# HighCWu/ControlLoRA

Measured on AMD Instinct MI355X. Metric: train images/sec SD-1.5+ControlLoRA 512^2 bs4/GPU, higher is better.
Workload: dtype f16; 1 GPU; configs/fill50k.json on SD-1.5 topology (seeded random weights), 512x512, bs=4/GPU, fp16; hot path = hint encoder + UNet fwd/bwd + adapter AdamW; latents/text embeddings synthetic (VAE/CLIP outside the hot path); global_batch=4, parallelism=dp1, hipgraph=True, allreduce_bytes=24188160, rccl_ranks=1, comm=torch, comm_requested=auto

## Files before the change

### controllora_amd/capi.py

```python
from __future__ import annotations

import ctypes as C
import os
from typing import Optional

import torch

_HERE = os.path.dirname(os.path.abspath(__file__))
LIB_PATH = os.environ.get("CLORA_LIB_PATH") or os.path.join(_HERE, "_build", "libclora.so")

ABI_VERSION = 4
OK, ERR_ARG, ERR_LAUNCH, ERR_WORKSPACE = 0, -1, -2, -3
_ERR = {ERR_ARG: "bad argument", ERR_LAUNCH: "kernel launch failed", ERR_WORKSPACE: "workspace too small"}


class CloraError(RuntimeError):
    pass


class ConvDesc(C.Structure):
    _fields_ = [(n, C.c_int) for n in (
        "enabled", "Hin", "Win", "Cin", "Hout", "Wout", "ksize", "mul", "kmul", "off", "lim_h", "lim_w", "shift",
        "need_even", "kchunk")]


class Epilogue(C.Structure):
    _fields_ = [("bias", C.c_void_p), ("rowadd", C.c_void_p), ("rows_per_batch", C.c_int), ("ld_rowadd", C.c_int),
                ("residual", C.c_void_p), ("ldr", C.c_int), ("lora_t", C.c_void_p), ("ldt", C.c_int),
                ("lora_u", C.c_void_p), ("ldu", C.c_int), ("lora_u_tr", C.c_int), ("lora_r", C.c_int), ("lora_seg", C.c_int), ("lora_scale", C.c_float),
                ("geglu", C.c_int), ("geglu_f", C.c_int), ("geglu_h", C.c_void_p), ("geglu_y", C.c_void_p),
                ("lora_dpack", C.c_void_p), ("lora_t_in", C.c_void_p), ("ldt_in", C.c_int), ("lora_t_in_rows", C.c_int),
                ("lora_t_in_mask", C.c_uint), ("defer", C.c_void_p),
                ("ln_gamma", C.c_void_p), ("ln_beta", C.c_void_p), ("ln_out", C.c_void_p), ("ln_eps", C.c_float),
                ("residual_lo", C.c_void_p), ("c_lo", C.c_void_p)]


class GemmTile(C.Structure):
    _fields_ = [(n, C.c_int) for n in ("tile_cfg", "family", "bm", "bn", "wm", "wn", "nst", "bk", "flags", "caps")]


TILE_RING, TILE_V1, TILE_EIGHT_PHASE, TILE_PATCH, TILE_PATCH_WIDE, TILE_STRIP = range(6)
TILE_CAP_GEGLU, TILE_CAP_DPACK, TILE_CAP_LN, TILE_CAP_CONV = 1, 2, 4, 8


class Deferred(C.Structure):
    _fields_ = [("partial", C.c_void_p), ("splits", C.c_int), ("M", C.c_int), ("N", C.c_int), ("C", C.c_void_p), ("ldc", C.c_int),
                ("epi", Epilogue)]


class LoraPackJob(C.Structure):
    _fields_ = [("D", C.c_void_p), ("out", C.c_void_p), ("ldd", C.c_int), ("R", C.c_int), ("K", C.c_int), ("kmajor", C.c_int),
                ("scale", C.c_float), ("pad_", C.c_int)]


class LoraDownJob(C.Structure):
    _fields_ = [("X", C.c_void_p), ("ldx", C.c_int), ("D", C.c_void_p), ("ldd", C.c_int), ("T", C.c_void_p), ("ldt", C.c_int),
                ("toff", C.c_int), ("M", C.c_int), ("K", C.c_int), ("R", C.c_int), ("accumulate", C.c_int), ("x_rows", C.c_int),
                ("d_kmajor", C.c_int), ("d_scale", C.c_float), ("X2", C.c_void_p), ("ldx2", C.c_int), ("x2_rows", C.c_int),
                ("r2", C.c_int), ("T_in", C.c_void_p), ("ldt_in", C.c_int), ("t_in_rows", C.c_int), ("t_in_r", C.c_int)]


class RankSite(C.Structure):
    _fields_ = [("Dq", C.c_void_p), ("lddq", C.c_int), ("Uc", C.c_void_p), ("lduc", C.c_int), ("M", C.c_void_p),
                ("Tc", C.c_void_p), ("ldtc", C.c_int), ("toff", C.c_int), ("Tq", C.c_void_p), ("ldtq", C.c_int),
                ("dTc", C.c_void_p), ("lddtc", C.c_int), ("gDq", C.c_void_p), ("gUc", C.c_void_p),
                ("rows", C.c_int), ("C", C.c_int), ("rc", C.c_int), ("scale", C.c_float)]


class LoraUpJob(C.Structure):
    _fields_ = [("base", C.c_void_p), ("ldb", C.c_int), ("T", C.c_void_p), ("ldt", C.c_int), ("toff", C.c_int), ("U", C.c_void_p),
                ("ldu", C.c_int), ("u_transposed", C.c_int), ("Y", C.c_void_p), ("ldy", C.c_int), ("M", C.c_int), ("N", C.c_int),
                ("R", C.c_int), ("scale", C.c_float)]


class LoraFoldMember(C.Structure):
    _fields_ = [("up", C.c_void_p), ("down", C.c_void_p), ("ldu", C.c_int), ("ldd", C.c_int), ("r", C.c_int), ("scale", C.c_float)]


LORA_FOLD_MAX_MEMBERS = 8


class LoraFoldJob(C.Structure):
    _fields_ = [("W", C.c_void_p), ("out", C.c_void_p), ("out_t", C.c_void_p), ("ldw", C.c_int), ("ldo", C.c_int), ("ldt", C.c_int),
                ("rows", C.c_int), ("K", C.c_int), ("nmem", C.c_int), ("m", LoraFoldMember * LORA_FOLD_MAX_MEMBERS)]


class ControlMixMember(C.Structure):
    _fields_ = [("T", C.c_void_p), ("ldt", C.c_int), ("toff", C.c_int), ("U", C.c_void_p), ("ldu", C.c_int), ("r", C.c_int),
                ("scale", C.c_float)]


CONTROL_MIX_MAX_MEMBERS = 8


class ControlMixJob(C.Structure):
    _fields_ = [("Y", C.c_void_p), ("ldy", C.c_int), ("M", C.c_int), ("N", C.c_int), ("rows_t", C.c_int), ("nmem", C.c_int),
                ("m", ControlMixMember * CONTROL_MIX_MAX_MEMBERS)]


class ControlChainMember(C.Structure):
    _fields_ = [("Dh", C.c_void_p), ("ldd", C.c_int), ("U", C.c_void_p), ("ldu", C.c_int), ("Tc", C.c_void_p), ("ldt", C.c_int),
                ("toff", C.c_int), ("r", C.c_int)]


CONTROL_CHAIN_MAX_MEMBERS = 8


class ControlChainJob(C.Structure):
    _fields_ = [("H", C.c_void_p), ("ldh", C.c_int), ("Y", C.c_void_p), ("ldy", C.c_int), ("G", C.c_void_p), ("ldg", C.c_int),
                ("M", C.c_int), ("C", C.c_int), ("rows_t", C.c_int), ("nmem", C.c_int), ("scale", C.c_float),
                ("m", ControlChainMember * CONTROL_CHAIN_MAX_MEMBERS)]


class LoraWgradJob(C.Structure):
    _fields_ = [("A", C.c_void_p), ("lda", C.c_int), ("T", C.c_void_p), ("ldt", C.c_int), ("toff", C.c_int), ("G", C.c_void_p),
                ("gs_n", C.c_int), ("gs_j", C.c_int), ("M", C.c_int), ("N", C.c_int), ("R", C.c_int), ("scale", C.c_float),
                ("a_rows", C.c_int), ("A2", C.c_void_p), ("lda2", C.c_int)]


class ConvPackJob(C.Structure):
    _fields_ = [("w", C.c_void_p), ("fwd", C.c_void_p), ("dgrad", C.c_void_p), ("Co", C.c_int), ("Ci", C.c_int), ("ksize", C.c_int),
                ("Cip", C.c_int), ("Cop", C.c_int), ("pad_", C.c_int)]


class ConvUnpackJob(C.Structure):
    _fields_ = [("stage", C.c_void_p), ("stage_b", C.c_void_p), ("grad_w", C.c_void_p), ("grad_b", C.c_void_p), ("Co", C.c_int),
                ("Ci", C.c_int), ("ksize", C.c_int), ("Cip", C.c_int)]


class SamplerCoef(C.Structure):
    _fields_ = [(n, C.c_float) for n in ("guidance", "x0_x", "x0_e", "k_x", "k_x0", "k_h", "k_e", "k_n")]


class ConvActJob(C.Structure):
    _fields_ = [("x", C.c_void_p), ("ldx", C.c_int), ("w", C.c_void_p), ("bias", C.c_void_p), ("y", C.c_void_p), ("ldy", C.c_int),
                ("Cin", C.c_int), ("Cout", C.c_int), ("relu", C.c_int)]


CONV_ACT_MAX_JOBS = 2
LORA_MAX_JOBS = 16
LORA_WGRAD_MAX_JOBS = 32
WGRAD_JOBS_PER_LAUNCH = min(LORA_WGRAD_MAX_JOBS, max(1, int(os.environ.get("CLORA_WGRAD_JOBS", "32"))))
CONV_MAX_JOBS = 32
CANNY_MAX_GROUP = 64
_P, _I, _Z, _F, _LL = C.c_void_p, C.c_int, C.c_size_t, C.c_float, C.c_longlong
_PROTOS = {
    "clora_gemm_f16": [_P, _I, _P, _P, _I, _I, _I, _I, C.POINTER(ConvDesc), C.POINTER(Epilogue), _I, _P, _Z, _P],
    "clora_gemm_f16_ex": [_P, _I, _P, _P, _I, _I, _I, _I, C.POINTER(ConvDesc), C.POINTER(Epilogue), _I, _I, _P, _Z, _P],
    "clora_conv_patch_eligible": [_I, C.POINTER(ConvDesc), _I],
    "clora_conv_strip_eligible": [_I, _I, C.POINTER(ConvDesc)],
    "clora_set_option": [C.c_char_p, _I],
    "clora_conv_wgrad_f16": [_P, _I, _P, _I, _P, _P, _I, _I, _I, C.POINTER(ConvDesc), _I, _P],
    "clora_conv_weight_pack_f32": [_P, _I, _I, _I, _I, _I, _P, _P, _P],
    "clora_conv_wgrad_unpack_f32": [_P, _P, _P, _P, _I, _I, _I, _I, _P],
    "clora_conv_weight_pack_multi_f32": [C.POINTER(ConvPackJob), _I, _P],
    "clora_conv_wgrad_unpack_multi_f32": [C.POINTER(ConvUnpackJob), _I, _P],
    "clora_attn_fwd_f16": [_P, _I, _P, _I, _P, _I, _P, _I, _P, _I, _I, _I, _I, _I, _F, _P],
    "clora_attn_max_head_dim": [_I],
    "clora_attn_fwd_causal_f16": [_P, _I, _P, _I, _P, _I, _P, _I, _I, _I, _I, _I, _F, _P],
    "clora_attn_bwd_f16": [_P, _I, _P, _I, _P, _I, _P, _I, _P, _I, _P, _P, _P, _I, _P, _I, _P, _I, _I, _I, _I, _I, _I, _F, _P, _Z, _P],
    "clora_groupnorm_fwd_f16": [_P, _P, _P, _P, _P, _I, _I, _I, _I, _F, _I, _P, _Z, _P],
    "clora_groupnorm_bwd_f16": [_P, _P, _P, _P, _P, _P, _P, _P, _P, _I, _I, _I, _I, _I, _I, _P, _Z, _P],
    "clora_groupnorm_fwd_f16_ex": [_P, _P, _I, C.POINTER(Deferred), _P, _P, _P, _P, _P, _I, _I, _I, _I, _F, _I, _P, _Z, _P],
    "clora_groupnorm_bwd_f16_ex": [_P, _P, C.POINTER(Deferred), _P, _P, _P, _I, _P, _P, _P, _P, _P, _I, _I, _I, _I, _I, _I, _P, _Z, _P],
    "clora_groupnorm_fwd_f16_team": [_P, _P, _I, C.POINTER(Deferred), _P, _P, _P, _P, _P, _I, _I, _I, _I, _F, _I, _P, _Z, _P, _Z, _P],
    "clora_groupnorm_fwd_f16_lo": [_P, _P, _I, C.POINTER(Deferred), _P, _P, _P, _P, _P, _I, _I, _I, _I, _F, _I, _P, _Z, _P, _Z, _P, _P, _P],
    "clora_layernorm_fwd_f16_lo": [_P, _P, _P, _P, _I, _I, _F, _P, _P],
    "clora_groupnorm_bwd_f16_team": [_P, _P, C.POINTER(Deferred), _P, _P, _P, _I, _P, _P, _P, _P, _P, _I, _I, _I, _I, _I, _I, _P, _Z, _P, _Z, _P],
    "clora_layernorm_bwd_f16_ex": [_P, _P, C.POINTER(Deferred), _P, _P, _P, _I, _I, _F, _P],
    "clora_finish_deferred": [C.POINTER(Deferred), _P],
    "clora_gemm_ln_fusable": [_I, _I, _I, _I, _I],
    "clora_gemm_tile_info": [_I, C.POINTER(GemmTile)],
    "clora_gemm_tile_at": [_I, C.POINTER(GemmTile)],
    "clora_gemm_fused_down_tile": [_I, _I, _I, C.POINTER(_I)],
    "clora_layernorm_fwd_f16": [_P, _P, _P, _P, _I, _I, _F, _P],
    "clora_softmax_rows_f16": [_P, _P, _I, _I, _I, _F, _P],
    "clora_layernorm_bwd_f16": [_P, _P, _P, _P, _P, _I, _I, _F, _P],
    "clora_geglu_fwd_f16": [_P, _P, _I, _I, _P],
    "clora_geglu_bwd_f16": [_P, _P, _P, _I, _I, _P],
    "clora_lora_down_f16": [_P, _I, _P, _I, _P, _I, _I, _I, _I, _I, _I, _I, _I, _F, _P],
    "clora_lora_down_multi_f16": [C.POINTER(LoraDownJob), _I, _P],
    "clora_lora_wgrad_multi_f16": [C.POINTER(LoraWgradJob), _I, _P, _Z, _P],
    "clora_lora_pack_f16": [_P, _I, _I, _P],
    "clora_rank_compose_f32": [C.POINTER(RankSite), _I, _P],
    "clora_rank_mix_f32": [C.POINTER(RankSite), _I, _I, _P, _Z, _P],
    "clora_rank_compose_bwd_f32": [C.POINTER(RankSite), _I, _P, _P],
    "clora_lora_up_f16": [_P, _I, _P, _I, _I, _P, _I, _I, _P, _I, _I, _I, _I, _F, _P],
    "clora_lora_up_multi_f16": [C.POINTER(LoraUpJob), _I, _P],
    "clora_lora_fold_f16": [_P, _I, _P],
    "clora_control_mix_q_f16": [C.POINTER(ControlMixJob), _P],
    "clora_control_chain_f16": [C.POINTER(ControlChainJob), _P],
    "clora_lora_wgrad_f16": [_P, _I, _P, _I, _I, _P, _I, _I, _I, _I, _I, _F, _I, _P, _Z, _P],
    "clora_comm_unique_id": [_P],
    "clora_comm_init": [_P, _I, _I],
    "clora_comm_library": [C.c_char_p, _Z],
    "clora_comm_world": [],
    "clora_comm_rank": [],
    "clora_allreduce_flat_f32": [_P, _Z, _P],
    "clora_comm_destroy": [],
    "clora_add_f16": [_P, _P, _P, _Z, _P],
    "clora_silu_f16": [_P, _P, _Z, _P],
    "clora_timestep_embedding_f16": [_P, _I, _I, _P, _P, _I, _I, _P],
    "clora_silu_bwd_f16": [_P, _P, _P, _Z, _P],
    "clora_quick_gelu_f16": [_P, _P, _Z, _P],
    "clora_copy2d_f16": [_P, _I, _P, _I, _Z, _I, _P],
    "clora_pool2x2_sum_f16": [_P, _P, _I, _I, _I, _I, _P],
    "clora_colsum_f16": [_P, _I, _P, _I, _I, _P],
    "clora_mse_f16": [_P, _P, _P, _P, _Z, _F, _P, _P],
    "clora_mse_weighted_f16": [_P, _P, _P, _P, _P, _I, _Z, _F, _P, _P],
    "clora_cast_f32_to_f16": [_P, _P, _Z, _P],
    "clora_cast_f16_to_f32": [_P, _P, _Z, _P],
    "clora_grad_sumsq_f32": [_P, _Z, _P, _P],
    "clora_optim_prep_f32": [_P, _F, _F, _F, _I, _F, _F, _I, _P],
    "clora_adamw_flat_f32": [_P, _P, _P, _P, _Z, _P, _F, _F, _F, _F, _F, _P],
    "clora_canny_classify_u8": [_P, _P, _P, _P, _I, _I, _I, _I, _P],
    "clora_canny_hysteresis_u8": [_P, _P, _I, _I, _I, _I, _I, _P],
    "clora_canny_emit": [_P, _P, _P, _I, _I, _I, _P],
    "clora_sampler_step_f16": [_P, _LL, _LL, _LL, _LL, _P, _P, _P, _P, _P, _LL, _I, _I, _I, _I, C.POINTER(SamplerCoef), _P],
    "clora_conv_act_f16": [C.POINTER(ConvActJob), _I, _I, _I, _I, _I, _P, _Z, _P],
    "clora_conv_act_workspace": [C.POINTER(ConvActJob), _I, _I, _I, _I, _I],
    "clora_conv_act_splits": [C.POINTER(ConvActJob), _I, _I, _I, _I, _I],
    "clora_conv_act_pack_f32": [_P, _P, _P, _I, _I, _I, _I, _P],
    "clora_maxpool2x2_f16": [_P, _P, _I, _I, _I, _I, _P],
    "clora_abi_version": [],
    "clora_clock_probe": [_P, _I, _I, _P],
    "clora_groupnorm_workspace_bytes": [_I, _I, _I, _I, _I, _I],
    "clora_groupnorm_team_state_bytes": [],
    "clora_lora_wgrad_workspace_bytes": [_I, _I, _I],
    "clora_rank_gram_ws_bytes": [_I, _I],
}


class Lib:

    def __init__(self, path: str = LIB_PATH, require_device: bool = True):
        if not os.path.exists(path):
            raise CloraError(
                f"{path} not found: the gfx950 kernel library is not built.  Run `python -m controllora_amd.build` "
                "(hipcc --offload-arch=gfx950).  There is no CPU / PyTorch fallback for this path.")
        self.path = path
        self.require_device = require_device
        self.cdll = C.CDLL(path)
        got = self.cdll.clora_abi_version() if hasattr(self.cdll, "clora_abi_version") else -1
        if got != ABI_VERSION and os.environ.get("CLORA_ABI_ANY", "") != "1":
            raise CloraError(f"{path} reports ABI {got}, this binding is written for ABI {ABI_VERSION} (include/clora.h); rebuild with "
                             "`python -m controllora_amd.build` (CLORA_ABI_ANY=1 overrides for A/B runs of older builds whose "
                             "struct layouts are known to match)")
        for name, argtypes in _PROTOS.items():
            if not hasattr(self.cdll, name) and os.environ.get("CLORA_ABI_ANY", "") == "1":
                continue
            fn = getattr(self.cdll, name)
            fn.argtypes = argtypes
            fn.restype = C.c_int
        self.cdll.clora_build_info.restype = C.c_char_p
        self.cdll.clora_groupnorm_workspace_bytes.restype = C.c_size_t
        self.cdll.clora_groupnorm_team_state_bytes.restype = C.c_size_t
        self.cdll.clora_lora_wgrad_workspace_bytes.restype = C.c_size_t
        self.cdll.clora_rank_gram_ws_bytes.restype = C.c_size_t
        if hasattr(self.cdll, "clora_conv_act_workspace"):
            self.cdll.clora_conv_act_workspace.restype = C.c_size_t
        self._options_from_env()
        self._derived = {}

    def derived(self, key, make):
        if key not in self._derived:
            self._derived[key] = make(self)
        return self._derived[key]

    def tiles(self) -> dict:
        def read(L):
            rows, r = {}, GemmTile()
            while L.cdll.clora_gemm_tile_at(len(rows), C.byref(r)) == OK:
                rows[r.tile_cfg], r = r, GemmTile()
            return rows
        return self.derived("tiles", read)

    _ENV_OPTIONS = {"CLORA_TILE_ORDER": ("tile_order", {"m": 0, "n": 1, "auto": 2, "a": 2, "grid": 3, "g": 3}), "CLORA_LN_ROWS": ("ln_rows", None),
                    "CLORA_ATTN_FWD_WAVES": ("attn_fwd_waves", None), "CLORA_ATTN_BWD_WAVES": ("attn_bwd_waves", None),
                    "CLORA_GN_BLOCKS": ("gn_blocks", None), "CLORA_EPI_TWO_PHASE": ("epi_two_phase", None),
                    "CLORA_LORA_DOWN_MODE": ("lora_down_mode", None), "CLORA_GN_UNROLL": ("gn_unroll", None),
                    "CLORA_EPI_HOIST": ("epi_hoist", None), "CLORA_GN_RESIDENT": ("gn_resident", None),
                    "CLORA_DEFER_MAX_ROWS": ("defer_max_rows", None), "CLORA_WGRAD_PATCH": ("wgrad_patch", None), "CLORA_STRIP_BLOCKS": ("strip_blocks", None),
                    "CLORA_GN_TEAM": ("gn_team", None)}

    def _options_from_env(self):
        for var, (name, names) in self._ENV_OPTIONS.items():
            v = os.environ.get(var)
            if v is None or v == "":
                continue
            try:
                val = names[v] if (names and v in names) else int(v)
                self.call("clora_set_option", name.encode(), val)
            except (ValueError, CloraError) as e:
                allowed = f"one of {sorted(names)} or an integer" if names else "an integer in the range include/clora.h documents"
                raise CloraError(f"environment variable {var}={v!r} is not a valid value for the library option "
                                 f"{name!r} (expected {allowed})") from e

    def call(self, name: str, *args) -> None:
        rc = getattr(self.cdll, name)(*args)
        if rc != OK:
            raise CloraError(f"{name} failed: {_ERR.get(rc, rc)}")


_LIB: Optional[Lib] = None


def lib() -> Lib:
    global _LIB
    if _LIB is None:
        _LIB = Lib()
    return _LIB


def ptr(t: Optional[torch.Tensor], dtype=None) -> Optional[int]:
    if t is None:
        return None
    L = lib()
    if L.require_device and not t.is_cuda:
        raise CloraError("libclora kernels need tensors on a HIP device (no CPU fallback)")
    if dtype is not None and t.dtype != dtype:
        raise CloraError(f"expected {dtype}, got {t.dtype}")
    return t.data_ptr()


def stream() -> Optional[int]:
    if lib().require_device:
        return torch.cuda.current_stream().cuda_stream
    return None
```

### controllora_amd/csrc/clora_common.h

```cpp
#pragma once
#include <hip/hip_runtime.h>
#include <stdint.h>

typedef _Float16 half_t;
typedef _Float16 half2v __attribute__((ext_vector_type(2)));
typedef _Float16 half4v __attribute__((ext_vector_type(4)));
typedef _Float16 half8 __attribute__((ext_vector_type(8)));
typedef float floatx4 __attribute__((ext_vector_type(4)));

#define CLORA_WAVE 64

#define CLORA_OK 0
#define CLORA_ERR_ARG (-1)
#define CLORA_ERR_LAUNCH (-2)
#define CLORA_ERR_WORKSPACE (-3)

#ifndef CLORA_ASYNC_PRIMS
#define CLORA_ASYNC_PRIMS
#define CLORA_GLDS16(gptr, lptr)                                                                      \
    __builtin_amdgcn_global_load_lds((const __attribute__((address_space(1))) void*)(gptr),            \
                                     (__attribute__((address_space(3))) void*)(lptr), 16, 0, 0)
#define CLORA_WAIT_VMCNT(n) asm volatile("s_waitcnt vmcnt(%0)" ::"n"(n) : "memory")
#define CLORA_RAW_BARRIER() __builtin_amdgcn_s_barrier()
typedef __fp16 clora_fp16x4 __attribute__((__vector_size__(4 * sizeof(__fp16))));
// ... 10 lines not shown
#define CLORA_KEEP_PURE(x) asm("" : "+v"(x))
#define CLORA_FMA_F32(acc, a, b) asm("v_fma_f32 %0, %1, %2, %0" : "+v"(acc) : "v"(a), "v"(b))
#define CLORA_CYCLES() ((unsigned long long)__builtin_readcyclecounter())
#define CLORA_WALL_TICKS() ((unsigned long long)wall_clock64())
#define CLORA_MFMA_INPLACE(acc, a, b) asm volatile("v_mfma_f32_16x16x32_f16 %0, %1, %2, %0" : "+v"(acc) : "v"(a), "v"(b))
#define CLORA_MFMA_DRAIN() asm volatile("s_nop 15\n\ts_nop 15" ::: "memory")
#define CLORA_WAIT_LGKMCNT(n) asm volatile("s_waitcnt lgkmcnt(%0)" ::"n"(n) : "memory")
#define CLORA_SETPRIO(n) __builtin_amdgcn_s_setprio(n)
#define CLORA_SCHED_BARRIER() __builtin_amdgcn_sched_barrier(0)
typedef __attribute__((address_space(1))) unsigned long long clora_gu64;
typedef __attribute__((address_space(1))) unsigned clora_gu32;
#define CLORA_LD_AGENT_U64(p) __hip_atomic_load((clora_gu64*)(p), __ATOMIC_RELAXED, __HIP_MEMORY_SCOPE_AGENT)
#define CLORA_ST_AGENT_U64(p, v) __hip_atomic_store((clora_gu64*)(p), (unsigned long long)(v), __ATOMIC_RELAXED, __HIP_MEMORY_SCOPE_AGENT)
#define CLORA_LD_AGENT_U32(p) __hip_atomic_load((clora_gu32*)(p), __ATOMIC_RELAXED, __HIP_MEMORY_SCOPE_AGENT)
#define CLORA_ST_AGENT_U32(p, v) __hip_atomic_store((clora_gu32*)(p), (unsigned)(v), __ATOMIC_RELAXED, __HIP_MEMORY_SCOPE_AGENT)
#define CLORA_SLEEP() __builtin_amdgcn_s_sleep(1)
#endif
#ifndef CLORA_SEQUENTIAL_BLOCKS
#define CLORA_SEQUENTIAL_BLOCKS 0
#endif

__device__ __forceinline__ floatx4 mfma16(half8 a, half8 b, floatx4 c) {
    return __builtin_amdgcn_mfma_f32_16x16x32_f16(a, b, c, 0, 0, 0);
}

__device__ __forceinline__ half8 ld8(const half_t* p) { return *reinterpret_cast<const half8*>(p); }
__device__ __forceinline__ void st8(half_t* p, half8 v) { *reinterpret_cast<half8*>(p) = v; }
__device__ __forceinline__ half4v ld4(const half_t* p) { return *reinterpret_cast<const half4v*>(p); }
__device__ __forceinline__ void st4(half_t* p, half4v v) { *reinterpret_cast<half4v*>(p) = v; }
__device__ __forceinline__ half8 zero8() {
    half8 z = {0, 0, 0, 0, 0, 0, 0, 0};
    return z;
}
__device__ __forceinline__ floatx4 zero4f() {
    floatx4 z = {0.f, 0.f, 0.f, 0.f};
    return z;
}

__device__ __forceinline__ float sigmoid_f(float x) { return CLORA_RCP(1.0f + CLORA_EXP2(-1.4426950408889634f * x)); }
__device__ __forceinline__ float silu_f(float x) { return x * sigmoid_f(x); }
__device__ __forceinline__ float dsilu_f(float x) {
    float s = sigmoid_f(x);
    return s * (1.0f + x * (1.0f - s));
}
__device__ __forceinline__ void gelu_parts(float x, float& cdf, float& pdf) {
    const float ax = fabsf(x) * 0.70710678118654752f;
    const float t = CLORA_RCP(1.0f + 0.3275911f * ax);
    const float ex = CLORA_EXP2(-1.4426950408889634f * ax * ax);
    const float poly = t * (0.254829592f + t * (-0.284496736f + t * (1.421413741f + t * (-1.453152027f + t * 1.061405429f))));
    const float erf_abs = 1.0f - poly * ex;
    cdf = 0.5f * (1.0f + (x < 0.f ? -erf_abs : erf_abs));
    pdf = 0.39894228040143268f * ex;
}
__device__ __forceinline__ float gelu_f(float x) {
    float cdf, pdf;
    gelu_parts(x, cdf, pdf);
    return x * cdf;
}
__device__ __forceinline__ float dgelu_f(float x) {
    float cdf, pdf;
    gelu_parts(x, cdf, pdf);
    return cdf + x * pdf;
}

__device__ __forceinline__ float wave_sum(float v) {
    v += __shfl_xor(v, 32);
    v += __shfl_xor(v, 16);
    v += __shfl_xor(v, 8);
    v += __shfl_xor(v, 4);
    v += __shfl_xor(v, 2);
    v += __shfl_xor(v, 1);
    return v;
}
__device__ __forceinline__ float wave_max(float v) {
    v = fmaxf(v, __shfl_xor(v, 32));
    v = fmaxf(v, __shfl_xor(v, 16));
    v = fmaxf(v, __shfl_xor(v, 8));
    v = fmaxf(v, __shfl_xor(v, 4));
    v = fmaxf(v, __shfl_xor(v, 2));
    v = fmaxf(v, __shfl_xor(v, 1));
    return v;
}

enum { CLORA_OPT_TILE_ORDER = 0, CLORA_OPT_LN_ROWS, CLORA_OPT_ATTN_FWD_WAVES, CLORA_OPT_ATTN_BWD_WAVES, CLORA_OPT_GN_BLOCKS, CLORA_OPT_EPI_TWO_PHASE, CLORA_OPT_LORA_DOWN_MODE, CLORA_OPT_GN_UNROLL, CLORA_OPT_EPI_HOIST, CLORA_OPT_GN_RESIDENT, CLORA_OPT_DEFER_MAX_ROWS, CLORA_OPT_WGRAD_PATCH, CLORA_OPT_STRIP_BLOCKS, CLORA_OPT_GN_TEAM, CLORA_OPT_COUNT };
__attribute__((visibility("hidden"))) int clora_option(int id);
static inline int clora_xcd_policy() { return clora_option(CLORA_OPT_TILE_ORDER); }
static inline int clora_ln_rows() { return clora_option(CLORA_OPT_LN_ROWS); }

static inline int clora_check_launch() { return hipGetLastError() == hipSuccess ? CLORA_OK : CLORA_ERR_LAUNCH; }
static inline int clora_cdiv(long a, long b) { return (int)((a + b - 1) / b); }
```

### controllora_amd/csrc/clora_ew.hip

```cpp
#include "clora_common.h"
#include "../../include/clora.h"

namespace {

int ew_grid(size_t work) {
    size_t b = (work + 255) / 256;
    return (int)(b > 4096 ? 4096 : (b < 1 ? 1 : b));
}

#define EW_LOOP(i, n) for (size_t i = (size_t)blockIdx.x * 256 + threadIdx.x; i < (n); i += (size_t)gridDim.x * 256)

__global__ __launch_bounds__(256) void add_kernel(const half_t* a, const half_t* b, half_t* y, size_t n8) {
    EW_LOOP(i, n8) {
        const half8 x = ld8(a + i * 8), z = ld8(b + i * 8);
        half8 o;
#pragma unroll
        for (int e = 0; e < 8; ++e) o[e] = (half_t)((float)x[e] + (float)z[e]);
        st8(y + i * 8, o);
    }
}

__global__ __launch_bounds__(256) void silu_kernel(const half_t* x, half_t* y, size_t n8) {
    EW_LOOP(i, n8) {
        const half8 v = ld8(x + i * 8);
// ... 336 lines not shown
    if (!pred || !target || !loss_sum || (n & 7)) return CLORA_ERR_ARG;
    int blocks = ew_grid(n / 8);
    if (blocks > 256) blocks = 256;
    hipLaunchKernelGGL(mse_kernel, dim3(blocks), dim3(256), 0, (hipStream_t)stream, H(pred), H(target), loss_sum, HM(dpred),
                       n / 8, grad_scale, loss_scale);
    return clora_check_launch();
}
extern "C" int clora_mse_weighted_f16(const clora_half* pred, const clora_half* target, const float* weights, float* sample_sums,
                                      clora_half* dpred, int B, size_t n_per_sample, float grad_scale, const float* loss_scale,
                                      void* stream) {
    if (!pred || !target || !weights || !sample_sums || B <= 0 || n_per_sample == 0 || (n_per_sample & 7)) return CLORA_ERR_ARG;
    const int bx = n_per_sample / 8 > 256 ? 2 : 1;
    const int by = B < 1024 ? B : 1024;
    hipLaunchKernelGGL(mse_weighted_kernel, dim3(bx, by), dim3(256), 0, (hipStream_t)stream, H(pred), H(target), weights, sample_sums,
                       HM(dpred), B, n_per_sample / 8, grad_scale, loss_scale);
    return clora_check_launch();
}
extern "C" int clora_cast_f32_to_f16(const float* x, clora_half* y, size_t n, void* stream) {
    if (!x || !y) return CLORA_ERR_ARG;
    hipLaunchKernelGGL(cast_f32_f16_kernel, dim3(ew_grid(n)), dim3(256), 0, (hipStream_t)stream, x, HM(y), n);
    return clora_check_launch();
}
extern "C" int clora_cast_f16_to_f32(const clora_half* x, float* y, size_t n, void* stream) {
    if (!x || !y) return CLORA_ERR_ARG;
    hipLaunchKernelGGL(cast_f16_f32_kernel, dim3(ew_grid(n)), dim3(256), 0, (hipStream_t)stream, H(x), y, n);
    return clora_check_launch();
}
extern "C" int clora_grad_sumsq_f32(const float* g, size_t n, float* state, void* stream) {
    if (!g || !state) return CLORA_ERR_ARG;
    int blocks = ew_grid(n);
    if (blocks > kSumsqBlocks) blocks = kSumsqBlocks;
    hipLaunchKernelGGL(grad_sumsq_kernel, dim3(blocks), dim3(256), 0, (hipStream_t)stream, g, n);
    hipLaunchKernelGGL(grad_sumsq_fold_kernel, dim3(1), dim3(256), 0, (hipStream_t)stream, blocks, state);
    return clora_check_launch();
}
extern "C" int clora_optim_prep_f32(float* state, float max_norm, float beta1, float beta2, int dynamic_scale,
                                    float growth_factor, float backoff_factor, int growth_interval, void* stream) {
    if (!state) return CLORA_ERR_ARG;
    hipLaunchKernelGGL(optim_prep_kernel, dim3(1), dim3(64), 0, (hipStream_t)stream, state, max_norm, beta1, beta2,
                       dynamic_scale, growth_factor, backoff_factor, growth_interval);
    return clora_check_launch();
}
extern "C" int clora_adamw_flat_f32(float* p, const float* g, float* m, float* v, size_t n, const float* state, float lr,
                                    float beta1, float beta2, float eps, float weight_decay, void* stream) {
    if (!p || !g || !m || !v || !state) return CLORA_ERR_ARG;
    hipLaunchKernelGGL(adamw_kernel, dim3(ew_grid(n)), dim3(256), 0, (hipStream_t)stream, p, g, m, v, n, state, lr, beta1,
                       beta2, eps, weight_decay);
    return clora_check_launch();
}
__global__ __launch_bounds__(256) void clock_probe_kernel(unsigned long long* out, int iters) {
    const int l = threadIdx.x & 63;
    half8 a, b;
#pragma unroll
    for (int e = 0; e < 8; ++e) {
        a[e] = (half_t)(((l * 37 + e * 11 + blockIdx.x) % 61) * (1.0f / 32.0f) - 0.95f);
        b[e] = (half_t)(((l * 53 + e * 29 + threadIdx.x) % 59) * (1.0f / 32.0f) - 0.9f);
    }
    floatx4 acc[8];
#pragma unroll
    for (int q = 0; q < 8; ++q) acc[q] = zero4f();
    __syncthreads();
    const unsigned long long c0 = CLORA_CYCLES(), w0 = CLORA_WALL_TICKS();
    for (int it = 0; it < iters; ++it) {
#pragma unroll
        for (int q = 0; q < 8; ++q) CLORA_MFMA_INPLACE(acc[q], a, b);
    }
    CLORA_MFMA_DRAIN();
    float s = 0.f;
#pragma unroll
    for (int q = 0; q < 8; ++q) s += acc[q][0] + acc[q][1] + acc[q][2] + acc[q][3];
    const unsigned long long c1 = CLORA_CYCLES(), w1 = CLORA_WALL_TICKS();
    if (threadIdx.x == 0) {
        out[3 * (size_t)blockIdx.x] = c1 - c0;
        out[3 * (size_t)blockIdx.x + 1] = w1 - w0;
        out[3 * (size_t)blockIdx.x + 2] = (unsigned long long)__float_as_uint(s);
    }
}
extern "C" int clora_clock_probe(unsigned long long* out, int blocks, int iters, void* stream) {
    if (!out || blocks <= 0 || iters <= 0) return CLORA_ERR_ARG;
    hipLaunchKernelGGL(clock_probe_kernel, dim3(blocks), dim3(256), 0, (hipStream_t)stream, out, iters);
    return clora_check_launch();
}
extern "C" int clora_abi_version(void) { return CLORA_ABI_VERSION; }
extern "C" const char* clora_build_info(void) { return "libclora gfx950 (v_mfma_f32_16x16x32_f16), ABI 2"; }

namespace {
struct ConvPackJobs { clora_conv_pack_job_t j[CLORA_CONV_MAX_JOBS]; };
struct ConvUnpackJobs { clora_conv_unpack_job_t j[CLORA_CONV_MAX_JOBS]; };

__global__ __launch_bounds__(256) void conv_weight_pack_multi_kernel(ConvPackJobs jobs) {
    const clora_conv_pack_job_t& p = jobs.j[blockIdx.y];
    const int taps = p.ksize * p.ksize, Co = p.Co, Ci = p.Ci, Cip = p.Cip, Cop = p.Cop;
    const float* w = p.w;
    half_t* fwd = (half_t*)p.fwd;
    half_t* dgrad = (half_t*)p.dgrad;
    const int nf = Co * taps * Cip, nd = dgrad ? Cip * taps * Cop : 0;
    for (int i = blockIdx.x * 256 + threadIdx.x; i < nf + nd; i += gridDim.x * 256) {
        if (i < nf) {
            const int ci = i % Cip, tap = (i / Cip) % taps, co = i / (Cip * taps);
            fwd[i] = ci < Ci ? (half_t)w[((size_t)co * Ci + ci) * taps + tap] : (half_t)0.f;
        } else {
            const int q = i - nf;
            const int co = q % Cop, tap = (q / Cop) % taps, ci = q / (Cop * taps);
            dgrad[q] = (ci < Ci && co < Co) ? (half_t)w[((size_t)co * Ci + ci) * taps + tap] : (half_t)0.f;
        }
    }
}

__global__ __launch_bounds__(256) void conv_wgrad_unpack_multi_kernel(ConvUnpackJobs jobs) {
    const clora_conv_unpack_job_t& p = jobs.j[blockIdx.y];
    const int taps = p.ksize * p.ksize, Co = p.Co, Ci = p.Ci, Cip = p.Cip;
    const int nw = Co * taps * Cip;
    for (int i = blockIdx.x * 256 + threadIdx.x; i < nw + (p.grad_b ? Co : 0); i += gridDim.x * 256) {
        if (i < nw) {
            const int ci = i % Cip, tap = (i / Cip) % taps, co = i / (Cip * taps);
            const float v = p.stage[i];
            p.stage[i] = 0.f;
            if (ci < Ci) p.grad_w[((size_t)co * Ci + ci) * taps + tap] += v;
        } else {
            const int co = i - nw;
            p.grad_b[co] += p.stage_b[co];
            p.stage_b[co] = 0.f;
        }
    }
}
}

extern "C" int clora_conv_weight_pack_multi_f32(const clora_conv_pack_job_t* jobs, int njobs, void* stream) {
    if (!jobs || njobs <= 0 || njobs > CLORA_CONV_MAX_JOBS) return CLORA_ERR_ARG;
    ConvPackJobs cj;
    long most = 0;
    for (int i = 0; i < njobs; ++i) {
        const clora_conv_pack_job_t& j = jobs[i];
        if (!j.w || !j.fwd || j.Co <= 0 || j.Ci <= 0 || (j.ksize != 1 && j.ksize != 3) || j.Cip < j.Ci || (j.Cip & 7) ||
            (j.dgrad && (j.Cop < j.Co || (j.Cop & 7))))
            return CLORA_ERR_ARG;
        const int taps = j.ksize * j.ksize;
        const long total = (long)j.Co * taps * j.Cip + (j.dgrad ? (long)j.Cip * taps * j.Cop : 0);
        if (total > most) most = total;
        cj.j[i] = j;
    }
    int blocks = clora_cdiv(most, 256 * 4);
    if (blocks > 1024) blocks = 1024;
    hipLaunchKernelGGL(conv_weight_pack_multi_kernel, dim3(blocks, njobs), dim3(256), 0, (hipStream_t)stream, cj);
    return clora_check_launch();
}

extern "C" int clora_conv_wgrad_unpack_multi_f32(const clora_conv_unpack_job_t* jobs, int njobs, void* stream) {
    if (!jobs || njobs <= 0 || njobs > CLORA_CONV_MAX_JOBS) return CLORA_ERR_ARG;
    ConvUnpackJobs cj;
    long most = 0;
    for (int i = 0; i < njobs; ++i) {
        const clora_conv_unpack_job_t& j = jobs[i];
        if (!j.stage || !j.grad_w || j.Co <= 0 || j.Ci <= 0 || j.Cip < j.Ci || (j.ksize != 1 && j.ksize != 3) ||
            ((j.grad_b == nullptr) != (j.stage_b == nullptr)))
            return CLORA_ERR_ARG;
        const long total = (long)j.Co * j.ksize * j.ksize * j.Cip + (j.grad_b ? j.Co : 0);
        if (total > most) most = total;
        cj.j[i] = j;
    }
    int blocks = clora_cdiv(most, 256 * 4);
    if (blocks > 1024) blocks = 1024;
    hipLaunchKernelGGL(conv_wgrad_unpack_multi_kernel, dim3(blocks, njobs), dim3(256), 0, (hipStream_t)stream, cj);
    return clora_check_launch();
}
```

### controllora_amd/csrc/clora_gemm.hip

```cpp
#include <string.h>
#include "clora_common.h"
#include "../../include/clora.h"
#include "clora_epilogue.h"

namespace {

struct GemmArgs {
    const half_t* A;
    const half_t* B;
    half_t* C;
    float* partial;
    int lda, ldc, M, N, K;
    int k_per_split;
    int tiles_n;
    int two_phase;
    int hoist_on;
    int tiles_m, n_major;
    int xg_s, xg_m, xg_n;
    clora_conv_t conv;
    clora_epilogue_t epi;
};

template <int BM, int BN, int WM, int WN>
__global__ __launch_bounds__(256) void gemm_kernel(GemmArgs p) {
    constexpr int BK = 32, LD = BK + 8;
    constexpr int FM = BM / WM / 16, FN = BN / WN / 16;
    constexpr int A_CH = BM / 64, B_CH = BN / 64;
    constexpr int STAGE = (BM + BN) * LD;
    constexpr int C_LD = BN + 8;
    constexpr int SMEM = (2 * STAGE > BM * C_LD) ? 2 * STAGE : BM * C_LD;
    __shared__ __attribute__((aligned(16))) half_t smem[SMEM];

    const int t = threadIdx.x;
    const int tile_m = blockIdx.x / p.tiles_n, tile_n = blockIdx.x % p.tiles_n;
    const int split = blockIdx.y;
    const int m0 = tile_m * BM, n0 = tile_n * BN;
    const int kbeg = split * p.k_per_split;
    const int kend = (kbeg + p.k_per_split < p.K) ? kbeg + p.k_per_split : p.K;
    const int nk = (kend - kbeg + BK - 1) / BK;

    const int kc = t & 3, r0 = t >> 2;
    const bool conv = p.conv.enabled != 0;
    bool a_ok[A_CH];
    size_t a_base[A_CH];
    int a_ty[A_CH], a_tx[A_CH];
#pragma unroll
    for (int i = 0; i < A_CH; ++i) {
        const int m = m0 + r0 + 64 * i;
        a_ok[i] = m < p.M;
        a_base[i] = 0; a_ty[i] = 0; a_tx[i] = 0;
        if (a_ok[i]) {
            if (!conv) {
                a_base[i] = (size_t)m * p.lda;
            } else {
                const int hw = p.conv.Hout * p.conv.Wout;
                const int b = m / hw, rem = m - b * hw;
                const int yo = rem / p.conv.Wout, xo = rem - yo * p.conv.Wout;
                a_base[i] = (size_t)b * p.conv.Hin * p.conv.Win;
                a_ty[i] = yo * p.conv.mul + p.conv.off;
                a_tx[i] = xo * p.conv.mul + p.conv.off;
            }
        }
    }
    bool b_ok[B_CH];
    size_t b_base[B_CH];
#pragma unroll
    for (int i = 0; i < B_CH; ++i) {
        const int n = n0 + r0 + 64 * i;
        b_ok[i] = n < p.N;
        b_base[i] = (size_t)n * p.K;
    }
    int k = kbeg + kc * 8;
    const int kcs = p.conv.kchunk > 0 ? p.conv.kchunk : p.conv.Cin, ntap = p.conv.ksize * p.conv.ksize;
    int tap = 0, ci = k, cb = 0;
    if (conv) { cb = (k / (ntap * kcs)) * kcs; const int r = k % (ntap * kcs); tap = r / kcs; ci = r - tap * kcs; }

    half8 ra[A_CH], rb[B_CH];
    auto load_tile = [&]() {
        const bool kok = k < kend;
        int ky = 0, kx = 0;
        if (conv) { ky = tap / p.conv.ksize; kx = tap - ky * p.conv.ksize; }
#pragma unroll
        for (int i = 0; i < A_CH; ++i) {
            half8 v = zero8();
            if (a_ok[i] && kok) {
                if (!conv) {
                    v = ld8(p.A + a_base[i] + k);
                } else {
                    const int ty = a_ty[i] + ky * p.conv.kmul, tx = a_tx[i] + kx * p.conv.kmul;
                    bool ok = ty >= 0 && ty < p.conv.lim_h && tx >= 0 && tx < p.conv.lim_w;
                    if (p.conv.need_even) ok = ok && (((ty | tx) & 1) == 0);
                    if (ok)
                        v = ld8(p.A + (a_base[i] + (size_t)(ty >> p.conv.shift) * p.conv.Win + (tx >> p.conv.shift)) * p.conv.Cin + cb + ci);
                }
            }
            ra[i] = v;
        }
#pragma unroll
        for (int i = 0; i < B_CH; ++i) {
            half8 v = zero8();
            if (b_ok[i] && kok) v = ld8(p.B + b_base[i] + k);
            rb[i] = v;
        }
// ... 800 lines not shown
#pragma unroll
        for (int ks = 0; ks < 2; ++ks)
#pragma unroll
            for (int j = 0; j < 2; ++j) b0[ks][j] = ld8(buf + 1 * HT + b_row + j * 16 * BK + fsw[ks]);
#pragma unroll
        for (int ks = 0; ks < 2; ++ks)
#pragma unroll
            for (int i = 0; i < 4; ++i) a0[ks][i] = ld8(buf + 0 * HT + a_row + i * 16 * BK + fsw[ks]);
        stage(kt + 1, 3);
        CLORA_WAIT_LGKMCNT(0);
        CLORA_RAW_BARRIER();
        CLORA_SCHED_BARRIER();
        CLORA_SETPRIO(1);
#pragma unroll
        for (int ks = 0; ks < 2; ++ks)
#pragma unroll
            for (int i = 0; i < 4; ++i)
#pragma unroll
                for (int j = 0; j < 2; ++j) acc[i][j] = mfma16(a0[ks][i], b0[ks][j], acc[i][j]);
        CLORA_SETPRIO(0);
        CLORA_SCHED_BARRIER();
        CLORA_RAW_BARRIER();
#pragma unroll
        for (int ks = 0; ks < 2; ++ks)
#pragma unroll
            for (int j = 0; j < 2; ++j) b1[ks][j] = ld8(buf + 2 * HT + b_row + j * 16 * BK + fsw[ks]);
        stage(kt + 2, 0);
        CLORA_WAIT_LGKMCNT(0);
        CLORA_RAW_BARRIER();
        CLORA_SCHED_BARRIER();
        CLORA_SETPRIO(1);
#pragma unroll
        for (int ks = 0; ks < 2; ++ks)
#pragma unroll
            for (int i = 0; i < 4; ++i)
#pragma unroll
                for (int j = 0; j < 2; ++j) acc[i][2 + j] = mfma16(a0[ks][i], b1[ks][j], acc[i][2 + j]);
        CLORA_SETPRIO(0);
        CLORA_SCHED_BARRIER();
        CLORA_RAW_BARRIER();
#pragma unroll
        for (int ks = 0; ks < 2; ++ks)
#pragma unroll
            for (int i = 0; i < 4; ++i) a1[ks][i] = ld8(buf + 3 * HT + a_row + i * 16 * BK + fsw[ks]);
        stage(kt + 2, 1);
        CLORA_WAIT_LGKMCNT(0);
        CLORA_RAW_BARRIER();
        CLORA_SCHED_BARRIER();
        CLORA_SETPRIO(1);
#pragma unroll
        for (int ks = 0; ks < 2; ++ks)
#pragma unroll
            for (int i = 0; i < 4; ++i)
#pragma unroll
                for (int j = 0; j < 2; ++j) acc[4 + i][2 + j] = mfma16(a1[ks][i], b1[ks][j], acc[4 + i][2 + j]);
        CLORA_SETPRIO(0);
        CLORA_SCHED_BARRIER();
        CLORA_RAW_BARRIER();
        stage(kt + 2, 2);
        CLORA_WAIT_VMCNT(kInFlight8p);
        CLORA_RAW_BARRIER();
        CLORA_SCHED_BARRIER();
        CLORA_SETPRIO(1);
#pragma unroll
        for (int ks = 0; ks < 2; ++ks)
#pragma unroll
            for (int i = 0; i < 4; ++i)
#pragma unroll
                for (int j = 0; j < 2; ++j) acc[4 + i][j] = mfma16(a1[ks][i], b0[ks][j], acc[4 + i][j]);
        CLORA_SETPRIO(0);
        CLORA_SCHED_BARRIER();
        CLORA_RAW_BARRIER();
    }
    if (wr == 0) CLORA_RAW_BARRIER();
    CLORA_WAIT_VMCNT(0);
    dma_epilogue<BM, BN, WM, WN, NT, SMEM, true>(p, acc, m0, n0, split, smem, t);
}

template <int BM, int BN> struct PatchCfg {
    static constexpr int MAXPP = (BM == 256) ? 400 : 288;
};
constexpr int kPatchWide = 392;

template <int BM, int BN, int WM, int WN, int NST, int MAXPP_ = 0>
__global__ __launch_bounds__(WM * WN * 64, 1) void conv3x3_patch_kernel(GemmArgs p) {
    constexpr int NT = WM * WN * 64, NW = WM * WN, BK = 64;
    constexpr int FM = BM / WM / 16, FN = BN / WN / 16;
    constexpr int MAXPP = MAXPP_ > 0 ? MAXPP_ : PatchCfg<BM, BN>::MAXPP;
    constexpr int PA_IN = (MAXPP / 8 + NW - 1) / NW;
    constexpr int B_NI = BN / 8;
    constexpr int B_IN = (B_NI + NW - 1) / NW;
    constexpr bool NODUMP = BM == 256 && BN == 160;
    constexpr int PATCH = MAXPP * 64 + (NODUMP ? 0 : 512);
    constexpr int BST = BN * BK + (((B_NI % NW) && !NODUMP) ? 512 : 0);
    constexpr int SMEM = 2 * PATCH + NST * BST;
    static_assert(SMEM * 2 <= 160 * 1024, "LDS per workgroup");
    static_assert(!NODUMP || (PA_IN >= 2 && (NW * PA_IN - NW) * 8 <= MAXPP && B_IN >= 2 && NW * B_IN - NW <= B_NI), "a surplus instruction needs a valid predecessor in its wave");
    static_assert(64 * (BN + 4) * 2 <= SMEM, "epilogue staging");
    __shared__ __attribute__((aligned(16))) half_t smem[SMEM];
    half_t* const Pb = smem;
    half_t* const Bring = smem + 2 * PATCH;

    const int t = threadIdx.x;
    const int tiles = gridDim.x, nwg = gridDim.x * gridDim.y;
    const int lin = blockIdx.y * gridDim.x + blockIdx.x;
    const int xq = nwg >> 3, xr = nwg & 7, xcd = lin & 7;
    const int logical = (xcd < xr ? xcd * (xq + 1) : xr * (xq + 1) + (xcd - xr) * xq) + (lin >> 3);
    int split = logical / tiles, tile = logical - split * tiles;
    int tile_m = p.n_major ? tile % p.tiles_m : tile / p.tiles_n, tile_n = p.n_major ? tile / p.tiles_m : tile % p.tiles_n;
    if (p.xg_m) {
        const int rn = p.tiles_n / p.xg_n, rm = p.tiles_m / p.xg_m, rs = (int)gridDim.y / p.xg_s, idx = lin >> 3;
        const int sl = idx / (rm * rn), r = idx - sl * (rm * rn);
        split = (xcd / (p.xg_m * p.xg_n)) * rs + sl;
        tile_m = ((xcd / p.xg_n) % p.xg_m) * rm + r / rn;
        tile_n = (xcd % p.xg_n) * rn + r % rn;
    }
    const int m0 = tile_m * BM, n0 = tile_n * BN;
    const int w = t >> 6, l = t & 63, g = l >> 4, li = l & 15;
    const int wm = w / WN, wn = w % WN;
    const half_t* zero_page = reinterpret_cast<const half_t*>(g_clora_zero16);

    const int H = p.conv.Hout, W = p.conv.Wout, C = p.conv.Cin, HW = H * W, sh = p.conv.shift;
    const int nimg = HW >= BM ? 1 : BM / HW, rpi = HW >= BM ? (W >= BM ? 1 : BM / W) : H, TW = W > BM ? BM : W;
    const int PW = TW + 2, PRI = rpi + 2;
    const int npp = nimg * PRI * PW;
    const int b0 = m0 / HW, y0 = (m0 - b0 * HW) / W, x0 = W > BM ? (m0 - b0 * HW - y0 * W) : 0;
    const int nb = p.M / HW;
    const int slabs = C / 64;
    const int cs_beg = split * p.k_per_split, cs_end_ = cs_beg + p.k_per_split;
    const int cs_end = cs_end_ < slabs ? cs_end_ : slabs;

    int poff[PA_IN];
#pragma unroll
    for (int j = 0; j < PA_IN; ++j) {
        const int ip = (NODUMP && (w + NW * j) * 8 >= MAXPP) ? w + NW * (j - 1) : w + NW * j;
        const int sl = ip * 64 + l, pp = sl >> 3, pos = sl & 7;
        poff[j] = -1;
        if (pp < npp) {
            const int img = pp / (PRI * PW), rem = pp - img * (PRI * PW);
            const int pr = rem / PW, pc = rem - pr * PW;
            const int y = y0 - 1 + pr, x = x0 + pc - 1, b = b0 + img;
            if (b < nb && y >= 0 && y < H && x >= 0 && x < W)
                poff[j] = ((b * p.conv.Hin + (y >> sh)) * p.conv.Win + (x >> sh)) * C + ((pos ^ (pp & 7)) * 8);
        }
    }
    auto issue_patch = [&](int cs, int buf) {
        half_t* dst = Pb + buf * PATCH;
        const bool live = cs < cs_end;
#pragma unroll
        for (int j = 0; j < PA_IN; ++j) {
            const int i = w + NW * j;
            const half_t* src = (live && poff[j] >= 0) ? p.A + poff[j] + cs * 64 : zero_page;
            CLORA_GLDS16(src, (i * 8 < MAXPP) ? dst + i * 512 : dst + (NODUMP ? (i - NW) * 512 : MAXPP * 64));
        }
    };
    const int lrow = l >> 3, bpos = l & 7, kc = bpos ^ (lrow & 7);
    bool b_ok[B_IN];
    size_t b_base[B_IN];
#pragma unroll
    for (int i = 0; i < B_IN; ++i) {
        const int ib = w + NW * i, ibe = (NODUMP && ib >= B_NI) ? ib - NW : ib, n = n0 + ibe * 8 + lrow;
        b_ok[i] = ibe < B_NI && n < p.N;
        b_base[i] = (size_t)n * p.K + kc * 8;
    }
    const int kbeg = cs_beg * 576, kend = cs_end * 576;
    int kq = kbeg;
    auto issue_b = [&](int buf) {
        half_t* Bs = Bring + buf * BST;
        const bool kok = kq < kend;
#pragma unroll
        for (int i = 0; i < B_IN; ++i) {
            const int ib = w + NW * i;
            const half_t* src = (b_ok[i] && kok) ? p.B + b_base[i] + kq : zero_page;
            CLORA_GLDS16(src, Bs + (ib < B_NI ? ib * 8 * BK : (NODUMP ? (ib - NW) * 8 * BK : BN * BK)));
        }
        kq += BK;
    };

    int pp0[FM];
#pragma unroll
    for (int i = 0; i < FM; ++i) {
        const int ml = wm * FM * 16 + i * 16 + li;
        const int img = ml / (rpi * TW), rem = ml - img * (rpi * TW);
        const int yl = rem / TW, x = rem - yl * TW;
        pp0[i] = (img * PRI + yl) * PW + x;
    }
    int bsw[2];
#pragma unroll
    for (int ks = 0; ks < 2; ++ks) bsw[ks] = ((ks * 4 + g) ^ (li & 7)) * 8;
    const int toff0 = 1 + p.conv.off, tmul = p.conv.kmul;

    floatx4 acc[FM][FN];
#pragma unroll
    for (int i = 0; i < FM; ++i)
#pragma unroll
        for (int j = 0; j < FN; ++j) acc[i][j] = zero4f();

    issue_patch(cs_beg, 0);
#pragma unroll
    for (int st = 0; st < NST - 1; ++st) issue_b(st);
    int rd = 0, wr = NST - 1;
    for (int cs = cs_beg; cs < cs_end; ++cs) {
        const half_t* P = Pb + ((cs - cs_beg) & 1) * PATCH;
#pragma unroll
        for (int tap = 0; tap < 9; ++tap) {
            if (tap >= 1 && tap <= NST - 1) CLORA_WAIT_VMCNT((NST - 2) * B_IN + PA_IN);
            else CLORA_WAIT_VMCNT((NST - 2) * B_IN);
            CLORA_RAW_BARRIER();
            issue_b(wr);
            wr = (wr + 1 == NST) ? 0 : wr + 1;
            if (tap == 0) issue_patch(cs + 1, ((cs - cs_beg) & 1) ^ 1);
            const half_t* Bs = Bring + rd * BST;
            rd = (rd + 1 == NST) ? 0 : rd + 1;
            const int ky = tap / 3, kx = tap - ky * 3;
            const int tapoff = (toff0 + ky * tmul) * PW + (toff0 + kx * tmul);
            half8 af[2][FM], bf[2][FN];
#pragma unroll
            for (int i = 0; i < FM; ++i) {
                const int pp = pp0[i] + tapoff;
                const half_t* q = P + pp * 64;
                const int k7 = pp & 7;
                af[0][i] = ld8(q + ((g ^ k7) * 8));
                af[1][i] = ld8(q + (((4 + g) ^ k7) * 8));
            }
#pragma unroll
            for (int ks = 0; ks < 2; ++ks)
#pragma unroll
                for (int j = 0; j < FN; ++j) bf[ks][j] = ld8(Bs + (wn * FN * 16 + j * 16 + li) * BK + bsw[ks]);
#pragma unroll
            for (int ks = 0; ks < 2; ++ks)
#pragma unroll
                for (int i = 0; i < FM; ++i)
#pragma unroll
                    for (int j = 0; j < FN; ++j) acc[i][j] = mfma16(af[ks][i], bf[ks][j], acc[i][j]);
        }
    }
    CLORA_WAIT_VMCNT(0);
    dma_epilogue<BM, BN, WM, WN, NT, SMEM>(p, acc, m0, n0, split, smem, t);
}

__global__ __launch_bounds__(256) void splitk_finish_kernel(GemmArgs p, int splits) {
    const size_t chunks = (size_t)p.M * (p.N / 8);
    for (size_t c = (size_t)blockIdx.x * 256 + threadIdx.x; c < chunks; c += (size_t)gridDim.x * 256) {
        const int m = (int)(c / (p.N / 8));
        const int n = (int)(c - (size_t)m * (p.N / 8)) * 8;
        if (p.epi.c_lo) {
            half8 lo;
            st8(p.C + (size_t)m * p.ldc + n, finish_chunk8(p.partial, splits, p.M, p.N, p.epi, m, n, &lo));
            st8((half_t*)p.epi.c_lo + (size_t)m * p.ldc + n, lo);
        } else {
            st8(p.C + (size_t)m * p.ldc + n, finish_chunk8(p.partial, splits, p.M, p.N, p.epi, m, n));
        }
    }
}

struct WgradArgs {
    const half_t* dY;
    const half_t* X;
    float* dW;
    float* db;
    int ldy, ldx, M, N, K;
    int oihw_ci;
    int m_per_block;
    int tiles_n, tiles_k;
    clora_conv_t conv;
};

__device__ __attribute__((aligned(16))) const unsigned short g_clora_one16[8] = {0x3C00u, 0, 0, 0, 0, 0, 0, 0};

__global__ __launch_bounds__(256, 3) void conv_wgrad_kernel(WgradArgs p) {
    constexpr int BMR = 64, NST = 3;
    constexpr int SUB = BMR * 16;
    constexpr int STAGE = 8 * SUB;
    __shared__ __attribute__((aligned(16))) half_t smem[NST * STAGE];
    const int t = threadIdx.x;
    const int tile = blockIdx.x;
    const int tn = tile % p.tiles_n, tk = tile / p.tiles_n;
    const int n0 = tn * 64, k0 = tk * 64;
    const int mbeg = blockIdx.y * p.m_per_block;
    const int mend = (mbeg + p.m_per_block < p.M) ? mbeg + p.m_per_block : p.M;
    const int nst = (mend - mbeg + BMR - 1) / BMR;
    const bool conv = p.conv.enabled != 0;
    const half_t* zero_page = reinterpret_cast<const half_t*>(g_clora_zero16);
    const half_t* one_page = reinterpret_cast<const half_t*>(g_clora_one16);

    const int w = t >> 6, l = t & 63, g = l >> 4, li = l & 15;
    const int lm = (w & 1) * 32 + (l >> 1);
    const int c8 = (l & 1) * 8;
    int ncol[2], kcol[2], ky[2], kx[2], ci[2];
    bool n_ok[2], k_ok[2], k_one[2];
#pragma unroll
    for (int q = 0; q < 2; ++q) {
        const int sub = q * 2 + (w >> 1);
        ncol[q] = n0 + sub * 16 + c8;
        kcol[q] = k0 + sub * 16 + c8;
        n_ok[q] = ncol[q] < p.N;
        k_ok[q] = kcol[q] < p.K;
        k_one[q] = p.db != nullptr && kcol[q] == p.K;
        ky[q] = 0; kx[q] = 0; ci[q] = kcol[q];
        if (conv && k_ok[q]) {
            const int tap = kcol[q] / p.conv.Cin;
            ci[q] = kcol[q] - tap * p.conv.Cin;
            ky[q] = tap / p.conv.ksize;
            kx[q] = tap - ky[q] * p.conv.ksize;
        }
    }
    int mrow = mbeg + lm;
    auto issue_stage = [&](int buf) {
        half_t* base = smem + buf * STAGE + (w & 1) * 512;
        const bool mok = mrow < mend;
        size_t xrow = 0;
        int ty0 = 0, tx0 = 0;
        if (mok) {
            if (!conv) {
                xrow = (size_t)mrow * p.ldx;
            } else {
                const int hw = p.conv.Hout * p.conv.Wout;
// ... 464 lines not shown
        const size_t orow = ((size_t)img * p.H + y) * p.W + x0 + (w * MF) * 16 + li;
#pragma unroll
        for (int m = 0; m < MF; ++m)
#pragma unroll
            for (int f = 0; f < NF; ++f) {
                const int n = f * 16 + 4 * g;
                if (n < p.N) {
                    half4v o;
#pragma unroll
                    for (int r = 0; r < 4; ++r) o[r] = (half_t)acc[f][m][r];
                    st4(p.C + (orow + m * 16) * p.ldc + n, o);
                }
            }
        CLORA_RAW_BARRIER();
    }
    CLORA_WAIT_VMCNT(0);
}

template <int CIN, int NF, int TW>
int launch_strip(StripArgs& a, hipStream_t s) {
    a.nseg = a.W / TW;
    const long strips = (long)a.nimg * a.nseg;
    const long target = clora_option(CLORA_OPT_STRIP_BLOCKS);
    long rpb = ((long)a.H * strips + target - 1) / target;
    if (rpb < 8) rpb = 8;
    if (rpb > a.H) rpb = a.H;
    a.rows_per_block = (int)rpb;
    a.row_chunks = clora_cdiv(a.H, rpb);
    hipLaunchKernelGGL((conv3x3_strip_kernel<CIN, NF, TW>), dim3((unsigned)(strips * a.row_chunks)), dim3(256), 0, s, a);
    return clora_check_launch();
}

template <int NF, int TW>
int launch_strip8(StripArgs& a, hipStream_t s) {
    a.nseg = a.W / TW;
    const long strips = (long)a.nimg * a.nseg;
    const long target = clora_option(CLORA_OPT_STRIP_BLOCKS);
    long rpb = ((long)a.H * strips + target - 1) / target;
    if (rpb < 8) rpb = 8;
    if (rpb > a.H) rpb = a.H;
    a.rows_per_block = (int)rpb;
    a.row_chunks = clora_cdiv(a.H, rpb);
    hipLaunchKernelGGL((conv3x3_strip8_kernel<NF, TW>), dim3((unsigned)(strips * a.row_chunks)), dim3(256), 0, s, a);
    return clora_check_launch();
}

int strip_plan(int M, int N, const clora_conv_t& c) {
    if (!c.enabled || c.ksize != 3 || c.mul != 1 || c.shift != 0 || c.need_even != 0 || c.kchunk != 0) return 0;
    if (!((c.kmul == 1 && c.off == -1) || (c.kmul == -1 && c.off == 1))) return 0;
    if (c.Hout != c.Hin || c.Wout != c.Win || c.lim_h != c.Hin || c.lim_w != c.Win || c.Hout <= 0 || (c.Wout % 128)) return 0;
    if ((M % (c.Hout * c.Wout)) || (long)M * 64 >= (1L << 31) || (N & 3)) return 0;
    if (c.Cin == 8 && N <= 32) return 802;
    if (c.Cin == 8 && N <= 64) return 804;
    if (c.Cin == 32 && N <= 32) return 3202;
    if (c.Cin == 32 && N <= 64) return 3204;
    if (c.Cin == 64 && N <= 32) return 6402;
    return 0;
}

__global__ __launch_bounds__(256) void conv_weight_pack_kernel(const float* w, int Co, int Ci, int taps, int Cip, int Cop,
                                                               half_t* fwd, half_t* dgrad) {
    const int nf = Co * taps * Cip, nd = dgrad ? Cip * taps * Cop : 0;
    for (int i = blockIdx.x * 256 + threadIdx.x; i < nf + nd; i += gridDim.x * 256) {
        if (i < nf) {
            const int ci = i % Cip, tap = (i / Cip) % taps, co = i / (Cip * taps);
            fwd[i] = ci < Ci ? (half_t)w[((size_t)co * Ci + ci) * taps + tap] : (half_t)0.f;
        } else {
            const int q = i - nf;
            const int co = q % Cop, tap = (q / Cop) % taps, ci = q / (Cop * taps);
            dgrad[q] = (ci < Ci && co < Co) ? (half_t)w[((size_t)co * Ci + ci) * taps + tap] : (half_t)0.f;
        }
    }
}

int conv_mode(const GemmArgs& a, int bk) {
    const clora_conv_t& c = a.conv;
    if (!c.enabled) return 0;
    const int kcs = c.kchunk > 0 ? c.kchunk : c.Cin;
    const bool fast = c.ksize == 3 && c.shift == 0 && c.need_even == 0 && (c.kmul == 1 || c.kmul == -1) &&
                      (kcs % bk) == 0 && (a.k_per_split % bk) == 0 && c.lim_h == c.Hin && c.lim_w == c.Win;
    return fast ? 2 : 1;
}

int g_opts[CLORA_OPT_COUNT] = {3, 1, 0, 0, 512, 1, 1, 0, 1, 1, 4, 1, 512, 2};
int tile_order_mode() { return g_opts[CLORA_OPT_TILE_ORDER]; }

double fabric_model_bytes(int tiles_m, int tiles_n, int splits, double a_panel, double b_panel, bool n_major) {
    const int tiles = tiles_m * tiles_n, nwg = tiles * splits;
    const int inner = n_major ? tiles_m : tiles_n;
    const int xq = nwg >> 3, xr = nwg & 7;
    double bytes = 0.0;
    int beg = 0;
    for (int x = 0; x < 8; ++x) {
        const int end = beg + xq + (x < xr ? 1 : 0);
        for (int sp = beg / tiles; sp * tiles < end && sp < splits; ++sp) {
            const int t0 = (beg > sp * tiles ? beg : sp * tiles) - sp * tiles, t1 = (end < (sp + 1) * tiles ? end : (sp + 1) * tiles) - sp * tiles;
            if (t1 <= t0) continue;
            const int outer = (t1 - 1) / inner - t0 / inner + 1;
            const int inn = (t1 - t0 < inner) ? t1 - t0 : inner;
            bytes += n_major ? outer * b_panel + inn * a_panel : outer * a_panel + inn * b_panel;
        }
        beg = end;
    }
    return bytes;
}

void pick_tile_order(GemmArgs& a, int BM, int BN, int splits, bool patch) {
    a.tiles_m = clora_cdiv(a.M, BM);
    a.n_major = 0;
    a.xg_s = a.xg_m = a.xg_n = 0;
    const int mode = tile_order_mode();
    if (mode == 0 || a.tiles_m == 1 || a.tiles_n == 1) return;
    if (mode == 1) { a.n_major = 1; return; }
    const double kper = patch ? (double)a.k_per_split * 576 : (double)a.k_per_split;
    const double a_panel = a.conv.enabled && a.conv.ksize == 3 ? BM * (kper / 9.0) * 2.0 * 1.5 : BM * kper * 2.0;
    const double b_panel = BN * kper * 2.0;
    const double m_cost = fabric_model_bytes(a.tiles_m, a.tiles_n, splits, a_panel, b_panel, false);
    const double n_cost = fabric_model_bytes(a.tiles_m, a.tiles_n, splits, a_panel, b_panel, true);
    a.n_major = n_cost < 0.85 * m_cost;
    if (mode == 3) {
        double best = 0.95 * (a.n_major ? n_cost : m_cost);
        for (int gs = 1; gs <= 8; gs *= 2)
            for (int gm = 1; gs * gm <= 8; gm *= 2) {
                const int gn = 8 / (gs * gm);
                if (splits % gs || a.tiles_m % gm || a.tiles_n % gn) continue;
                const double c = 8.0 * (splits / gs) * ((a.tiles_m / gm) * a_panel + (a.tiles_n / gn) * b_panel);
                if (c < best) { best = c; a.xg_s = gs; a.xg_m = gm; a.xg_n = gn; }
            }
        if (a.xg_m) a.n_major = 0;
    }
}

constexpr int kG = CLORA_TILE_CAP_GEGLU, kD = CLORA_TILE_CAP_DPACK, kL = CLORA_TILE_CAP_LN, kC = CLORA_TILE_CAP_CONV;
#define CLORA_GEMM_TILES(RING, V1, EIGHT, PATCH, WPATCH, STRIP)                                                                      \
    PATCH(71, 256, 128, 4, 2, 3, 64, 0, 0)           \
    PATCH(72, 128, 128, 2, 4, 3, 64, 0, 0)           \
    PATCH(73, 128, 128, 4, 2, 3, 64, 0, 0)           \
    PATCH(74, 256, 64, 8, 1, 4, 64, 0, 0)                                                                                            \
    PATCH(75, 128, 64, 4, 2, 4, 64, 0, 0)                                                                                            \
    WPATCH(77, 128, 128, 2, 4, 3, 64, 0, 0)          \
    WPATCH(78, 128, 64, 4, 2, 4, 64, 0, 0)                                                                                           \
    PATCH(79, 256, 160, 4, 2, 3, 64, 0, 0)           \
    PATCH(76, 128, 160, 4, 2, 3, 64, 0, 0)           \
    RING(1, 128, 128, 2, 2, 3, 32, 0, kG | kC)       \
    RING(2, 128, 64, 4, 1, 3, 32, 0, kC)                                                                                             \
    RING(3, 64, 64, 2, 2, 3, 32, 0, kC)                                                                                              \
    RING(4, 128, 128, 2, 2, 5, 32, 0, kG | kC)       \
    RING(5, 128, 64, 4, 1, 6, 32, 0, kC)                                                                                             \
    RING(6, 64, 64, 2, 2, 8, 32, 0, kC)                                                                                              \
    RING(7, 256, 128, 2, 2, 3, 32, 0, kG | kC)       \
    RING(8, 256, 128, 2, 2, 3, 32, 1, kG | kC)                                                                                       \
    RING(21, 128, 128, 2, 2, 2, 64, 0, kG | kD | kC)  \
    RING(22, 128, 64, 4, 1, 3, 64, 0, kD | kC)                                                                                       \
    RING(23, 64, 64, 2, 2, 3, 64, 0, kD | kC)                                                                                        \
    RING(26, 128, 64, 4, 1, 2, 64, 0, kD | kC)                                                                                       \
    RING(31, 128, 128, 2, 2, 3, 32, 1, kG | kC)      \
    RING(32, 128, 64, 4, 1, 3, 32, 1, kC)                                                                                            \
    RING(33, 64, 64, 2, 2, 3, 32, 1, kC)                                                                                             \
    RING(9, 128, 128, 2, 2, 3, 32, 2, kG | kC)       \
    RING(51, 128, 320, 4, 2, 2, 64, 0, kD | kL | kC)  \
    RING(52, 64, 320, 2, 4, 3, 64, 0, kD | kL | kC)  \
    RING(53, 128, 256, 4, 2, 3, 64, 0, kG | kC)                                                                                      \
    RING(57, 256, 320, 4, 2, 2, 64, 1, kC)           \
    RING(58, 256, 256, 4, 2, 2, 64, 1, kG | kC)                                                                                      \
    EIGHT(59, 256, 256, 2, 4, 0, 64, 0, kG)          \
    RING(54, 128, 320, 4, 2, 2, 64, 1, kD | kL | kC)  \
    RING(55, 64, 320, 2, 4, 3, 64, 1, kD | kL | kC)                                                                                  \
    RING(56, 128, 256, 4, 2, 3, 64, 1, kG | kC)                                                                                      \
    RING(41, 128, 128, 2, 2, 2, 64, 1, kG | kD | kC)  \
    RING(42, 128, 64, 4, 1, 3, 64, 1, kD | kC)                                                                                       \
    RING(43, 64, 64, 2, 2, 3, 64, 1, kD | kC)                                                                                        \
    V1(11, 128, 128, 2, 2, 3, 32, 0, kC)             \
    V1(12, 128, 64, 4, 1, 3, 32, 0, kC)              \
    V1(13, 64, 64, 2, 2, 3, 32, 0, kC)                                                                                               \
    STRIP(61, 0, 0, 0, 0, 0, 0, 0, 0)
#ifdef CLORA_DMA_PROBE
#define CLORA_GEMM_PROBE_TILES(RING)                                                                                    \
    RING(91, 128, 128, 2, 2, 2, 64, 4, 0) RING(92, 128, 128, 2, 2, 2, 64, 8, 0) RING(93, 128, 128, 2, 2, 2, 64, 12, 0)  \
    RING(94, 128, 64, 4, 1, 2, 64, 4, 0) RING(95, 128, 64, 4, 1, 2, 64, 8, 0) RING(96, 128, 64, 4, 1, 2, 64, 12, 0)
#else
#define CLORA_GEMM_PROBE_TILES(RING)
#endif

constexpr bool tile_carries_dpack(int BM, int BN, int waves, int NST, int BK) {
    return BK == 64 && ((waves == 8 && BN == 320 && BM <= 128) || (waves == 4 && BM * BN <= 128 * 128 && NST <= 3));
}
constexpr bool tile_takes_geglu(int BN) { return BN % 128 == 0; }
constexpr bool tile_fuses_ln(int BM, int BN, int waves) { return BN == 320 && waves == 8 && (BM == 64 || BM == 128); }

#define CLORA_ROW(FAM, cfg, BM, BN, WM, WN, NST, BK, FLAGS, caps) {cfg, FAM, BM, BN, WM, WN, NST, BK, FLAGS, caps},
#define ROW_RING(...) CLORA_ROW(CLORA_TILE_RING, __VA_ARGS__)
#define ROW_V1(...) CLORA_ROW(CLORA_TILE_V1, __VA_ARGS__)
#define ROW_EIGHT(...) CLORA_ROW(CLORA_TILE_EIGHT_PHASE, __VA_ARGS__)
#define ROW_PATCH(...) CLORA_ROW(CLORA_TILE_PATCH, __VA_ARGS__)
#define ROW_WPATCH(...) CLORA_ROW(CLORA_TILE_PATCH_WIDE, __VA_ARGS__)
#define ROW_STRIP(...) CLORA_ROW(CLORA_TILE_STRIP, __VA_ARGS__)
constexpr clora_gemm_tile_t kTileRows[] = {CLORA_GEMM_TILES(ROW_RING, ROW_V1, ROW_EIGHT, ROW_PATCH, ROW_WPATCH, ROW_STRIP)
                                           CLORA_GEMM_PROBE_TILES(ROW_RING)};
constexpr int kNumTileRows = sizeof(kTileRows) / sizeof(kTileRows[0]);
constexpr clora_gemm_tile_t kNoTile = {-1, -1, 0, 0, 0, 0, 0, 32, 0, 0};

#define CHECK_RING(cfg, BM, BN, WM, WN, NST, BK, FLAGS, caps)                                                                         \
    static_assert((((caps) & kD) != 0) == tile_carries_dpack(BM, BN, (WM) * (WN), NST, BK), "tile " #cfg ": D bit");                 \
    static_assert((((caps) & kG) != 0) == tile_takes_geglu(BN), "tile " #cfg ": G bit");                                             \
    static_assert((((caps) & kL) != 0) == tile_fuses_ln(BM, BN, (WM) * (WN)), "tile " #cfg ": L bit");
#define CHECK_OTHER(cfg, BM, BN, WM, WN, NST, BK, FLAGS, caps) static_assert(((caps) & (kD | kL)) == 0, "tile " #cfg ": only the DMA ring carries D / L");
CLORA_GEMM_TILES(CHECK_RING, CHECK_OTHER, CHECK_OTHER, CHECK_OTHER, CHECK_OTHER, CHECK_OTHER)

const clora_gemm_tile_t& tile_row(int cfg) {
    for (const clora_gemm_tile_t& r : kTileRows)
        if (r.tile_cfg == cfg) return r;
    return kNoTile;
}

template <int BM, int BN, int WM, int WN, int NST = 3, int BK = 32, int FLAGS = 0>
int launch_gemm(GemmArgs& a, int splits, hipStream_t s, bool dma) {
    a.tiles_n = clora_cdiv(a.N, BN);
    const int tiles_m = clora_cdiv(a.M, BM);
    pick_tile_order(a, BM, BN, splits, false);
    if (!dma) { a.n_major = 0; a.xg_s = a.xg_m = a.xg_n = 0; }
    const dim3 grid(tiles_m * a.tiles_n, splits);
    if (dma && a.epi.lora_dpack) {
        if constexpr (tile_carries_dpack(BM, BN, WM * WN, NST, BK)) {
            hipLaunchKernelGGL((gemm_dma_kernel<BM, BN, WM, WN, NST, 0, BK, FLAGS, 8>), grid, dim3(WM * WN * 64), 0, s, a);
            return clora_check_launch();
        } else {
            return CLORA_ERR_ARG;
        }
    }
    if (dma) {
        const int cm = conv_mode(a, BK);
        if (cm == 0) hipLaunchKernelGGL((gemm_dma_kernel<BM, BN, WM, WN, NST, 0, BK, FLAGS>), grid, dim3(WM * WN * 64), 0, s, a);
        else if (cm == 1) hipLaunchKernelGGL((gemm_dma_kernel<BM, BN, WM, WN, NST, 1, BK, FLAGS>), grid, dim3(WM * WN * 64), 0, s, a);
        else hipLaunchKernelGGL((gemm_dma_kernel<BM, BN, WM, WN, NST, 2, BK, FLAGS>), grid, dim3(WM * WN * 64), 0, s, a);
    }
    else if constexpr (BM * BN <= 128 * 128 && WM * WN == 4)
        hipLaunchKernelGGL((gemm_kernel<BM, BN, WM, WN>), dim3(tiles_m * a.tiles_n, splits), dim3(256), 0, s, a);
    else return CLORA_ERR_ARG;
    return clora_check_launch();
}

int launch_gemm_8p(GemmArgs& a, int splits, hipStream_t s) {
    a.tiles_n = clora_cdiv(a.N, 256);
    pick_tile_order(a, 256, 256, splits, false);
    const dim3 grid(clora_cdiv(a.M, 256) * a.tiles_n, splits);
    hipLaunchKernelGGL((gemm_8p_kernel<0>), grid, dim3(512), 0, s, a);
    return clora_check_launch();
}

bool patch_eligible(const GemmArgs& a, int bm, int maxpp = 0) {
    const clora_conv_t& c = a.conv;
    if (!c.enabled || c.ksize != 3 || c.mul != 1 || c.need_even != 0 || c.kchunk != 64 || (c.Cin % 64)) return false;
    if (c.shift == 0) {
        if (!((c.kmul == 1 && c.off == -1) || (c.kmul == -1 && c.off == 1))) return false;
        if (c.Hout != c.Hin || c.Wout != c.Win || c.lim_h != c.Hin || c.lim_w != c.Win) return false;
    } else {
        if (c.shift != 1 || c.kmul != 1 || c.off != -1 || c.Hout != 2 * c.Hin || c.Wout != 2 * c.Win || c.lim_h != c.Hout || c.lim_w != c.Wout)
            return false;
    }
    const int W = c.Wout, HW = c.Hout * c.Wout;
    if (W <= 0 || (a.M % HW) || (long)a.M * c.Cin >= (1L << 31)) return false;
    if ((bm % W) && !(maxpp > 0 && (W % bm) == 0)) return false;
    if (!((HW % bm) == 0 || (bm % HW) == 0)) return false;
    const int nimg = HW >= bm ? 1 : bm / HW, rpi = HW >= bm ? (W >= bm ? 1 : bm / W) : c.Hout, tw = W > bm ? bm : W;
    return nimg * (rpi + 2) * (tw + 2) <= (maxpp > 0 ? maxpp : (bm == 256 ? 400 : 288));
}

bool is_patch_tile(const clora_gemm_tile_t& r) { return r.family == CLORA_TILE_PATCH || r.family == CLORA_TILE_PATCH_WIDE; }
bool patch_eligible(const GemmArgs& a, const clora_gemm_tile_t& r) {
    return patch_eligible(a, r.bm, r.family == CLORA_TILE_PATCH_WIDE ? kPatchWide : 0);
}

template <int BM, int BN, int WM, int WN, int NST, int MAXPP_ = 0>
int launch_patch(GemmArgs& a, int splits, hipStream_t s) {
    a.tiles_n = clora_cdiv(a.N, BN);
    pick_tile_order(a, BM, BN, splits, true);
    const dim3 grid(clora_cdiv(a.M, BM) * a.tiles_n, splits);
    hipLaunchKernelGGL((conv3x3_patch_kernel<BM, BN, WM, WN, NST, MAXPP_>), grid, dim3(WM * WN * 64), 0, s, a);
    return clora_check_launch();
}

int finish_or_defer(GemmArgs& a, int splits, clora_deferred_t* defer, hipStream_t s) {
    if (defer) {
        defer->partial = a.partial; defer->splits = splits; defer->M = a.M; defer->N = a.N; defer->C = (clora_half*)a.C; defer->ldc = a.ldc;
        defer->epi = a.epi;
        defer->epi.defer = nullptr;
        return CLORA_OK;
    }
    const size_t chunks = (size_t)a.M * (a.N / 8);
    int blocks = (int)((chunks + 255) / 256);
    if (blocks > 2048) blocks = 2048;
    hipLaunchKernelGGL(splitk_finish_kernel, dim3(blocks), dim3(256), 0, s, a, splits);
    return clora_check_launch();
}


}

namespace {
struct TileCfg { int cfg, conc; double t_k; };
const TileCfg kTiles[3] = {{1, 3, 0.85e-6}, {2, 4, 0.82e-6}, {3, 6, 0.52e-6}};

void plan_gemm(int M, int N, int K, int max_split, int& tile, int& splits) {
    const int ksteps = clora_cdiv(K, 32);
    double best = 1e30;
    tile = 0; splits = 1;
    for (int c = 0; c < 3; ++c) {
        const TileCfg& tc = kTiles[c];
        const clora_gemm_tile_t& r = tile_row(tc.cfg);
        const long tiles = (long)clora_cdiv(M, r.bm) * clora_cdiv(N, r.bn);
        for (int s = 1; s <= max_split && s <= 16; ++s) {
            if (s > 1 && ksteps / s < 4) break;
            const int kps = clora_cdiv(ksteps, s);
            const int real_s = clora_cdiv(ksteps, kps);
            const long blocks = tiles * real_s;
            const long rounds = (blocks + 256L * tc.conc - 1) / (256L * tc.conc);
            double t = (double)rounds * (kps * tc.t_k + 3.0e-6);
            if (real_s > 1) t += (double)M * N * (8.0 * real_s + 2.0) / 6.0e12 + 4.0e-6;
            if (t < best) { best = t; tile = c; splits = real_s; }
        }
    }
}
}

extern "C" int clora_gemm_f16_ex(const clora_half* A, int lda, const clora_half* B, clora_half* C, int ldc, int M, int N,
                                 int K, const clora_conv_t* conv, const clora_epilogue_t* epi, int split_k, int tile_cfg,
                                 void* workspace, size_t workspace_bytes, void* stream) {
    if (!A || !B || (!C && !(epi && epi->geglu == 1)) || M <= 0 || N <= 0 || K <= 0 || (K & 7) || (N & 7) || (ldc & 7)) return CLORA_ERR_ARG;
    GemmArgs a;
    a.A = (const half_t*)A; a.B = (const half_t*)B; a.C = (half_t*)C; a.partial = nullptr;
    a.lda = lda; a.ldc = ldc; a.M = M; a.N = N; a.K = K;
    a.tiles_m = 0; a.n_major = 0; a.xg_s = a.xg_m = a.xg_n = 0;
    a.two_phase = g_opts[CLORA_OPT_EPI_TWO_PHASE];
    a.hoist_on = g_opts[CLORA_OPT_EPI_HOIST];
    if (conv && conv->enabled) {
        a.conv = *conv;
        if ((conv->Cin & 7) || K != conv->ksize * conv->ksize * conv->Cin) return CLORA_ERR_ARG;
        if (conv->kchunk < 0 || (conv->kchunk > 0 && ((conv->kchunk & 7) || conv->Cin % conv->kchunk))) return CLORA_ERR_ARG;
    } else {
        a.conv = clora_conv_t();
        a.conv.enabled = 0;
        if (lda & 7) return CLORA_ERR_ARG;
    }
    if (epi) a.epi = *epi; else a.epi = clora_epilogue_t();
    if (a.epi.ln_out && (!a.epi.ln_gamma || !a.epi.ln_beta || !clora_gemm_ln_fusable(M, N, K, tile_cfg, split_k) || a.epi.geglu ||
                         a.conv.enabled || ((uintptr_t)a.epi.ln_gamma & 15) || ((uintptr_t)a.epi.ln_beta & 15)))
        return CLORA_ERR_ARG;
    clora_deferred_t* const defer = a.epi.defer;
    a.epi.defer = nullptr;
    if (defer) {
        if (a.epi.geglu) return CLORA_ERR_ARG;
        defer->splits = 0;
        defer->partial = nullptr;
    }
    if (a.epi.lora_t && (a.epi.lora_r <= 0 || a.epi.lora_seg <= 0 || (a.epi.lora_seg & 15))) return CLORA_ERR_ARG;
    if (a.epi.rowadd && a.epi.rows_per_batch <= 0) return CLORA_ERR_ARG;
    if (a.epi.residual && (a.epi.ldr & 7)) return CLORA_ERR_ARG;
    if ((a.epi.residual_lo && !a.epi.residual) || ((a.epi.residual_lo || a.epi.c_lo) && (a.epi.geglu || !C || (ldc & 7))) || (a.epi.c_lo && defer))
        return CLORA_ERR_ARG;
    if (a.epi.geglu) {
        const int F = a.epi.geglu_f;
        if (a.epi.geglu < 0 || a.epi.geglu > 2 || F <= 0 || (F & 63) || a.epi.rowadd || a.epi.residual || a.epi.lora_t) return CLORA_ERR_ARG;
        if (a.epi.geglu == 1 && (N != 2 * F || !a.epi.geglu_y || (C && ldc < 2 * F))) return CLORA_ERR_ARG;
        if (a.epi.geglu == 2 && (N != F || !a.epi.geglu_h || !C || ldc < 2 * F)) return CLORA_ERR_ARG;
        if (split_k > 1) return CLORA_ERR_ARG;
        split_k = 1;
    }
    hipStream_t s = (hipStream_t)stream;
    if (tile_row(tile_cfg).family == CLORA_TILE_STRIP) {
        const int plan = (a.conv.enabled && split_k <= 1 && !defer && !a.epi.rowadd && !a.epi.residual && !a.epi.lora_t && !a.epi.geglu &&
                          !a.epi.ln_out && !a.epi.c_lo && C && (ldc & 3) == 0 && K == 9 * a.conv.Cin)
                             ? strip_plan(M, N, a.conv) : 0;
        if (plan) {
            StripArgs q;
            q.X = a.A; q.Wt = a.B; q.C = a.C; q.bias = a.epi.bias; q.N = N; q.ldc = ldc; q.H = a.conv.Hout; q.W = a.conv.Wout;
            q.nimg = M / (a.conv.Hout * a.conv.Wout); q.off = a.conv.off; q.kmul = a.conv.kmul;
            if (plan == 802) return launch_strip8<2, 128>(q, s);
            if (plan == 804) return launch_strip8<4, 128>(q, s);
            if (plan == 3202) return launch_strip<32, 2, 128>(q, s);
            if (plan == 3204) return launch_strip<32, 4, 128>(q, s);
            return launch_strip<64, 2, 128>(q, s);
        }
        tile_cfg = 0;
    }
    int tile = 0, splits = 1;
    const int ws_cap = workspace ? (int)(workspace_bytes / ((size_t)M * N * sizeof(float))) : 1;
    plan_gemm(M, N, K, split_k >= 1 ? 1 : (ws_cap < 1 ? 1 : ws_cap), tile, splits);
    if (split_k >= 1) {
        const int ksteps = clora_cdiv(K, 32);
        splits = split_k > ksteps ? ksteps : split_k;
    }
    if (a.epi.lora_dpack) {
        const clora_epilogue_t& e = a.epi;
        if (a.conv.enabled || !e.lora_t || e.lora_r != 4 || e.geglu || (e.lora_seg % 64) || (N % e.lora_seg) || (K & 63) || split_k > 1 ||
            (e.ldt & 3) || (e.lora_u_tr ? (e.ldu & 3) != 0 : e.ldu != 4) || N / e.lora_seg > 32 ||
            (e.lora_t_in && ((e.ldt_in & 3) || e.lora_t_in_rows < 0)))
            return CLORA_ERR_ARG;
        clora_gemm_fused_down_tile(M, e.lora_seg, tile_cfg, &tile_cfg);
        split_k = 1; splits = 1;
    }
    const clora_gemm_tile_t* row = &tile_row(tile_cfg > 0 ? tile_cfg : kTiles[tile].cfg);
    const bool dma = row->family != CLORA_TILE_V1;
    const clora_gemm_tile_t& patch = tile_row((N % 160 == 0) ? 76 : 72);
    if (tile_cfg == 0 && !a.epi.geglu && patch_eligible(a, patch)) {
        row = &patch;
        if (split_k == 0) {
            const long blocks = (long)clora_cdiv(M, patch.bm) * clora_cdiv(N, patch.bn);
            const int slabs = a.conv.Cin / 64;
            int want = (int)((256 + blocks - 1) / blocks);
            if (want > slabs) want = slabs;
            while (want > 1 && (!workspace || workspace_bytes < (size_t)want * M * N * sizeof(float))) --want;
            splits = want < 1 ? 1 : want;
        }
    }
    if (a.epi.geglu) {
        if (!dma) return CLORA_ERR_ARG;
        if (a.epi.geglu == 1 && !(row->caps & kG)) { if (tile_cfg > 0) return CLORA_ERR_ARG; row = &tile_row(1); }
    }
    if (is_patch_tile(*row)) {
        if (!patch_eligible(a, *row)) row = &tile_row(21);
        else {
            const int slabs = a.conv.Cin / 64;
            if (splits > slabs) splits = slabs;
            a.k_per_split = clora_cdiv(slabs, splits);
            splits = clora_cdiv(slabs, a.k_per_split);
            if (splits > 1) {
                if (!workspace || workspace_bytes < (size_t)splits * M * N * sizeof(float)) return CLORA_ERR_WORKSPACE;
                a.partial = (float*)workspace;
            }
            int rc;
            switch (row->tile_cfg) {
#define CASE_PATCH(cfg, BM, BN, WM, WN, NST, BK, FLAGS, caps) case cfg: rc = launch_patch<BM, BN, WM, WN, NST>(a, splits, s); break;
#define CASE_WPATCH(cfg, BM, BN, WM, WN, NST, BK, FLAGS, caps) case cfg: rc = launch_patch<BM, BN, WM, WN, NST, kPatchWide>(a, splits, s); break;
#define CASE_NONE(...)
                CLORA_GEMM_TILES(CASE_NONE, CASE_NONE, CASE_NONE, CASE_PATCH, CASE_WPATCH, CASE_NONE)
                default: return CLORA_ERR_ARG;
            }
            if (rc != CLORA_OK) return rc;
            if (splits > 1) rc = finish_or_defer(a, splits, defer, s);
            return rc;
        }
    }
    if (a.conv.enabled && row->family == CLORA_TILE_EIGHT_PHASE) row = &tile_row(58);
    const int bk = row->bk;
    a.k_per_split = clora_cdiv(clora_cdiv(K, bk), splits) * bk;
    splits = clora_cdiv(K, a.k_per_split);
    if (splits > 1) {
        if (!workspace || workspace_bytes < (size_t)splits * M * N * sizeof(float)) return CLORA_ERR_WORKSPACE;
        a.partial = (float*)workspace;
    }
    int rc;
    switch (row->tile_cfg) {
#define CASE_RING(cfg, BM, BN, WM, WN, NST, BK, FLAGS, caps) case cfg: rc = launch_gemm<BM, BN, WM, WN, NST, BK, FLAGS>(a, splits, s, true); break;
#define CASE_V1(cfg, BM, BN, WM, WN, NST, BK, FLAGS, caps) case cfg: rc = launch_gemm<BM, BN, WM, WN, NST, BK, FLAGS>(a, splits, s, false); break;
#define CASE_EIGHT(cfg, ...) case cfg: rc = launch_gemm_8p(a, splits, s); break;
        CLORA_GEMM_TILES(CASE_RING, CASE_V1, CASE_EIGHT, CASE_NONE, CASE_NONE, CASE_NONE)
        CLORA_GEMM_PROBE_TILES(CASE_RING)
        default: return CLORA_ERR_ARG;
    }
    if (rc != CLORA_OK) return rc;
    if (splits > 1) rc = finish_or_defer(a, splits, defer, s);
    return rc;
}

extern "C" int clora_gemm_ln_fusable(int M, int N, int K, int tile_cfg, int split_k) {
    (void)K;
    const clora_gemm_tile_t& r = tile_row(tile_cfg);
    return M > 0 && (r.caps & kL) && N == r.bn && split_k == 1 ? 1 : 0;
}

extern "C" int clora_gemm_tile_info(int tile_cfg, clora_gemm_tile_t* out) {
    const clora_gemm_tile_t& r = tile_row(tile_cfg);
    if (!out || &r == &kNoTile) return CLORA_ERR_ARG;
    *out = r;
    return CLORA_OK;
}

extern "C" int clora_gemm_tile_at(int index, clora_gemm_tile_t* out) {
    if (!out || index < 0 || index >= kNumTileRows) return CLORA_ERR_ARG;
    *out = kTileRows[index];
    return CLORA_OK;
}

extern "C" int clora_gemm_fused_down_tile(int M, int lora_seg, int tile_cfg, int* out) {
    if (!out || M <= 0 || lora_seg <= 0) return CLORA_ERR_ARG;
    const clora_gemm_tile_t& r = tile_row(tile_cfg);
    if ((r.caps & kD) && lora_seg % r.bn == 0) *out = tile_cfg;
    else if (lora_seg % tile_row(55).bn == 0) *out = M >= 32768 ? 54 : 55;
    else *out = 43;
    return CLORA_OK;
}

extern "C" int clora_finish_deferred(const clora_deferred_t* d, void* stream) {
    if (!d || !d->partial || !d->C || d->splits <= 1 || d->M <= 0 || d->N <= 0 || (d->N & 7) || (d->ldc & 7)) return CLORA_ERR_ARG;
    GemmArgs a = GemmArgs();
    a.partial = const_cast<float*>(d->partial); a.C = (half_t*)d->C; a.ldc = d->ldc; a.M = d->M; a.N = d->N; a.epi = d->epi;
    a.epi.defer = nullptr;
    return finish_or_defer(a, d->splits, nullptr, (hipStream_t)stream);
}

int clora_option(int id) { return (id >= 0 && id < CLORA_OPT_COUNT) ? g_opts[id] : 0; }

extern "C" int clora_set_option(const char* name, int value) {
    if (!name) return CLORA_ERR_ARG;
    struct Opt { const char* name; int id, lo, hi; };
    static const Opt kOpts[] = {{"tile_order", CLORA_OPT_TILE_ORDER, 0, 3}, {"ln_rows", CLORA_OPT_LN_ROWS, 0, 1},
                                {"attn_fwd_waves", CLORA_OPT_ATTN_FWD_WAVES, 0, 16}, {"attn_bwd_waves", CLORA_OPT_ATTN_BWD_WAVES, 0, 8},
                                {"gn_blocks", CLORA_OPT_GN_BLOCKS, 64, 1 << 16}, {"epi_two_phase", CLORA_OPT_EPI_TWO_PHASE, 0, 1},
                                {"lora_down_mode", CLORA_OPT_LORA_DOWN_MODE, 0, 2}, {"gn_unroll", CLORA_OPT_GN_UNROLL, 0, 1},
                                {"epi_hoist", CLORA_OPT_EPI_HOIST, 0, 1}, {"gn_resident", CLORA_OPT_GN_RESIDENT, 0, 1},
                                {"defer_max_rows", CLORA_OPT_DEFER_MAX_ROWS, 0, 16}, {"wgrad_patch", CLORA_OPT_WGRAD_PATCH, 0, 8192}, {"strip_blocks", CLORA_OPT_STRIP_BLOCKS, 64, 16384},
                                {"gn_team", CLORA_OPT_GN_TEAM, 0, 4}};
    for (const Opt& o : kOpts)
        if (!strcmp(name, o.name)) {
            if (value < o.lo || value > o.hi) return CLORA_ERR_ARG;
            if ((o.id == CLORA_OPT_ATTN_FWD_WAVES && value != 0 && value != 4 && value != 6 && value != 8 && value != 16) ||
                (o.id == CLORA_OPT_ATTN_BWD_WAVES && value != 0 && value != 4 && value != 8)) return CLORA_ERR_ARG;
            g_opts[o.id] = value;
            return CLORA_OK;
        }
    return CLORA_ERR_ARG;
}

extern "C" int clora_conv_strip_eligible(int M, int N, const clora_conv_t* conv) {
    return (conv && strip_plan(M, N, *conv)) ? 1 : 0;
}

extern "C" int clora_conv_patch_eligible(int M, const clora_conv_t* conv, int tile_cfg) {
    const clora_gemm_tile_t& r = tile_row(tile_cfg);
    if (!conv || !is_patch_tile(r)) return 0;
    GemmArgs a;
    a.M = M; a.conv = *conv;
    return patch_eligible(a, r) ? 1 : 0;
}

extern "C" int clora_gemm_f16(const clora_half* A, int lda, const clora_half* B, clora_half* C, int ldc, int M, int N,
                              int K, const clora_conv_t* conv, const clora_epilogue_t* epi, int split_k,
                              void* workspace, size_t workspace_bytes, void* stream) {
    return clora_gemm_f16_ex(A, lda, B, C, ldc, M, N, K, conv, epi, split_k, 0, workspace, workspace_bytes, stream);
}

__global__ __launch_bounds__(256) void conv_wgrad_unpack_kernel(float* stage, float* stage_b, float* gw, float* gb, int Co, int Ci,
                                                                int taps, int Cip) {
    const int nw = Co * taps * Cip;
    for (int i = blockIdx.x * 256 + threadIdx.x; i < nw + (gb ? Co : 0); i += gridDim.x * 256) {
        if (i < nw) {
            const int ci = i % Cip, tap = (i / Cip) % taps, co = i / (Cip * taps);
            const float v = stage[i];
            stage[i] = 0.f;
            if (ci < Ci) gw[((size_t)co * Ci + ci) * taps + tap] += v;
        } else {
            const int co = i - nw;
            gb[co] += stage_b[co];
            stage_b[co] = 0.f;
        }
    }
}

extern "C" int clora_conv_wgrad_unpack_f32(float* stage, float* stage_b, float* grad_w, float* grad_b, int Co, int Ci, int ksize,
                                           int Cip, void* stream) {
    if (!stage || !grad_w || Co <= 0 || Ci <= 0 || Cip < Ci || (ksize != 1 && ksize != 3) || ((grad_b == nullptr) != (stage_b == nullptr)))
        return CLORA_ERR_ARG;
    const int taps = ksize * ksize;
    const long total = (long)Co * taps * Cip + (grad_b ? Co : 0);
    int blocks = (int)((total + 255) / 256);
    if (blocks > 2048) blocks = 2048;
    hipLaunchKernelGGL(conv_wgrad_unpack_kernel, dim3(blocks), dim3(256), 0, (hipStream_t)stream, stage, stage_b, grad_w, grad_b,
                       Co, Ci, taps, Cip);
    return clora_check_launch();
}

extern "C" int clora_conv_weight_pack_f32(const float* w, int Co, int Ci, int ksize, int Cip, int Cop, clora_half* fwd,
                                          clora_half* dgrad, void* stream) {
    if (!w || !fwd || Co <= 0 || Ci <= 0 || (ksize != 1 && ksize != 3) || Cip < Ci || (Cip & 7) || (dgrad && (Cop < Co || (Cop & 7))))
        return CLORA_ERR_ARG;
    const int taps = ksize * ksize;
    const long total = (long)Co * taps * Cip + (dgrad ? (long)Cip * taps * Cop : 0);
    int blocks = (int)((total + 255) / 256);
    if (blocks > 2048) blocks = 2048;
    hipLaunchKernelGGL(conv_weight_pack_kernel, dim3(blocks), dim3(256), 0, (hipStream_t)stream, w, Co, Ci, taps, Cip, Cop,
                       (half_t*)fwd, (half_t*)dgrad);
    return clora_check_launch();
}

extern "C" int clora_conv_wgrad_f16(const clora_half* dY, int ldy, const clora_half* X, int ldx, float* dW, float* db,
                                    int M, int N, int K, const clora_conv_t* conv, int oihw_ci, void* stream) {
    if (!dY || !X || !dW || M <= 0 || N <= 0 || K <= 0 || (K & 7) || (N & 7) || (ldy & 7) || oihw_ci < 0) return CLORA_ERR_ARG;
    WgradArgs a;
    a.dY = (const half_t*)dY; a.X = (const half_t*)X; a.dW = dW; a.db = db;
    a.ldy = ldy; a.ldx = ldx; a.M = M; a.N = N; a.K = K; a.oihw_ci = oihw_ci;
    if (conv && conv->enabled) {
        a.conv = *conv;
        if ((conv->Cin & 7) || K != conv->ksize * conv->ksize * conv->Cin || conv->kchunk != 0) return CLORA_ERR_ARG;
    } else {
        a.conv = clora_conv_t();
// ... 40 lines not shown
```

### controllora_amd/kernels.py

```python
from __future__ import annotations

import ctypes as C
import os
from typing import Optional, Tuple

import torch

from . import capi
from .capi import ConvDesc, Epilogue, ptr

f16, f32 = torch.float16, torch.float32


class KernelProfiler:

    def __init__(self, detail=False):
        self.detail = detail
        self.records = []

    def summary(self):
        torch.cuda.synchronize()
        agg = {}
        for name, e0, e1, fl, by in self.records:
            a = agg.setdefault(name, dict(calls=0, ms=0.0, flops=0.0, bytes=0.0))
            a["calls"] += 1
            a["ms"] += e0.elapsed_time(e1)
            a["flops"] += fl
            a["bytes"] += by
        return agg


PROFILER: Optional[KernelProfiler] = None


_PENDING = {}
_pending_task = [None]
FUSE_LN = os.environ.get("CLORA_FUSE_LN", "1") != "0"
DEFER_FINISH = os.environ.get("CLORA_DEFER_FINISH", "1") != "0"


class LayerNormSlot:

    def __init__(self, gamma, beta, eps):
        self.params, self.out = (gamma, beta, eps), None


def flush_pending():
    while _PENDING:
        _, (d, keep) = _PENDING.popitem()
        capi.lib().call("clora_finish_deferred", C.byref(d), capi.stream())


def take_pending(t: torch.Tensor):
    hit = _PENDING.pop(t.data_ptr(), None) if _PENDING else None
    if _PENDING:
        flush_pending()
    return hit if hit is not None else (None, None)


def _call(name, *args, flops=0.0, nbytes=0.0, tag=None):
    if _PENDING:
        flush_pending()
    if PROFILER is None:
        capi.lib().call(name, *args, capi.stream())
        return
    e0, e1 = torch.cuda.Event(enable_timing=True), torch.cuda.Event(enable_timing=True)
    e0.record()
    capi.lib().call(name, *args, capi.stream())
    e1.record()
    PROFILER.records.append((name if not (tag and PROFILER.detail) else f"{name}[{tag}]", e0, e1, float(flops), float(nbytes)))


def _c2(t: torch.Tensor) -> torch.Tensor:
    assert t.is_contiguous(), "kernel operands must be contiguous"
    return t.reshape(-1, t.shape[-1])


def conv_fwd_desc(Hin, Win, Cin, ksize=3, stride=1, pad=1, upsample=False, asym_pad=False, kchunk=0) -> Tuple[ConvDesc, int, int]:
    if upsample:
        Hout, Wout = 2 * Hin, 2 * Win
        return ConvDesc(1, Hin, Win, Cin, Hout, Wout, ksize, 1, 1, -pad, 2 * Hin, 2 * Win, 1, 0, kchunk), Hout, Wout
    if asym_pad:
        Hout, Wout = (Hin + 1 - ksize) // stride + 1, (Win + 1 - ksize) // stride + 1
        return ConvDesc(1, Hin, Win, Cin, Hout, Wout, ksize, stride, 1, 0, Hin, Win, 0, 0, kchunk), Hout, Wout
    Hout, Wout = (Hin + 2 * pad - ksize) // stride + 1, (Win + 2 * pad - ksize) // stride + 1
    return ConvDesc(1, Hin, Win, Cin, Hout, Wout, ksize, stride, 1, -pad, Hin, Win, 0, 0, kchunk), Hout, Wout


def conv_dgrad_desc(Hout, Wout, Cout, Hin, Win, ksize=3, stride=1, pad=1, asym_pad=False, kchunk=0) -> ConvDesc:
    p = 0 if asym_pad else pad
    if stride == 1:
        return ConvDesc(1, Hout, Wout, Cout, Hin, Win, ksize, 1, -1, p, Hout, Wout, 0, 0, kchunk)
    assert stride == 2
    return ConvDesc(1, Hout, Wout, Cout, Hin, Win, ksize, 1, -1, p, 2 * Hout, 2 * Wout, 1, 1, kchunk)


_ws_cache = {}


def workspace(nbytes: int, device) -> torch.Tensor:
    key = str(device)
    w = _ws_cache.get(key)
    if w is None or w.numel() < nbytes:
        floor = GEMM_WS_BYTES if torch.device(device).type == "cuda" else (1 << 20)
        if w is not None:
            _ws_retired.append(w)
        w = torch.empty(max(nbytes, floor), dtype=torch.uint8, device=device)
        _ws_cache[key] = w
    return w


_ws_retired = []
CONV_STRIP = os.environ.get("CLORA_CONV_STRIP", "1") != "0"
GEMM_WS_BYTES = 256 << 20


def gemm_tiles() -> dict:
    return capi.lib().tiles()


def _tile_has(tile_cfg: int, cap: int) -> bool:
    r = gemm_tiles().get(tile_cfg)
    return r is not None and bool(r.caps & cap)


def fused_down_tile(M: int, lora_seg: int, tile_cfg: int) -> int:
    out = C.c_int()
    capi.lib().call("clora_gemm_fused_down_tile", M, lora_seg, tile_cfg, C.byref(out))
    return out.value



_TUNING = None


def tuning_key(M, N, K, conv) -> str:
    if conv is None:
        return f"{M}x{N}x{K}"
    return f"{M}x{N}x{K}:c{conv.ksize}m{conv.mul}k{conv.kmul}s{conv.shift}e{conv.need_even}h{conv.Hin}"


def tuned_entry(M, N, K, conv):
    global _TUNING
    if _TUNING is None:
        import json
        path = os.environ.get("CLORA_GEMM_TUNING_FILE") or os.path.join(os.path.dirname(os.path.abspath(__file__)), "gemm_tuning_gfx950.json")
        use = os.path.exists(path) and os.environ.get("CLORA_GEMM_TUNING", "1") != "0"
        _TUNING = json.load(open(path))["table"] if use else {}
    return _TUNING.get(tuning_key(M, N, K, conv))


def _tuned_fused(M, N, K):
    tuned_entry(M, N, K, None)
    return _TUNING.get(f"{M}x{N}x{K}:x")


def gemm(A: torch.Tensor, Bw: torch.Tensor, M: int, N: int, K: int, *, lda: Optional[int] = None,
         conv: Optional[ConvDesc] = None, bias=None, rowadd=None, rows_per_batch=0, residual=None,
         lora_t=None, lora_u=None, lora_seg=0, lora_scale=1.0, lora_u_tr=False, lora_r=None,
         out: Optional[torch.Tensor] = None,
         split_k: int = 0, tile_cfg: int = 0, _tuned: bool = True,
         geglu: int = 0, geglu_h: Optional[torch.Tensor] = None, geglu_y: Optional[torch.Tensor] = None,
         geglu_keep_h: bool = True, lora_dpack: Optional[torch.Tensor] = None, lora_t_in: Optional[torch.Tensor] = None,
         lora_t_in_mask: int = 0, lora_t_in_rows: int = 0, defer: bool = False, ln=None, trunk: bool = False) -> torch.Tensor:
    assert A.dtype == f16 and Bw.dtype == f16 and Bw.shape == (N, K) and Bw.is_contiguous()
    e = Epilogue()
    if geglu == 1:
        F_ = N // 2
        C_ = torch.empty((M, N), dtype=f16, device=A.device) if geglu_keep_h else None
        y = geglu_y if geglu_y is not None else torch.empty((M, F_), dtype=f16, device=A.device)
        e.geglu, e.geglu_f, e.geglu_y = 1, F_, ptr(y, f16)
    elif geglu == 2:
        assert geglu_h is not None and geglu_h.shape == (M, 2 * N) and geglu_h.is_contiguous()
        C_ = out if out is not None else torch.empty((M, 2 * N), dtype=f16, device=A.device)
        e.geglu, e.geglu_f, e.geglu_h = 2, N, ptr(geglu_h, f16)
    else:
        C_ = out if out is not None else torch.empty((M, N), dtype=f16, device=A.device)
    assert C_ is None or (C_.dtype == f16 and C_.stride(-1) == 1)
    ldc = (C_.stride(0) if C_.dim() == 2 else N) if C_ is not None else N
    if bias is not None:
        assert bias.dtype == f32 and bias.numel() == N
        e.bias = ptr(bias)
    if rowadd is not None:
        assert rowadd.dtype == f16 and rowadd.dim() == 2 and rowadd.shape[1] == N and rowadd.stride(1) == 1 and rowadd.stride(0) % 8 == 0
        e.rowadd, e.rows_per_batch, e.ld_rowadd = ptr(rowadd), rows_per_batch, rowadd.stride(0)
    if residual is not None:
        assert residual.dtype == f16 and residual.stride(-1) == 1
        e.residual, e.ldr = ptr(residual), (residual.stride(0) if residual.dim() == 2 else N)
    c_lo = trunk_hit = None
    want_lo_out = not _TRUNK_NO_OUT[0]
    if _TRUNK_LO_ON[0] and not geglu and C_ is not None and C_.dim() == 2 and (residual is not None or (trunk and want_lo_out)):
        if residual is not None:
            hit = _TRUNK_LO.get(residual.data_ptr()) if _TRUNK_NORMS[0] else _TRUNK_LO.pop(residual.data_ptr(), None)
            if hit is not None and hit[0].numel() == residual.numel() and (residual.stride(0) if residual.dim() == 2 else N) == e.ldr:
                e.residual_lo = ptr(hit[1], f16)
                _trunk_keep[:] = [hit]
                trunk_hit = hit
        if want_lo_out:
            c_lo = torch.empty_strided(C_.shape, C_.stride(), dtype=f16, device=A.device)
            e.c_lo = ptr(c_lo)
            defer = False
    if lora_t is not None:
        assert lora_t.dtype == f32 and lora_u.dtype == f32 and lora_t.stride(1) == 1 and lora_u.stride(1) == 1
        e.lora_t, e.ldt, e.lora_u, e.ldu, e.lora_u_tr = ptr(lora_t), lora_t.stride(0), ptr(lora_u), lora_u.stride(0), int(lora_u_tr)
        e.lora_r = lora_r if lora_r is not None else (lora_u.shape[0] if lora_u_tr else lora_u.shape[1])
        e.lora_seg, e.lora_scale = (lora_seg or N), float(lora_scale)
    if lora_dpack is not None:
        assert lora_t is not None and lora_dpack.dtype == f16 and lora_dpack.is_contiguous() and lora_dpack.shape == (N // e.lora_seg * 8, K)
        e.lora_dpack = ptr(lora_dpack)
        if lora_t_in is not None:
            assert lora_t_in.dtype == f32 and lora_t_in.stride(1) == 1
            e.lora_t_in, e.ldt_in, e.lora_t_in_rows, e.lora_t_in_mask = ptr(lora_t_in), lora_t_in.stride(0), int(lora_t_in_rows), int(lora_t_in_mask)
        split_k = 1
    if (CONV_STRIP and conv is not None and split_k == 0 and tile_cfg == 0 and not geglu and rowadd is None and residual is None
            and lora_t is None and not defer and ln is None and capi.lib().cdll.clora_conv_strip_eligible(M, N, C.byref(conv))):
        tile_cfg, split_k = 61, 1
    if _tuned and split_k == 0 and tile_cfg == 0:
        hit = tuned_entry(M, N, K, conv)
        if hit is not None:
            tile_cfg, split_k = hit
    if geglu:
        split_k = 1
        if geglu == 1 and not _tile_has(tile_cfg, capi.TILE_CAP_GEGLU):
            tile_cfg = 0
    ws = workspace(GEMM_WS_BYTES if split_k == 0 else max(split_k, 1) * M * N * 4, A.device) if split_k != 1 else None
    if (ln is not None and ln.out is None and FUSE_LN and not geglu and conv is None and C_ is not None and C_.is_contiguous()
            and not (_TRUNK_NORMS[0] and c_lo is not None)):
        tc = tile_cfg
        if lora_dpack is not None and not _tile_has(tc, capi.TILE_CAP_LN):
            tc = fused_down_tile(M, e.lora_seg, 0)
        if capi.lib().cdll.clora_gemm_ln_fusable(M, N, K, tc, split_k):
            g_, b_, eps_ = ln.params
            assert g_.dtype == f32 and b_.dtype == f32 and g_.numel() == N and b_.numel() == N
            tile_cfg = tc
            ln.out = torch.empty((M, N), dtype=f16, device=A.device)
            e.ln_gamma, e.ln_beta, e.ln_out, e.ln_eps = ptr(g_), ptr(b_), ptr(ln.out), float(eps_)
    d = None
    if defer and DEFER_FINISH and split_k != 1 and not geglu and PROFILER is None and C_ is not None and C_.is_contiguous():
        d = capi.Deferred()
        e.defer = C.addressof(d)
    _call("clora_gemm_f16_ex", ptr(A), lda if lda is not None else K, ptr(Bw), ptr(C_) if C_ is not None else None, ldc, M, N, K,
          C.byref(conv) if conv is not None else None, C.byref(e), split_k, tile_cfg,
          ptr(ws) if ws is not None else None, ws.numel() if ws is not None else 0,
          flops=2.0 * M * N * K, nbytes=2.0 * (A.numel() + N * K + M * N),
          tag=f"{M}x{N}x{K}{'conv' if conv is not None else ''}")
    if d is not None and d.splits > 1:
        _PENDING[C_.data_ptr()] = (d, (C_, bias, rowadd, residual, lora_t, lora_u, ws, trunk_hit))
        task = _graph_task_id()
        if task >= 0 and _pending_task[0] != task:
            _pending_task[0] = task
            torch.autograd.Variable._execution_engine.queue_callback(flush_pending)
    if c_lo is not None:
        _TRUNK_LO[C_.data_ptr()] = (C_, c_lo)
    if geglu == 1:
        return y, C_
    return C_


_TRUNK_LO = {}
_trunk_keep = []
_TRUNK_LO_ON = [False]
_TRUNK_NORMS = [False]
TRUNK_LO_MODE = os.environ.get("CLORA_TRUNK_LO", "infer")


class TrunkLo:

    def __init__(self, enabled: bool, norms: bool = False):
        self.enabled = bool(enabled)
        self.norms = self.enabled and bool(norms)

    def __enter__(self):
        self.prev, self.prev_norms = _TRUNK_LO_ON[0], _TRUNK_NORMS[0]
        if self.enabled and not self.prev:
            _TRUNK_LO.clear(); _trunk_keep.clear()
        _TRUNK_LO_ON[0] = self.enabled or self.prev
        _TRUNK_NORMS[0] = self.norms or self.prev_norms
        return self

    def __exit__(self, *exc):
        _TRUNK_LO_ON[0], _TRUNK_NORMS[0] = self.prev, self.prev_norms
        if not self.prev:
            _TRUNK_LO.clear(); _trunk_keep.clear()
        return False


def trunk_lo_of(x: torch.Tensor, *also) -> Optional[torch.Tensor]:
    if not (_TRUNK_NORMS[0] and _TRUNK_LO) or torch.is_grad_enabled() or x.requires_grad or any(t.requires_grad for t in also):
        return None
    hit = _TRUNK_LO.get(x.data_ptr())
    if hit is None or hit[0].numel() != x.numel() or not hit[0].is_contiguous() or not x.is_contiguous():
        return None
    return hit[1].view(x.shape)


_TRUNK_NO_OUT = [False]


class TrunkNoOut:

    def __init__(self, cond: bool = True, norm_reads: bool = False):
        self.cond = bool(cond) and not (norm_reads and _TRUNK_NORMS[0])

    def __enter__(self):
        self.prev = _TRUNK_NO_OUT[0]
        _TRUNK_NO_OUT[0] = self.cond or self.prev
        return self

    def __exit__(self, *exc):
        _TRUNK_NO_OUT[0] = self.prev
        return False


def trunk_lo_wanted() -> bool:
    return TRUNK_LO_MODE == "always" or (TRUNK_LO_MODE in ("infer", "norms") and not torch.is_grad_enabled())


def trunk_norms_wanted() -> bool:
    return TRUNK_LO_MODE == "norms" and not torch.is_grad_enabled()


def conv_patch_eligible(M: int, conv: ConvDesc, tile_cfg: int) -> bool:
    return bool(capi.lib().cdll.clora_conv_patch_eligible(M, C.byref(conv), tile_cfg))


TILE_ORDERS = {"m": 0, "n": 1, "auto": 2, "grid": 3}
DEFAULT_TILE_ORDER = "grid"


def set_option(name: str, value: int) -> None:
    capi.lib().call("clora_set_option", name.encode(), int(value))


def set_tile_order(mode: str) -> None:
    set_option("tile_order", TILE_ORDERS[mode])


def conv_wgrad(dY: torch.Tensor, X: torch.Tensor, M: int, N: int, K: int, conv: Optional[ConvDesc],
               ldx: Optional[int] = None, with_bias: bool = False):
    buf = torch.zeros(N * K + (N if with_bias else 0), dtype=f32, device=dY.device)
    dW, db = buf[:N * K].view(N, K), (buf[N * K:] if with_bias else None)
    _call("clora_conv_wgrad_f16", ptr(dY, f16), N, ptr(X, f16), ldx if ldx is not None else K, ptr(dW), ptr(db), M, N, K,
          C.byref(conv) if conv is not None else None, 0, flops=2.0 * M * N * K)
    return (dW, db) if with_bias else dW


def conv_wgrad_into(dY: torch.Tensor, X: torch.Tensor, M: int, N: int, K: int, conv: Optional[ConvDesc],
                    weight_grad: torch.Tensor, bias_grad: Optional[torch.Tensor]):
    assert weight_grad.dtype == f32 and weight_grad.is_contiguous() and weight_grad.shape[0] == N
    _call("clora_conv_wgrad_f16", ptr(dY, f16), N, ptr(X, f16), K, ptr(weight_grad), ptr(bias_grad, f32) if bias_grad is not None else None,
          M, N, K, C.byref(conv) if conv is not None else None, weight_grad.shape[1], flops=2.0 * M * N * K)


def conv_wgrad_staged(dY, X, M, N, K, conv, stage: torch.Tensor, weight_grad: torch.Tensor, bias_grad: Optional[torch.Tensor], Cip: int):
    assert stage.dtype == f32 and stage.numel() == N * K + N and weight_grad.dtype == f32 and weight_grad.is_contiguous()
    sw, sb = stage[:N * K], stage[N * K:]
    _call("clora_conv_wgrad_f16", ptr(dY, f16), N, ptr(X, f16), K, ptr(sw), ptr(sb), M, N, K,
          C.byref(conv) if conv is not None else None, 0, flops=2.0 * M * N * K)
    if bias_grad is not None and conv_unpack_defer(conv_unpack_job(stage, weight_grad, bias_grad, Cip), stage, weight_grad, bias_grad):
        return
    Co, Ci, k, _ = weight_grad.shape
    _call("clora_conv_wgrad_unpack_f32", ptr(sw), ptr(sb) if bias_grad is not None else None, ptr(weight_grad),
          ptr(bias_grad, f32) if bias_grad is not None else None, Co, Ci, k, Cip)
    if bias_grad is None:
        sb.zero_()


def conv_weight_pack(weight: torch.Tensor, Cip: int, need_dgrad: bool, out=None):
    Co, Ci, k, _ = weight.shape
    Cop = (Co + 7) // 8 * 8
    if out is not None:
        fwd, dgrad = out
    else:
        fwd = torch.empty((Co, k * k * Cip), dtype=f16, device=weight.device)
        dgrad = torch.empty((Cip, k * k * Cop), dtype=f16, device=weight.device) if need_dgrad else None
    _call("clora_conv_weight_pack_f32", ptr(weight, f32), Co, Ci, k, Cip, Cop, ptr(fwd), ptr(dgrad) if dgrad is not None else None)
    return fwd, dgrad


def conv_pack_job(weight: torch.Tensor, Cip: int, fwd: torch.Tensor, dgrad: Optional[torch.Tensor]):
    Co, Ci, k, _ = weight.shape
    assert weight.dtype == f32 and weight.is_contiguous() and fwd.dtype == f16 and fwd.numel() == Co * k * k * Cip
    return capi.ConvPackJob(ptr(weight, f32), ptr(fwd), ptr(dgrad) if dgrad is not None else None, Co, Ci, k, Cip, (Co + 7) // 8 * 8, 0)


def conv_weight_pack_multi(jobs):
    for i in range(0, len(jobs), capi.CONV_MAX_JOBS):
        chunk = jobs[i:i + capi.CONV_MAX_JOBS]
        arr = (capi.ConvPackJob * len(chunk))(*chunk)
        _call("clora_conv_weight_pack_multi_f32", arr, len(chunk))


def conv_unpack_job(stage: torch.Tensor, weight_grad: torch.Tensor, bias_grad: Optional[torch.Tensor], Cip: int):
    Co, Ci, k, _ = weight_grad.shape
    nw = Co * k * k * Cip
    assert stage.dtype == f32 and stage.numel() == nw + Co and weight_grad.dtype == f32 and weight_grad.is_contiguous()
    sw, sb = stage[:nw], stage[nw:]
    return capi.ConvUnpackJob(ptr(sw), ptr(sb) if bias_grad is not None else None, ptr(weight_grad),
                              ptr(bias_grad, f32) if bias_grad is not None else None, Co, Ci, k, Cip)


def conv_wgrad_unpack_multi(jobs):
    for i in range(0, len(jobs), capi.CONV_MAX_JOBS):
        chunk = jobs[i:i + capi.CONV_MAX_JOBS]
        arr = (capi.ConvUnpackJob * len(chunk))(*chunk)
        _call("clora_conv_wgrad_unpack_multi_f32", arr, len(chunk))


def softmax_rows(x: torch.Tensor, scale: float = 1.0, out: Optional[torch.Tensor] = None) -> torch.Tensor:
    assert x.dim() == 2 and x.stride(1) == 1
    y = out if out is not None else torch.empty_like(x)
    assert y.stride(0) == x.stride(0)
    _call("clora_softmax_rows_f16", ptr(x, f16), ptr(y, f16), x.shape[0], x.shape[1], x.stride(0), float(scale),
          nbytes=4.0 * x.numel())
    return y


def attn_max_head_dim(backward: bool = False) -> int:
    return int(capi.lib().cdll.clora_attn_max_head_dim(1 if backward else 0))


def attn_fwd(q, k, v, B, H, Nq, Nk, D, scale, out=None):
    o = out if out is not None else torch.empty((B * Nq, H * D), dtype=f16, device=q.device)
    lse = torch.empty((B, H, Nq), dtype=f32, device=q.device)
    _call("clora_attn_fwd_f16", ptr(q, f16), q.stride(0), ptr(k, f16), k.stride(0), ptr(v, f16), v.stride(0),
          ptr(o), o.stride(0), ptr(lse), B, H, Nq, Nk, D, float(scale), flops=4.0 * B * H * Nq * Nk * D)
    return o, lse


def attn_fwd_causal(q, k, v, B, H, N, D, scale, out=None):
    o = out if out is not None else torch.empty((B * N, H * D), dtype=f16, device=q.device)
    _call("clora_attn_fwd_causal_f16", ptr(q, f16), q.stride(0), ptr(k, f16), k.stride(0), ptr(v, f16), v.stride(0),
          ptr(o), o.stride(0), B, H, N, D, float(scale), flops=2.0 * B * H * N * N * D)
    return o


def attn_bwd(q, k, v, o, dO, lse, B, H, Nq, Nk, D, scale, dq, dk, dv):
    delta = torch.empty((B, H, Nq), dtype=f32, device=q.device)
    ws = workspace(16 * 2 * B * Nk * H * D * 4, q.device) if Nk <= 1024 else None
    _call("clora_attn_bwd_f16", ptr(q, f16), q.stride(0), ptr(k, f16), k.stride(0), ptr(v, f16), v.stride(0),
          ptr(o, f16), o.stride(0), ptr(dO, f16), dO.stride(0), ptr(lse, f32), ptr(delta),
          ptr(dq, f16), dq.stride(0), ptr(dk, f16), dk.stride(0), ptr(dv, f16), dv.stride(0),
          B, H, Nq, Nk, D, float(scale), ptr(ws) if ws is not None else None, ws.numel() if ws is not None else 0,
          flops=10.0 * B * H * Nq * Nk * D)
    return dq, dk, dv


_gn_team = {}


def _dev_key(device) -> str:
    d = torch.device(device)
    if d.type == "cuda" and d.index is None:
        d = torch.device("cuda", torch.cuda.current_device())
    return str(d)


def gn_team_state(device) -> torch.Tensor:
    key = _dev_key(device)
    st = _gn_team.get(key)
    if st is None:
        st = torch.zeros(capi.lib().cdll.clora_groupnorm_team_state_bytes(), dtype=torch.uint8, device=device)
        _gn_team[key] = st
    return st


def gn_team_errors(device) -> int:
    st = _gn_team.get(_dev_key(device))
    return 0 if st is None else int(st[:4].view(torch.int32).item())


def _gn_ws(B, HW, Cc, G, device, bwd, params):
    n = capi.lib().cdll.clora_groupnorm_workspace_bytes(B, HW, Cc, G, int(bwd), int(params))
    if n == 0:
        raise capi.CloraError(f"unsupported GroupNorm shape B={B} HW={HW} C={Cc} G={G}")
    return workspace(n, device)


def groupnorm_fwd(x, gamma, beta, G, eps, silu, x2=None, x_lo=None, x2_lo=None):
    B, HW, Ca = x.shape
    Cc = Ca + (x2.shape[-1] if x2 is not None else 0)
    src, _keep = take_pending(x)
    y = torch.empty((B, HW, Cc), dtype=f16, device=x.device)
    stats = torch.empty((B, G, 2), dtype=f32, device=x.device)
    xcat = torch.empty((B, HW, Cc), dtype=f16, device=x.device) if x2 is not None else None
    if src is not None and x2 is not None:
        capi.lib().call("clora_finish_deferred", C.byref(src), capi.stream())
        src = None
    ws = _gn_ws(B, HW, Cc, G, x.device, False, False)
    team = gn_team_state(x.device)
    entry, lo_args = "clora_groupnorm_fwd_f16_team", ()
    if x_lo is not None or x2_lo is not None:
        assert x_lo is None or (x_lo.shape == x.shape and x_lo.is_contiguous())
        assert x2_lo is None or (x2 is not None and x2_lo.shape == x2.shape and x2_lo.is_contiguous())
        assert x.is_contiguous() and (x2 is None or x2.is_contiguous())
        entry = "clora_groupnorm_fwd_f16_lo"
        lo_args = (ptr(x_lo, f16) if x_lo is not None else None, ptr(x2_lo, f16) if x2_lo is not None else None)
    _call(entry, ptr(x, f16), ptr(x2, f16) if x2 is not None else None, Ca if x2 is not None else 0,
          C.byref(src) if src is not None else None, ptr(xcat) if xcat is not None else None, ptr(y), ptr(gamma, f32), ptr(beta, f32),
          ptr(stats), B, HW, Cc, G, float(eps), int(silu), ptr(team), team.numel(), ptr(ws), ws.numel(), *lo_args)
    return (y, stats, xcat) if x2 is not None else (y, stats)


def groupnorm_bwd(x, dy, gamma, beta, stats, G, silu, want_param_grads=False, grads_into=None, dres=None, split_at=0):
    B, HW, Cc = x.shape
    dy_src, _keep = take_pending(dy)
    if split_at:
        dx = torch.empty((B, HW, split_at), dtype=f16, device=x.device)
        dx2 = torch.empty((B, HW, Cc - split_at), dtype=f16, device=x.device)
    else:
        dx, dx2 = torch.empty_like(x), None
    dg = db = None
    if grads_into is not None:
        dg, db = grads_into
        want_param_grads = True
    elif want_param_grads:
        dg = torch.empty(Cc, dtype=f32, device=x.device)
        db = torch.empty(Cc, dtype=f32, device=x.device)
    ws = _gn_ws(B, HW, Cc, G, x.device, True, want_param_grads)
    assert dres is None or (dres.shape == x.shape and dres.is_contiguous())
    team = gn_team_state(x.device)
    _call("clora_groupnorm_bwd_f16_team", ptr(x, f16), ptr(dy, f16), C.byref(dy_src) if dy_src is not None else None,
          ptr(dres, f16) if dres is not None else None, ptr(dx), ptr(dx2) if dx2 is not None else None, int(split_at),
          ptr(gamma, f32), ptr(beta, f32), ptr(stats, f32),
          ptr(dg, f32) if dg is not None else None, ptr(db, f32) if db is not None else None, B, HW, Cc, G, int(silu),
          int(grads_into is not None), ptr(team), team.numel(), ptr(ws), ws.numel())
    if split_at:
        dx = (dx, dx2)
    return (dx, None, None) if grads_into is not None else (dx, dg, db)


def layernorm_fwd(x, gamma, beta, eps, x_lo=None):
    x2 = _c2(x)
    y = torch.empty_like(x)
    if x_lo is not None:
        assert x_lo.shape == x.shape and x_lo.is_contiguous()
        _call("clora_layernorm_fwd_f16_lo", ptr(x2, f16), ptr(y), ptr(gamma, f32), ptr(beta, f32), x2.shape[0], x2.shape[1], float(eps),
              ptr(x_lo, f16))
        return y
    _call("clora_layernorm_fwd_f16", ptr(x2, f16), ptr(y), ptr(gamma, f32), ptr(beta, f32), x2.shape[0], x2.shape[1], float(eps))
    return y


def layernorm_bwd(x, dy, gamma, eps, dres=None):
    x2 = _c2(x)
    dx = torch.empty_like(x)
    dy_src, _keep = take_pending(dy)
    _call("clora_layernorm_bwd_f16_ex", ptr(x2, f16), ptr(_c2(dy), f16), C.byref(dy_src) if dy_src is not None else None,
          ptr(_c2(dres), f16) if dres is not None else None, ptr(dx), ptr(gamma, f32), x2.shape[0], x2.shape[1], float(eps))
    return dx


def geglu_fwd(h):
    h2 = _c2(h)
    M, F2 = h2.shape
    y = torch.empty(h.shape[:-1] + (F2 // 2,), dtype=f16, device=h.device)
    _call("clora_geglu_fwd_f16", ptr(h2, f16), ptr(y), M, F2 // 2)
    return y


def geglu_bwd(h, dy):
    h2 = _c2(h)
    M, F2 = h2.shape
    dh = torch.empty_like(h)
    _call("clora_geglu_bwd_f16", ptr(h2, f16), ptr(_c2(dy), f16), ptr(dh), M, F2 // 2)
    return dh


# ... 508 lines not shown
```

### controllora_amd/ops.py

```python
from __future__ import annotations

from typing import List, Optional, Sequence, Tuple

import torch

from . import kernels as K

f16, f32 = torch.float16, torch.float32


class LinearPack:

    def __init__(self, weight: torch.Tensor, bias: Optional[torch.Tensor], pad_n_to: int = 8):
        w = weight.detach().reshape(weight.shape[0], -1).to(f16)
        N, Kd = w.shape
        if Kd % 8:
            w = torch.cat([w, w.new_zeros(N, 8 - Kd % 8)], 1)
            Kd = w.shape[1]
        Np = (N + pad_n_to - 1) // pad_n_to * pad_n_to
        if Np != N:
            w = torch.cat([w, w.new_zeros(Np - N, Kd)], 0)
        self.N, self.K, self.N_logical = Np, Kd, N
        self.w = w.contiguous()
        self.wt = w.t().contiguous()
        self.bias = None
        if bias is not None:
            b = bias.detach().to(f32)
            self.bias = torch.cat([b, b.new_zeros(Np - N)]) if Np != N else b.contiguous()


class FoldedPack:

    def __init__(self, base: LinearPack):
        self.base = base
        self.N, self.K, self.N_logical, self.bias = base.N, base.K, base.N_logical, base.bias
        self.w = torch.empty_like(base.w)
        self.wt = torch.empty_like(base.wt)

    def jobs(self, segments):
        assert sorted((r0, r0 + n) for r0, n, _ in segments)[0][0] == 0 and sum(n for _, n, _ in segments) == self.N
        return [K.lora_fold_job(self.base.w[r0:r0 + n], self.w[r0:r0 + n], self.wt[:, r0:r0 + n], members) for r0, n, members in segments]


class GegluPack:

    def __init__(self, weight: torch.Tensor, bias: Optional[torch.Tensor]):
        w = weight.detach().to(f16)
        N, Kd = w.shape
        F_ = N // 2
        assert N % 128 == 0 and Kd % 8 == 0
        idx = torch.arange(N, device=w.device).reshape(N // 128, 2, 64)
        src = torch.where(torch.arange(2, device=w.device).reshape(1, 2, 1) == 0,
                          (idx[:, :1] // 128) * 64 + idx[:, :1] % 64,
                          F_ + (idx[:, 1:] // 128) * 64 + idx[:, 1:] % 64).reshape(-1)
        self.N, self.K, self.F = N, Kd, F_
        self.w = w[src].contiguous()
        self.wt = w.t().contiguous()
        self.bias = bias.detach().to(f32)[src].contiguous() if bias is not None else None


import os as _os
KCHUNK = int(_os.environ.get("CLORA_KCHUNK", "64"))


def conv_k_order(w_taps_ci: torch.Tensor, kchunk: int) -> torch.Tensor:
    rows, taps, Cc = w_taps_ci.shape
    if kchunk == 0:
        return w_taps_ci.reshape(rows, taps * Cc).contiguous()
    return w_taps_ci.reshape(rows, taps, Cc // kchunk, kchunk).permute(0, 2, 1, 3).reshape(rows, taps * Cc).contiguous()


class ConvPack:

    def __init__(self, weight: torch.Tensor, bias: Optional[torch.Tensor], stride=1, pad=1, upsample=False,
                 asym_pad=False, need_dgrad=True):
        w = weight.detach().to(f16)
        Co, Ci, kh, kw = w.shape
        assert kh == 3 and kw == 3
        Cip, Cop = (Ci + 7) // 8 * 8, (Co + 7) // 8 * 8
        wp = w.new_zeros(Cop, 3, 3, Cip)
        wp[:Co, :, :, :Ci] = w.permute(0, 2, 3, 1)
        self.Ci, self.Co, self.Cip, self.Cop = Ci, Co, Cip, Cop
        self.kchunk = KCHUNK if (KCHUNK and Cip % KCHUNK == 0) else 0
        self.kchunk_d = KCHUNK if (KCHUNK and Cop % KCHUNK == 0) else 0
        self.w = conv_k_order(wp.reshape(Cop, 9, Cip), self.kchunk)
        self.wd = None
        if need_dgrad:
            wd = w.new_zeros(Cip, 3, 3, Cop)
            wd[:Ci, :, :, :Co] = w.permute(1, 2, 3, 0)
            self.wd = conv_k_order(wd.reshape(Cip, 9, Cop), self.kchunk_d)
        self.bias = None
        if bias is not None:
            b = bias.detach().to(f32)
            self.bias = torch.cat([b, b.new_zeros(Cop - Co)]) if Cop != Co else b.contiguous()
        self.stride, self.pad, self.upsample, self.asym_pad = stride, pad, upsample, asym_pad


class _FrozenLinearFn(torch.autograd.Function):
    @staticmethod
    def forward(ctx, x, pack: LinearPack, residual, rowadd, rows_per_batch, defer_out=False, defer_dx=False, ln=None, trunk=False):
        M = x.shape[0]
        y = K.gemm(x, pack.w, M, pack.N, pack.K, bias=pack.bias, residual=residual, rowadd=rowadd,
                   rows_per_batch=rows_per_batch, defer=defer_out and ln is None, ln=ln, trunk=trunk)
        ctx.pack, ctx.has_res, ctx.defer_dx = pack, residual is not None, defer_dx
        return y

    @staticmethod
    def backward(ctx, dy):
        dy = dy.contiguous()
        p = ctx.pack
        dx = K.gemm(dy, p.wt, dy.shape[0], p.K, p.N, defer=ctx.defer_dx) if ctx.needs_input_grad[0] else None
        return dx, None, (dy if ctx.has_res and ctx.needs_input_grad[2] else None), None, None, None, None, None, None


def frozen_linear(x, pack: LinearPack, residual=None, rowadd=None, rows_per_batch=0, defer_out=False, defer_dx=False, ln=None, trunk=False):
    return _FrozenLinearFn.apply(x, pack, residual, rowadd, rows_per_batch, defer_out, defer_dx, ln, trunk)


class _FrozenConvFn(torch.autograd.Function):
    @staticmethod
    def forward(ctx, x, pack: ConvPack, B, H, W, residual, rowadd, defer_out=False, defer_dx=False):
        cd, Ho, Wo = K.conv_fwd_desc(H, W, pack.Cip, 3, pack.stride, pack.pad, pack.upsample, pack.asym_pad, pack.kchunk)
        M = B * Ho * Wo
        y = K.gemm(x, pack.w, M, pack.Cop, 9 * pack.Cip, conv=cd, bias=pack.bias, residual=residual, rowadd=rowadd,
                   rows_per_batch=Ho * Wo, defer=defer_out)
        ctx.pack, ctx.dims, ctx.has_res, ctx.defer_dx = pack, (B, H, W, Ho, Wo), residual is not None, defer_dx
        return y

    @staticmethod
    def backward(ctx, dy):
        dy = dy.contiguous()
        p = ctx.pack
        B, H, W, Ho, Wo = ctx.dims
        dx = None
        if ctx.needs_input_grad[0]:
            Hi, Wi = (2 * H, 2 * W) if p.upsample else (H, W)
            cdd = K.conv_dgrad_desc(Ho, Wo, p.Cop, Hi, Wi, 3, p.stride, p.pad, p.asym_pad, p.kchunk_d)
            dx = K.gemm(dy, p.wd, B * Hi * Wi, p.Cip, 9 * p.Cop, conv=cdd, defer=ctx.defer_dx and not p.upsample)
            if p.upsample:
                dx = K.pool2x2_sum(dx, B, H, W, p.Cip).reshape(B * H * W, p.Cip)
        return dx, None, None, None, None, (dy if ctx.has_res and ctx.needs_input_grad[5] else None), None, None, None


def frozen_conv3x3(x, pack: ConvPack, B, H, W, residual=None, rowadd=None, defer_out=False, defer_dx=False):
    return _FrozenConvFn.apply(x, pack, B, H, W, residual, rowadd, defer_out, defer_dx)


class _GroupNormFn(torch.autograd.Function):

    @staticmethod
    def forward(ctx, x, gamma, beta, G, eps, silu, fork):
        y, stats = K.groupnorm_fwd(x, gamma, beta, G, eps, silu, x_lo=K.trunk_lo_of(x))
        ctx.save_for_backward(x, gamma, beta, stats)
        ctx.cfg = (G, silu)
        ctx.affine = (gamma, beta)
        return (y, x) if fork else y

    @staticmethod
    def backward(ctx, dy, dres=None):
        x, gamma, beta, stats = ctx.saved_tensors
        G, silu = ctx.cfg
        into = None
        if ctx.needs_input_grad[1]:
            g_, b_ = ctx.affine
            into = (_grad_buffer(g_), _grad_buffer(b_))
        dx, _, _ = K.groupnorm_bwd(x, dy.contiguous(), gamma, beta, stats, G, silu, grads_into=into,
                                   dres=dres.contiguous().view_as(x) if dres is not None else None)
        return dx, None, None, None, None, None, None


def group_norm(x, gamma, beta, G, eps, silu):
    return _GroupNormFn.apply(x, gamma, beta, G, eps, silu, False)


class _GroupNormCatFn(torch.autograd.Function):

    @staticmethod
    def forward(ctx, a, b, gamma, beta, G, eps, silu):
        y, stats, xcat = K.groupnorm_fwd(a, gamma, beta, G, eps, silu, x2=b, x_lo=K.trunk_lo_of(a, b), x2_lo=K.trunk_lo_of(b, a))
        ctx.save_for_backward(xcat, gamma, beta, stats)
        ctx.cfg = (G, silu, a.shape[-1])
        return y, xcat

    @staticmethod
    def backward(ctx, dy, dres=None):
        xcat, gamma, beta, stats = ctx.saved_tensors
        G, silu, Ca = ctx.cfg
        (da, db), _, _ = K.groupnorm_bwd(xcat, dy.contiguous(), gamma, beta, stats, G, silu,
                                         dres=dres.contiguous().view_as(xcat) if dres is not None else None, split_at=Ca)
        return da, db, None, None, None, None, None


def group_norm_cat(a, b, gamma, beta, G, eps, silu):
    return _GroupNormCatFn.apply(a, b, gamma, beta, G, eps, silu)


def group_norm_fork(x, gamma, beta, G, eps, silu):
    return _GroupNormFn.apply(x, gamma, beta, G, eps, silu, True)


class _LayerNormFn(torch.autograd.Function):

    @staticmethod
    def forward(ctx, x, gamma, beta, eps, fork, pre=None):
        ctx.save_for_backward(x, gamma)
        ctx.eps = eps
        y = pre.view_as(x) if pre is not None else K.layernorm_fwd(x, gamma, beta, eps, x_lo=K.trunk_lo_of(x))
        return (y, x) if fork else y

    @staticmethod
    def backward(ctx, dy, dres=None):
        x, gamma = ctx.saved_tensors
        dx = K.layernorm_bwd(x, dy.contiguous(), gamma, ctx.eps, dres=dres.contiguous().view_as(x) if dres is not None else None)
        return dx, None, None, None, None, None


def layer_norm(x, gamma, beta, eps=1e-5, pre=None):
    return _LayerNormFn.apply(x, gamma, beta, eps, False, pre)


def layer_norm_fork(x, gamma, beta, eps=1e-5, pre=None):
    return _LayerNormFn.apply(x, gamma, beta, eps, True, pre)


class _GegluFn(torch.autograd.Function):
    @staticmethod
    def forward(ctx, h):
        ctx.save_for_backward(h)
        return K.geglu_fwd(h)

    @staticmethod
    def backward(ctx, dy):
        (h,) = ctx.saved_tensors
        return K.geglu_bwd(h, dy.contiguous())


def geglu(h):
    return _GegluFn.apply(h)


class _FeedForwardFn(torch.autograd.Function):

    @staticmethod
    def forward(ctx, x, pack1: "GegluPack", pack2: LinearPack, residual, defer_dx=False):
        ctx.defer_dx = defer_dx
        M = x.shape[0]
        need = ctx.needs_input_grad[0]
        y, h = K.gemm(x, pack1.w, M, pack1.N, pack1.K, bias=pack1.bias, geglu=1, geglu_keep_h=need)
        out = K.gemm(y, pack2.w, M, pack2.N, pack2.K, bias=pack2.bias, residual=residual)
        ctx.packs, ctx.has_res = (pack1, pack2), residual is not None
        if need:
            ctx.save_for_backward(h)
        return out

    @staticmethod
    def backward(ctx, dout):
        dout = dout.contiguous()
        (h,) = ctx.saved_tensors
        p1, p2 = ctx.packs
        M = dout.shape[0]
        dx = None
        if ctx.needs_input_grad[0]:
            dh = K.gemm(dout, p2.wt, M, p2.K, p2.N, geglu=2, geglu_h=h)
            dx = K.gemm(dh, p1.wt, M, p1.K, p1.N, defer=ctx.defer_dx)
        return dx, None, None, (dout if ctx.has_res and ctx.needs_input_grad[3] else None), None


def feed_forward(x, pack1: "GegluPack", pack2: LinearPack, residual=None, defer_dx=False):
    return _FeedForwardFn.apply(x, pack1, pack2, residual, defer_dx)


class _AddFn(torch.autograd.Function):
    @staticmethod
    def forward(ctx, a, b):
        return K.add(a, b)

    @staticmethod
# ... 1121 lines not shown
```

### controllora_amd/unet.py

```python
from __future__ import annotations

import math
from types import SimpleNamespace
from typing import Dict, Optional

import torch
import torch.nn as nn

from . import kernels as K
from . import ops

f16, f32 = torch.float16, torch.float32

import os as _os
CAT_IN_PLACE = _os.environ.get("CLORA_CAT_IN_PLACE", "1") != "0"

SD15_CONFIG = dict(
    in_channels=4, out_channels=4, block_out_channels=(320, 640, 1280, 1280), layers_per_block=2,
    down_block_types=("CrossAttnDownBlock2D", "CrossAttnDownBlock2D", "CrossAttnDownBlock2D", "DownBlock2D"),
    up_block_types=("UpBlock2D", "CrossAttnUpBlock2D", "CrossAttnUpBlock2D", "CrossAttnUpBlock2D"),
    attention_head_dim=8, cross_attention_dim=768, norm_num_groups=32, norm_eps=1e-5)


def _frozen(t: torch.Tensor) -> nn.Parameter:
# ... 1 lines not shown


class _Packed(nn.Module):

    def __init__(self):
        super().__init__()
        self._pack = None
        self._pack_key = None

    def _key(self):
        return tuple((p.data_ptr(), p._version, str(p.device)) for p in self.parameters(recurse=False))

    def pack(self):
        k = self._key()
        if self._pack is None or self._pack_key != k:
            self._pack, self._pack_key = self._build(), k
        return self._pack


class Conv3x3(_Packed):
    def __init__(self, cin, cout, stride=1, pad=1, upsample=False, need_dgrad=True, asym_pad=False):
        super().__init__()
        self.weight = _frozen(torch.empty(cout, cin, 3, 3, dtype=f16))
        self.bias = _frozen(torch.empty(cout, dtype=f16))
        self.cfg = dict(stride=stride, pad=pad, upsample=upsample, need_dgrad=need_dgrad, asym_pad=asym_pad)

    def _build(self):
        return ops.ConvPack(self.weight, self.bias, **self.cfg)

    def forward(self, x, B, H, W, residual=None, rowadd=None, defer_out=False, defer_dx=False):
        return ops.frozen_conv3x3(x, self.pack(), B, H, W, residual, rowadd, defer_out, defer_dx)


class Conv1x1(_Packed):

    def __init__(self, cin, cout):
        super().__init__()
        self.weight = _frozen(torch.empty(cout, cin, 1, 1, dtype=f16))
        self.bias = _frozen(torch.empty(cout, dtype=f16))

    def _build(self):
        return ops.LinearPack(self.weight, self.bias)

    def forward(self, x, residual=None, defer_out=False, defer_dx=False, ln=None, trunk=False):
        return ops.frozen_linear(x, self.pack(), residual, defer_out=defer_out, defer_dx=defer_dx, ln=ln, trunk=trunk)


class Linear(_Packed):
    def __init__(self, cin, cout, bias=True):
        super().__init__()
        self.weight = _frozen(torch.empty(cout, cin, dtype=f16))
        self.bias = _frozen(torch.empty(cout, dtype=f16)) if bias else None

    def _build(self):
        return ops.LinearPack(self.weight, self.bias)

    def forward(self, x, residual=None):
        return ops.frozen_linear(x, self.pack(), residual)


class _Norm(_Packed):
    def __init__(self, c):
        super().__init__()
        self.weight = _frozen(torch.empty(c, dtype=f16))
        self.bias = _frozen(torch.empty(c, dtype=f16))

    def _build(self):
        return self.weight.detach().to(f32).contiguous(), self.bias.detach().to(f32).contiguous()


class GroupNorm(_Norm):
    def __init__(self, groups, c, eps):
        super().__init__(c)
        self.groups, self.eps = groups, eps

    def forward(self, x, silu):
        g, b = self.pack()
        return ops.group_norm(x, g, b, self.groups, self.eps, silu)

    def fork(self, x, silu):
        g, b = self.pack()
        return ops.group_norm_fork(x, g, b, self.groups, self.eps, silu)

    def fork_cat(self, x, skip, silu):
        g, b = self.pack()
        return ops.group_norm_cat(x, skip, g, b, self.groups, self.eps, silu)


class LayerNorm(_Norm):
    def forward(self, x, pre=None):
        g, b = self.pack()
        return ops.layer_norm(x, g, b, 1e-5, pre)

    def fork(self, x, pre=None):
        g, b = self.pack()
        return ops.layer_norm_fork(x, g, b, 1e-5, pre)

    def slot(self):
        g, b = self.pack()
        return K.LayerNormSlot(g, b, 1e-5)


class CrossAttnProcessor:

    def __call__(self, attn, hidden_states, encoder_hidden_states=None, attention_mask=None, residual=None):
        return attn.plain_attention(hidden_states, encoder_hidden_states, residual)


class CrossAttention(nn.Module):

    def __init__(self, query_dim, cross_attention_dim=None, heads=8, dim_head=64):
        super().__init__()
        inner = heads * dim_head
        self.is_cross = cross_attention_dim is not None
        ctx = cross_attention_dim if cross_attention_dim is not None else query_dim
        self.heads, self.dim_head, self.scale, self.inner_dim, self.query_dim = heads, dim_head, dim_head ** -0.5, inner, query_dim
        self.to_q = Linear(query_dim, inner, bias=False)
        self.to_k = Linear(ctx, inner, bias=False)
        self.to_v = Linear(ctx, inner, bias=False)
        self.to_out = nn.ModuleList([Linear(inner, query_dim), nn.Dropout(0.0)])
        self.processor = CrossAttnProcessor()
        self._fused = None
        self._fused_key = None

    def set_processor(self, processor):
        if isinstance(getattr(self, "processor", None), nn.Module) and not isinstance(processor, nn.Module):
            self._modules.pop("processor")
        self.processor = processor

    def prepare_attention_mask(self, attention_mask, target_length, batch_size=None):
        if attention_mask is not None:
            raise NotImplementedError("attention masks are never used on this path (SURVEY.md A2)")
        return None

    def fused_packs(self):
        key = tuple((m.weight.data_ptr(), m.weight._version) for m in (self.to_q, self.to_k, self.to_v))
        if self._fused is None or self._fused_key != key:
            if self.is_cross:
                self._fused = (ops.LinearPack(self.to_q.weight, None),
                               ops.LinearPack(torch.cat([self.to_k.weight, self.to_v.weight], 0), None))
            else:
                self._fused = (ops.LinearPack(torch.cat([self.to_q.weight, self.to_k.weight, self.to_v.weight], 0), None),)
            self._fused_key = key
        return self._fused

    def forward(self, hidden_states, encoder_hidden_states=None, attention_mask=None, residual=None, **kw):
        if residual is not None and getattr(self.processor, "fuses_residual", True) is False:
            out = self.processor(self, hidden_states, encoder_hidden_states=encoder_hidden_states,
                                 attention_mask=attention_mask, **kw)
            return ops.add(out.reshape(residual.shape), residual)
        return self.processor(self, hidden_states, encoder_hidden_states=encoder_hidden_states,
                              attention_mask=attention_mask, residual=residual, **kw)

    def attend(self, q_or_qkv, kv, B, N, Nk):
        if kv is None:
            return ops.attention_self(q_or_qkv, B, self.heads, N, self.dim_head, self.scale)
        return ops.attention_cross(q_or_qkv, kv, B, self.heads, N, Nk, self.dim_head, self.scale)

    def plain_attention(self, hidden_states, encoder_hidden_states=None, residual=None):
        B, N, C_ = hidden_states.shape
        h2 = hidden_states.reshape(B * N, C_)
        packs = self.fused_packs()
        if self.is_cross:
            e2 = encoder_hidden_states.reshape(-1, encoder_hidden_states.shape[-1])
            q = ops.frozen_linear(h2, packs[0])
            kv = ops.frozen_linear(e2, packs[1])
            a = self.attend(q, kv, B, N, encoder_hidden_states.shape[1])
        else:
            a = self.attend(ops.frozen_linear(h2, packs[0]), None, B, N, N)
        res2 = residual.reshape(B * N, C_) if residual is not None else None
        return self.to_out[0](a, res2).reshape(B, N, C_)


class _GegluLinear(Linear):

    def _build(self):
        return ops.GegluPack(self.weight, self.bias)


class GEGLU(nn.Module):
    def __init__(self, dim_in, dim_out):
        super().__init__()
        self.proj = _GegluLinear(dim_in, dim_out * 2)


class FeedForward(nn.Module):
    def __init__(self, dim, mult=4):
        super().__init__()
        self.net = nn.ModuleList([GEGLU(dim, dim * mult), nn.Dropout(0.0), Linear(dim * mult, dim)])

    def forward(self, x, residual, defer_dx=False):
        return ops.feed_forward(x, self.net[0].proj.pack(), self.net[2].pack(), residual, defer_dx)


class BasicTransformerBlock(nn.Module):
    def __init__(self, dim, heads, dim_head, cross_attention_dim):
        super().__init__()
        self.attn1 = CrossAttention(dim, None, heads, dim_head)
        self.ff = FeedForward(dim)
        self.attn2 = CrossAttention(dim, cross_attention_dim, heads, dim_head)
        self.norm1, self.norm2, self.norm3 = LayerNorm(dim), LayerNorm(dim), LayerNorm(dim)

    def forward(self, x, ehs, kw, pre_ln1=None, last=True):
        B, N, C_ = x.shape
        grad = torch.is_grad_enabled() and x.requires_grad
        n, xr = self.norm1.fork(x, pre_ln1) if grad else (self.norm1(x, pre_ln1), x)
        with ops.input_from_norm(), ops.next_layernorm(self.norm2.slot()) as s2:
            x = self.attn1(n, residual=xr, **kw)
        n, xr = self.norm2.fork(x, s2.out) if grad else (self.norm2(x, s2.out), x)
        with ops.input_from_norm(), ops.next_layernorm(self.norm3.slot()) as s3:
            x = self.attn2(n, encoder_hidden_states=ehs, residual=xr, **kw)
        n, xr = self.norm3.fork(x, s3.out) if grad else (self.norm3(x, s3.out), x)
        with K.TrunkNoOut(last):
            return self.ff(n.reshape(B * N, C_), xr.reshape(B * N, C_), defer_dx=grad).reshape(B, N, C_)


class Transformer2DModel(nn.Module):
    def __init__(self, heads, dim_head, in_channels, cross_attention_dim, groups):
        super().__init__()
        inner = heads * dim_head
        self.norm = GroupNorm(groups, in_channels, 1e-6)
        self.proj_in = Conv1x1(in_channels, inner)
        self.transformer_blocks = nn.ModuleList([BasicTransformerBlock(inner, heads, dim_head, cross_attention_dim)])
        self.proj_out = Conv1x1(inner, in_channels)

    def forward(self, x, ehs, kw, out_to_norm=False, trunk_out=True):
        B, N, C_ = x.shape
        grad = torch.is_grad_enabled() and x.requires_grad
        n, xr = self.norm.fork(x, False) if grad else (self.norm(x, False), x)
        s1 = self.transformer_blocks[0].norm1.slot()
        h = self.proj_in(n.reshape(B * N, C_), defer_dx=grad, ln=s1, trunk=True).reshape(B, N, -1)
        for i, blk in enumerate(self.transformer_blocks):
            h = blk(h, ehs, kw, pre_ln1=s1.out if i == 0 else None, last=i == len(self.transformer_blocks) - 1)
        with K.TrunkNoOut(not trunk_out, norm_reads=out_to_norm):
            return self.proj_out(h.reshape(B * N, -1), xr.reshape(B * N, C_), defer_out=out_to_norm).reshape(B, N, C_)


class ResnetBlock2D(nn.Module):
    def __init__(self, cin, cout, temb_c, groups, eps):
        super().__init__()
        self.norm1 = GroupNorm(groups, cin, eps)
        self.conv1 = Conv3x3(cin, cout)
        self.time_emb_proj = Linear(temb_c, cout)
        self.norm2 = GroupNorm(groups, cout, eps)
        self.conv2 = Conv3x3(cout, cout)
        self.conv_shortcut = Conv1x1(cin, cout) if cin != cout else None

    def forward(self, x, temb_act, H, W, temb_proj=None, skip=None, out_to_norm=False, trunk_out=True):
        B, N, _ = x.shape
        if temb_proj is not None:
            t = temb_proj
        else:
            with torch.no_grad():
                t = self.time_emb_proj(temb_act)
        grad = torch.is_grad_enabled() and (x.requires_grad or (skip is not None and skip.requires_grad))
        if skip is not None:
            n, xr = self.norm1.fork_cat(x, skip, True)
        else:
            n, xr = self.norm1.fork(x, True) if grad else (self.norm1(x, True), x)
        Cin = xr.shape[-1]
        h = self.conv1(n.reshape(B * N, Cin), B, H, W, rowadd=t, defer_out=True, defer_dx=grad)
        Cout = h.shape[1]
        h = self.norm2(h.reshape(B, N, Cout), True).reshape(B * N, Cout)
        x2 = xr.reshape(B * N, Cin)
        sc = self.conv_shortcut(x2, trunk=True) if self.conv_shortcut is not None else x2
        with K.TrunkNoOut(not trunk_out, norm_reads=out_to_norm):
            return self.conv2(h, B, H, W, residual=sc, defer_out=out_to_norm, defer_dx=grad).reshape(B, N, Cout)


class Downsample2D(nn.Module):
    def __init__(self, c):
        super().__init__()
        self.conv = Conv3x3(c, c, stride=2, pad=1)

    def forward(self, x, H, W, out_to_norm=False):
        B, N, C_ = x.shape
        return self.conv(x.reshape(B * N, C_), B, H, W, defer_out=out_to_norm).reshape(B, (H // 2) * (W // 2), C_)


class Upsample2D(nn.Module):
    def __init__(self, c):
        super().__init__()
        self.conv = Conv3x3(c, c, upsample=True)

    def forward(self, x, H, W, out_to_norm=False):
        B, N, C_ = x.shape
        return self.conv(x.reshape(B * N, C_), B, H, W, defer_out=out_to_norm).reshape(B, 4 * N, C_)


class CrossAttnDownBlock2D(nn.Module):
    has_attn = True

    def __init__(self, cin, cout, temb_c, layers, heads, ctx, groups, eps, add_down):
        super().__init__()
        self.resnets = nn.ModuleList([ResnetBlock2D(cin if i == 0 else cout, cout, temb_c, groups, eps) for i in range(layers)])
        self.attentions = nn.ModuleList([Transformer2DModel(heads, cout // heads, cout, ctx, groups) for _ in range(layers)])
        self.downsamplers = nn.ModuleList([Downsample2D(cout)]) if add_down else None


class DownBlock2D(nn.Module):
    has_attn = False

    def __init__(self, cin, cout, temb_c, layers, groups, eps, add_down):
        super().__init__()
        self.resnets = nn.ModuleList([ResnetBlock2D(cin if i == 0 else cout, cout, temb_c, groups, eps) for i in range(layers)])
        self.downsamplers = nn.ModuleList([Downsample2D(cout)]) if add_down else None


class UNetMidBlock2DCrossAttn(nn.Module):
    def __init__(self, c, temb_c, heads, ctx, groups, eps):
        super().__init__()
        self.attentions = nn.ModuleList([Transformer2DModel(heads, c // heads, c, ctx, groups)])
        self.resnets = nn.ModuleList([ResnetBlock2D(c, c, temb_c, groups, eps), ResnetBlock2D(c, c, temb_c, groups, eps)])


class _UpBase(nn.Module):
    def __init__(self, cin, prev, cout, temb_c, layers, groups, eps, add_up):
        super().__init__()
        rs = []
        for i in range(layers):
            skip = cin if i == layers - 1 else cout
            rin = prev if i == 0 else cout
            rs.append(ResnetBlock2D(rin + skip, cout, temb_c, groups, eps))
        self.resnets = nn.ModuleList(rs)
        self.upsamplers = nn.ModuleList([Upsample2D(cout)]) if add_up else None


class UpBlock2D(_UpBase):
    has_attn = False


class CrossAttnUpBlock2D(_UpBase):
    has_attn = True

    def __init__(self, cin, prev, cout, temb_c, layers, heads, ctx, groups, eps, add_up):
        super().__init__(cin, prev, cout, temb_c, layers, groups, eps, add_up)
        self.attentions = nn.ModuleList([Transformer2DModel(heads, cout // heads, cout, ctx, groups) for _ in range(layers)])


class TimestepEmbedding(nn.Module):
    def __init__(self, cin, ct):
        super().__init__()
        self.linear_1, self.linear_2 = Linear(cin, ct), Linear(ct, ct)


class UNetOutput:
# ... 198 lines not shown
```

### include/clora.h

```cpp
#ifndef CLORA_H
#define CLORA_H
#include <stddef.h>
#include <stdint.h>

#ifdef __cplusplus
extern "C" {
#endif

#define CLORA_OK 0
#define CLORA_ERR_ARG (-1)
#define CLORA_ERR_LAUNCH (-2)
#define CLORA_ERR_WORKSPACE (-3)

typedef uint16_t clora_half;

typedef struct {
    int enabled;
    int Hin, Win, Cin;
    int Hout, Wout;
    int ksize;
    int mul, kmul, off, lim_h, lim_w, shift, need_even;
    int kchunk;
} clora_conv_t;

struct clora_deferred;

typedef struct {
    const float* bias;
    const clora_half* rowadd;
    int rows_per_batch;
    int ld_rowadd;
    const clora_half* residual;
    int ldr;
    const float* lora_t;
    int ldt;
    const float* lora_u;
    int ldu;
    int lora_u_tr;
    int lora_r;
    int lora_seg;
    float lora_scale;
    int geglu;
    int geglu_f;
    const clora_half* geglu_h;
    clora_half* geglu_y;
    const clora_half* lora_dpack;
    const float* lora_t_in;
    int ldt_in, lora_t_in_rows;
    unsigned lora_t_in_mask;
    struct clora_deferred* defer;
    const float* ln_gamma;
    const float* ln_beta;
    clora_half* ln_out;
    float ln_eps;
    const clora_half* residual_lo;
    clora_half* c_lo;
} clora_epilogue_t;

typedef struct clora_deferred {
    const float* partial;
    int splits, M, N;
    clora_half* C;
    int ldc;
    clora_epilogue_t epi;
} clora_deferred_t;
int clora_gemm_ln_fusable(int M, int N, int K, int tile_cfg, int split_k);

enum { CLORA_TILE_RING = 0,
       CLORA_TILE_V1 = 1,
       CLORA_TILE_EIGHT_PHASE = 2,
       CLORA_TILE_PATCH = 3,
       CLORA_TILE_PATCH_WIDE = 4,
       CLORA_TILE_STRIP = 5 };
#define CLORA_TILE_CAP_GEGLU 1
#define CLORA_TILE_CAP_DPACK 2
#define CLORA_TILE_CAP_LN 4
#define CLORA_TILE_CAP_CONV 8
typedef struct {
    int tile_cfg, family;
    int bm, bn, wm, wn;
    int nst, bk, flags;
    int caps;
} clora_gemm_tile_t;
int clora_gemm_tile_info(int tile_cfg, clora_gemm_tile_t* out);
int clora_gemm_tile_at(int index, clora_gemm_tile_t* out);
int clora_gemm_fused_down_tile(int M, int lora_seg, int tile_cfg, int* out);
int clora_finish_deferred(const clora_deferred_t* d, void* stream);

typedef struct {
    const float* D;
    clora_half* out;
    int ldd, R, K, kmajor;
    float scale;
    int pad_;
} clora_lora_pack_job_t;
int clora_lora_pack_f16(const clora_lora_pack_job_t* table, int njobs, int max_k, void* stream);

int clora_gemm_f16(const clora_half* A, int lda, const clora_half* B, clora_half* C, int ldc,
                   int M, int N, int K, const clora_conv_t* conv, const clora_epilogue_t* epi,
                   int split_k, void* workspace, size_t workspace_bytes, void* stream);
int clora_gemm_f16_ex(const clora_half* A, int lda, const clora_half* B, clora_half* C, int ldc,
                      int M, int N, int K, const clora_conv_t* conv, const clora_epilogue_t* epi,
                      int split_k, int tile_cfg, void* workspace, size_t workspace_bytes, void* stream);

int clora_conv_patch_eligible(int M, const clora_conv_t* conv, int tile_cfg);

int clora_conv_strip_eligible(int M, int N, const clora_conv_t* conv);

int clora_set_option(const char* name, int value);

int clora_conv_wgrad_f16(const clora_half* dY, int ldy, const clora_half* X, int ldx, float* dW, float* db,
                         int M, int N, int K, const clora_conv_t* conv, int oihw_ci, void* stream);

int clora_conv_wgrad_unpack_f32(float* stage, float* stage_b, float* grad_w, float* grad_b, int Co, int Ci, int ksize,
                                int Cip, void* stream);

int clora_conv_weight_pack_f32(const float* w, int Co, int Ci, int ksize, int Cip, int Cop, clora_half* fwd,
                               clora_half* dgrad, void* stream);

#define CLORA_CONV_MAX_JOBS 32
typedef struct {
    const float* w;
    clora_half* fwd;
    clora_half* dgrad;
    int Co, Ci, ksize, Cip, Cop, pad_;
} clora_conv_pack_job_t;
int clora_conv_weight_pack_multi_f32(const clora_conv_pack_job_t* jobs, int njobs, void* stream);
typedef struct {
    float* stage;
    float* stage_b;
    float* grad_w;
    float* grad_b;
    int Co, Ci, ksize, Cip;
} clora_conv_unpack_job_t;
int clora_conv_wgrad_unpack_multi_f32(const clora_conv_unpack_job_t* jobs, int njobs, void* stream);

int clora_attn_fwd_f16(const clora_half* q, int ldq, const clora_half* k, int ldk, const clora_half* v, int ldv,
                       clora_half* o, int ldo, float* lse, int B, int H, int Nq, int Nk, int D, float scale,
                       void* stream);
int clora_attn_max_head_dim(int backward);
int clora_attn_fwd_causal_f16(const clora_half* q, int ldq, const clora_half* k, int ldk, const clora_half* v, int ldv,
                              clora_half* o, int ldo, int B, int H, int N, int D, float scale, void* stream);
int clora_attn_bwd_f16(const clora_half* q, int ldq, const clora_half* k, int ldk, const clora_half* v, int ldv,
                       const clora_half* o, int ldo, const clora_half* dO, int lddo, const float* lse,
                       float* delta, clora_half* dq, int lddq, clora_half* dk, int lddk, clora_half* dv, int lddv,
                       int B, int H, int Nq, int Nk, int D, float scale, void* workspace, size_t workspace_bytes,
                       void* stream);

int clora_groupnorm_fwd_f16(const clora_half* x, clora_half* y, const float* gamma, const float* beta, float* stats,
                            int B, int HW, int C, int G, float eps, int fuse_silu, void* workspace,
                            size_t workspace_bytes, void* stream);
size_t clora_groupnorm_workspace_bytes(int B, int HW, int C, int G, int backward, int param_grads);
int clora_groupnorm_bwd_f16(const clora_half* x, const clora_half* dy, const clora_half* dres, clora_half* dx, const float* gamma,
                            const float* beta, const float* stats, float* dgamma, float* dbeta, int B, int HW, int C,
                            int G, int fuse_silu, int accumulate_params, void* workspace, size_t workspace_bytes,
                            void* stream);

int clora_groupnorm_fwd_f16_ex(const clora_half* x, const clora_half* x2, int Ca, const clora_deferred_t* src, clora_half* xcopy,
                               clora_half* y, const float* gamma, const float* beta, float* stats, int B, int HW, int C, int G,
                               float eps, int fuse_silu, void* workspace, size_t workspace_bytes, void* stream);
int clora_groupnorm_bwd_f16_ex(const clora_half* x, const clora_half* dy, const clora_deferred_t* dy_src, const clora_half* dres,
                               clora_half* dx, clora_half* dx2, int Ca, const float* gamma, const float* beta, const float* stats,
                               float* dgamma, float* dbeta, int B, int HW, int C, int G, int fuse_silu, int accumulate_params,
                               void* workspace, size_t workspace_bytes, void* stream);

size_t clora_groupnorm_team_state_bytes(void);
int clora_groupnorm_fwd_f16_team(const clora_half* x, const clora_half* x2, int Ca, const clora_deferred_t* src, clora_half* xcopy,
                                 clora_half* y, const float* gamma, const float* beta, float* stats, int B, int HW, int C, int G,
                                 float eps, int fuse_silu, void* team_state, size_t team_state_bytes, void* workspace,
                                 size_t workspace_bytes, void* stream);
int clora_groupnorm_bwd_f16_team(const clora_half* x, const clora_half* dy, const clora_deferred_t* dy_src, const clora_half* dres,
                                 clora_half* dx, clora_half* dx2, int Ca, const float* gamma, const float* beta, const float* stats,
                                 float* dgamma, float* dbeta, int B, int HW, int C, int G, int fuse_silu, int accumulate_params,
                                 void* team_state, size_t team_state_bytes, void* workspace, size_t workspace_bytes, void* stream);

int clora_groupnorm_fwd_f16_lo(const clora_half* x, const clora_half* x2, int Ca, const clora_deferred_t* src, clora_half* xcopy,
                               clora_half* y, const float* gamma, const float* beta, float* stats, int B, int HW, int C, int G,
                               float eps, int fuse_silu, void* team_state, size_t team_state_bytes, void* workspace,
                               size_t workspace_bytes, const clora_half* x_lo, const clora_half* x2_lo, void* stream);
int clora_layernorm_fwd_f16_lo(const clora_half* x, clora_half* y, const float* gamma, const float* beta, int M, int C,
                               float eps, const clora_half* x_lo, void* stream);

int clora_softmax_rows_f16(const clora_half* x, clora_half* y, int rows, int cols, int ld, float scale, void* stream);

int clora_layernorm_fwd_f16(const clora_half* x, clora_half* y, const float* gamma, const float* beta, int M, int C,
                            float eps, void* stream);
int clora_layernorm_bwd_f16(const clora_half* x, const clora_half* dy, const clora_half* dres, clora_half* dx,
                            const float* gamma, int M, int C, float eps, void* stream);
int clora_layernorm_bwd_f16_ex(const clora_half* x, const clora_half* dy, const clora_deferred_t* dy_src, const clora_half* dres,
// ... 165 lines not shown
```

Before: 183.8 images/s.

## Fuse ResNet 1x1 shortcut into conv2 patch GEMM as extra K tail

Adds a tail phase to the 3x3 patch conv kernel. After the 9*slabs conv steps it streams extra K slabs from the block input (or the x/skip pair), so the 1x1 shortcut projection is accumulated into the same output tile. The shortcut GEMM launch and its intermediate trunk tensor go away, along with the residual read in the epilogue. When no gradient is needed, the concatenated skip tensor is no longer materialised. The cost is a more complex kernel and a new split-K plan over the combined steps, and the path is on by default through a new option.

```diff
diff --git a/controllora_amd/capi.py b/controllora_amd/capi.py
--- a/controllora_amd/capi.py
+++ b/controllora_amd/capi.py
@@ -22,6 +22,10 @@
     _fields_ = [(n, C.c_int) for n in (
         "enabled", "Hin", "Win", "Cin", "Hout", "Wout", "ksize", "mul", "kmul", "off", "lim_h", "lim_w", "shift",
         "need_even", "kchunk")]
+
+
+class ConvTail(C.Structure):
+    _fields_ = [("a", C.c_void_p), ("b", C.c_void_p), ("ca", C.c_int), ("cb", C.c_int), ("lda", C.c_int), ("ldb", C.c_int)]
 
 
 class Epilogue(C.Structure):
@@ -148,6 +152,8 @@
     "clora_gemm_f16": [_P, _I, _P, _P, _I, _I, _I, _I, C.POINTER(ConvDesc), C.POINTER(Epilogue), _I, _P, _Z, _P],
     "clora_gemm_f16_ex": [_P, _I, _P, _P, _I, _I, _I, _I, C.POINTER(ConvDesc), C.POINTER(Epilogue), _I, _I, _P, _Z, _P],
     "clora_conv_patch_eligible": [_I, C.POINTER(ConvDesc), _I],
+    "clora_conv3x3_tail_f16": [_P, _P, _P, _I, _I, _I, _I, C.POINTER(ConvDesc), C.POINTER(ConvTail), C.POINTER(Epilogue), _I, _I, _P, _Z, _P],
+    "clora_conv_tail_eligible": [_I, _I, C.POINTER(ConvDesc), _I, _I, _I],
     "clora_conv_strip_eligible": [_I, _I, C.POINTER(ConvDesc)],
     "clora_set_option": [C.c_char_p, _I],
     "clora_conv_wgrad_f16": [_P, _I, _P, _I, _P, _P, _I, _I, _I, C.POINTER(ConvDesc), _I, _P],
@@ -281,7 +287,7 @@
                     "CLORA_LORA_DOWN_MODE": ("lora_down_mode", None), "CLORA_GN_UNROLL": ("gn_unroll", None),
                     "CLORA_EPI_HOIST": ("epi_hoist", None), "CLORA_GN_RESIDENT": ("gn_resident", None),
                     "CLORA_DEFER_MAX_ROWS": ("defer_max_rows", None), "CLORA_WGRAD_PATCH": ("wgrad_patch", None), "CLORA_STRIP_BLOCKS": ("strip_blocks", None),
-                    "CLORA_GN_TEAM": ("gn_team", None)}
+                    "CLORA_GN_TEAM": ("gn_team", None), "CLORA_RESNET_FUSE_SHORTCUT": ("resnet_fuse_shortcut", None)}
 
     def _options_from_env(self):
         for var, (name, names) in self._ENV_OPTIONS.items():
diff --git a/controllora_amd/csrc/clora_common.h b/controllora_amd/csrc/clora_common.h
--- a/controllora_amd/csrc/clora_common.h
+++ b/controllora_amd/csrc/clora_common.h
@@ -116,7 +116,7 @@
     return v;
 }
 
-enum { CLORA_OPT_TILE_ORDER = 0, CLORA_OPT_LN_ROWS, CLORA_OPT_ATTN_FWD_WAVES, CLORA_OPT_ATTN_BWD_WAVES, CLORA_OPT_GN_BLOCKS, CLORA_OPT_EPI_TWO_PHASE, CLORA_OPT_LORA_DOWN_MODE, CLORA_OPT_GN_UNROLL, CLORA_OPT_EPI_HOIST, CLORA_OPT_GN_RESIDENT, CLORA_OPT_DEFER_MAX_ROWS, CLORA_OPT_WGRAD_PATCH, CLORA_OPT_STRIP_BLOCKS, CLORA_OPT_GN_TEAM, CLORA_OPT_COUNT };
+enum { CLORA_OPT_TILE_ORDER = 0, CLORA_OPT_LN_ROWS, CLORA_OPT_ATTN_FWD_WAVES, CLORA_OPT_ATTN_BWD_WAVES, CLORA_OPT_GN_BLOCKS, CLORA_OPT_EPI_TWO_PHASE, CLORA_OPT_LORA_DOWN_MODE, CLORA_OPT_GN_UNROLL, CLORA_OPT_EPI_HOIST, CLORA_OPT_GN_RESIDENT, CLORA_OPT_DEFER_MAX_ROWS, CLORA_OPT_WGRAD_PATCH, CLORA_OPT_STRIP_BLOCKS, CLORA_OPT_GN_TEAM, CLORA_OPT_RESNET_FUSE_SHORTCUT, CLORA_OPT_COUNT };
 __attribute__((visibility("hidden"))) int clora_option(int id);
 static inline int clora_xcd_policy() { return clora_option(CLORA_OPT_TILE_ORDER); }
 static inline int clora_ln_rows() { return clora_option(CLORA_OPT_LN_ROWS); }
diff --git a/controllora_amd/csrc/clora_ew.hip b/controllora_amd/csrc/clora_ew.hip
--- a/controllora_amd/csrc/clora_ew.hip
+++ b/controllora_amd/csrc/clora_ew.hip
@@ -442,7 +442,9 @@
     return clora_check_launch();
 }
 extern "C" int clora_abi_version(void) { return CLORA_ABI_VERSION; }
-extern "C" const char* clora_build_info(void) { return "libclora gfx950 (v_mfma_f32_16x16x32_f16), ABI 2"; }
+#define CLORA_STR_(x) #x
+#define CLORA_STR(x) CLORA_STR_(x)
+extern "C" const char* clora_build_info(void) { return "libclora gfx950 (v_mfma_f32_16x16x32_f16), ABI " CLORA_STR(CLORA_ABI_VERSION); }
 
 namespace {
 struct ConvPackJobs { clora_conv_pack_job_t j[CLORA_CONV_MAX_JOBS]; };
diff --git a/controllora_amd/csrc/clora_gemm.hip b/controllora_amd/csrc/clora_gemm.hip
--- a/controllora_amd/csrc/clora_gemm.hip
+++ b/controllora_amd/csrc/clora_gemm.hip
@@ -19,6 +19,9 @@
     int xg_s, xg_m, xg_n;
     clora_conv_t conv;
     clora_epilogue_t epi;
+    const half_t* a2a;
+    const half_t* a2b;
+    int c2a, c2b, ld2a, ld2b;
 };
 
 template <int BM, int BN, int WM, int WN>
@@ -985,7 +988,7 @@
 };
 constexpr int kPatchWide = 392;
 
-template <int BM, int BN, int WM, int WN, int NST, int MAXPP_ = 0>
+template <int BM, int BN, int WM, int WN, int NST, int MAXPP_ = 0, bool TAIL = false>
 __global__ __launch_bounds__(WM * WN * 64, 1) void conv3x3_patch_kernel(GemmArgs p) {
     constexpr int NT = WM * WN * 64, NW = WM * WN, BK = 64;
     constexpr int FM = BM / WM / 16, FN = BN / WN / 16;
@@ -1030,8 +1033,11 @@
     const int b0 = m0 / HW, y0 = (m0 - b0 * HW) / W, x0 = W > BM ? (m0 - b0 * HW - y0 * W) : 0;
     const int nb = p.M / HW;
     const int slabs = C / 64;
-    const int cs_beg = split * p.k_per_split, cs_end_ = cs_beg + p.k_per_split;
+    const int w0 = split * p.k_per_split, w1 = w0 + p.k_per_split;
+    const int cs_beg = TAIL ? ((w0 + 8) / 9 < slabs ? (w0 + 8) / 9 : slabs) : w0, cs_end_ = TAIL ? (w1 + 8) / 9 : w1;
     const int cs_end = cs_end_ < slabs ? cs_end_ : slabs;
+    const int tsl_all = TAIL ? (p.c2a + p.c2b) / 64 : 0, tw0 = w0 - 9 * slabs, tw1 = w1 - 9 * slabs;
+    const int ts_beg = tw0 < 0 ? 0 : (tw0 < tsl_all ? tw0 : tsl_all), ts_end = tw1 < 0 ? 0 : (tw1 < tsl_all ? tw1 : tsl_all);
 
     int poff[PA_IN];
 #pragma unroll
@@ -1066,7 +1072,8 @@
         b_ok[i] = ibe < B_NI && n < p.N;
         b_base[i] = (size_t)n * p.K + kc * 8;
     }
-    const int kbeg = cs_beg * 576, kend = cs_end * 576;
+    const int tsl = ts_end - ts_beg;
+    const int kbeg = cs_beg * 576 + ts_beg * 64, kend = cs_end * 576 + ts_end * 64;
     int kq = kbeg;
     auto issue_b = [&](int buf) {
         half_t* Bs = Bring + buf * BST;
@@ -1136,6 +1143,64 @@
                 for (int i = 0; i < FM; ++i)
 #pragma unroll
                     for (int j = 0; j < FN; ++j) acc[i][j] = mfma16(af[ks][i], bf[ks][j], acc[i][j]);
+        }
+    }
+    if constexpr (TAIL) {
+        constexpr int A_IN = BM / 8 / NW, AST = BM * 64;
+        static_assert(BM % (8 * NW) == 0 && 3 * AST <= 2 * PATCH, "the tail's three A stages live in the patch pair");
+        if (tsl > 0) {
+            int a2row[A_IN];
+#pragma unroll
+            for (int j = 0; j < A_IN; ++j) {
+                const int m = m0 + (w + NW * j) * 8 + lrow;
+                a2row[j] = m < p.M ? m : -1;
+            }
+            const int sa = p.c2a / 64;
+            auto issue_a2 = [&](int sl, int q) {
+                const int s = ts_beg + sl;
+                const bool ina = s < sa;
+                const half_t* base = (ina ? p.a2a + s * 64 : p.a2b + (s - sa) * 64) + kc * 8;
+                const size_t ld = ina ? p.ld2a : p.ld2b;
+#pragma unroll
+                for (int j = 0; j < A_IN; ++j) {
+                    const half_t* src = (sl < tsl && a2row[j] >= 0) ? base + (size_t)a2row[j] * ld : zero_page;
+                    CLORA_GLDS16(src, Pb + q * AST + (w + NW * j) * 512);
+                }
+            };
+            CLORA_RAW_BARRIER();
+            issue_a2(0, 0);
+            issue_a2(1, 1);
+            CLORA_WAIT_VMCNT(A_IN);
+            int ard = 0, awr = 2;
+            for (int s = 0; s < tsl; ++s) {
+                if (s) CLORA_WAIT_VMCNT(B_IN + A_IN);
+                CLORA_RAW_BARRIER();
+                issue_b(wr);
+                wr = (wr + 1 == NST) ? 0 : wr + 1;
+                issue_a2(s + 2, awr);
+                awr = (awr + 1 == 3) ? 0 : awr + 1;
+                const half_t* As = Pb + ard * AST;
+                ard = (ard + 1 == 3) ? 0 : ard + 1;
+                const half_t* Bs = Bring + rd * BST;
+                rd = (rd + 1 == NST) ? 0 : rd + 1;
+                half8 af[2][FM], bf[2][FN];
+#pragma unroll
+                for (int i = 0; i < FM; ++i) {
+                    const half_t* q = As + (wm * FM * 16 + i * 16 + li) * 64;
+                    af[0][i] = ld8(q + ((g ^ (li & 7)) * 8));
+                    af[1][i] = ld8(q + (((4 + g) ^ (li & 7)) * 8));
+                }
+#pragma unroll
+                for (int ks = 0; ks < 2; ++ks)
+#pragma unroll
+                    for (int j = 0; j < FN; ++j) bf[ks][j] = ld8(Bs + (wn * FN * 16 + j * 16 + li) * BK + bsw[ks]);
+#pragma unroll
+                for (int ks = 0; ks < 2; ++ks)
+#pragma unroll
+                    for (int i = 0; i < FM; ++i)
+#pragma unroll
+                        for (int j = 0; j < FN; ++j) acc[i][j] = mfma16(af[ks][i], bf[ks][j], acc[i][j]);
+            }
         }
     }
     CLORA_WAIT_VMCNT(0);
@@ -1766,7 +1831,7 @@
     return fast ? 2 : 1;
 }
 
-int g_opts[CLORA_OPT_COUNT] = {3, 1, 0, 0, 512, 1, 1, 0, 1, 1, 4, 1, 512, 2};
+int g_opts[CLORA_OPT_COUNT] = {3, 1, 0, 0, 512, 1, 1, 0, 1, 1, 4, 1, 512, 2, 1};
 int tile_order_mode() { return g_opts[CLORA_OPT_TILE_ORDER]; }
 
 double fabric_model_bytes(int tiles_m, int tiles_n, int splits, double a_panel, double b_panel, bool n_major) {
@@ -1796,7 +1861,7 @@
     const int mode = tile_order_mode();
     if (mode == 0 || a.tiles_m == 1 || a.tiles_n == 1) return;
     if (mode == 1) { a.n_major = 1; return; }
-    const double kper = patch ? (double)a.k_per_split * 576 : (double)a.k_per_split;
+    const double kper = patch ? (double)a.k_per_split * (a.c2a ? 64 : 576) : (double)a.k_per_split;
     const double a_panel = a.conv.enabled && a.conv.ksize == 3 ? BM * (kper / 9.0) * 2.0 * 1.5 : BM * kper * 2.0;
     const double b_panel = BN * kper * 2.0;
     const double m_cost = fabric_model_bytes(a.tiles_m, a.tiles_n, splits, a_panel, b_panel, false);
@@ -1896,6 +1961,7 @@
         if (r.tile_cfg == cfg) return r;
     return kNoTile;
 }
+const clora_gemm_tile_t& default_patch_tile(int N) { return tile_row((N % 160 == 0) ? 76 : 72); }
 
 template <int BM, int BN, int WM, int WN, int NST = 3, int BK = 32, int FLAGS = 0>
 int launch_gemm(GemmArgs& a, int splits, hipStream_t s, bool dma) {
@@ -1955,12 +2021,24 @@
     return patch_eligible(a, r.bm, r.family == CLORA_TILE_PATCH_WIDE ? kPatchWide : 0);
 }
 
+constexpr bool tile_carries_tail(int BM, int BN) { return !(BM == 256 && BN == 160); }
+bool tail_eligible(const GemmArgs& a, const clora_gemm_tile_t& r, int ca, int cb) {
+    if (!clora_option(CLORA_OPT_RESNET_FUSE_SHORTCUT) || !is_patch_tile(r) || !tile_carries_tail(r.bm, r.bn) || !patch_eligible(a, r)) return false;
+    const clora_conv_t& c = a.conv;
+    if (c.shift != 0 || c.kmul != 1) return false;
+    return ca > 0 && cb >= 0 && (ca % 64) == 0 && (cb % 64) == 0;
+}
+
 template <int BM, int BN, int WM, int WN, int NST, int MAXPP_ = 0>
 int launch_patch(GemmArgs& a, int splits, hipStream_t s) {
     a.tiles_n = clora_cdiv(a.N, BN);
     pick_tile_order(a, BM, BN, splits, true);
     const dim3 grid(clora_cdiv(a.M, BM) * a.tiles_n, splits);
-    hipLaunchKernelGGL((conv3x3_patch_kernel<BM, BN, WM, WN, NST, MAXPP_>), grid, dim3(WM * WN * 64), 0, s, a);
+    if (a.c2a) {
+        if constexpr (tile_carries_tail(BM, BN)) hipLaunchKernelGGL((conv3x3_patch_kernel<BM, BN, WM, WN, NST, MAXPP_, true>), grid, dim3(WM * WN * 64), 0, s, a);
+        else return CLORA_ERR_ARG;
+    }
+    else hipLaunchKernelGGL((conv3x3_patch_kernel<BM, BN, WM, WN, NST, MAXPP_>), grid, dim3(WM * WN * 64), 0, s, a);
     return clora_check_launch();
 }
 
@@ -2007,9 +2085,10 @@
 }
 }
 
-extern "C" int clora_gemm_f16_ex(const clora_half* A, int lda, const clora_half* B, clora_half* C, int ldc, int M, int N,
-                                 int K, const clora_conv_t* conv, const clora_epilogue_t* epi, int split_k, int tile_cfg,
-                                 void* workspace, size_t workspace_bytes, void* stream) {
+namespace {
+int gemm_f16_impl(const clora_half* A, int lda, const clora_half* B, clora_half* C, int ldc, int M, int N,
+                  int K, const clora_conv_t* conv, const clora_conv_tail_t* tail, const clora_epilogue_t* epi, int split_k, int tile_cfg,
+                  void* workspace, size_t workspace_bytes, void* stream) {
     if (!A || !B || (!C && !(epi && epi->geglu == 1)) || M <= 0 || N <= 0 || K <= 0 || (K & 7) || (N & 7) || (ldc & 7)) return CLORA_ERR_ARG;
     GemmArgs a;
     a.A = (const half_t*)A; a.B = (const half_t*)B; a.C = (half_t*)C; a.partial = nullptr;
@@ -2017,9 +2096,16 @@
     a.tiles_m = 0; a.n_major = 0; a.xg_s = a.xg_m = a.xg_n = 0;
     a.two_phase = g_opts[CLORA_OPT_EPI_TWO_PHASE];
     a.hoist_on = g_opts[CLORA_OPT_EPI_HOIST];
+    a.a2a = a.a2b = nullptr; a.c2a = a.c2b = a.ld2a = a.ld2b = 0;
+    if (tail) {
+        if (!conv || !conv->enabled || !tail->a || tail->ca <= 0 || tail->cb < 0 || (tail->cb > 0 && !tail->b) || tail->lda < tail->ca ||
+            (tail->cb > 0 && tail->ldb < tail->cb) || (tail->lda & 7) || (tail->ldb & 7) || ((uintptr_t)tail->a & 15) || ((uintptr_t)tail->b & 15))
+            return CLORA_ERR_ARG;
+        a.a2a = (const half_t*)tail->a; a.a2b = (const half_t*)tail->b; a.c2a = tail->ca; a.c2b = tail->cb; a.ld2a = tail->lda; a.ld2b = tail->ldb;
+    }
     if (conv && conv->enabled) {
         a.conv = *conv;
-        if ((conv->Cin & 7) || K != conv->ksize * conv->ksize * conv->Cin) return CLORA_ERR_ARG;
+        if ((conv->Cin & 7) || K != conv->ksize * conv->ksize * conv->Cin + a.c2a + a.c2b) return CLORA_ERR_ARG;
         if (conv->kchunk < 0 || (conv->kchunk > 0 && ((conv->kchunk & 7) || conv->Cin % conv->kchunk))) return CLORA_ERR_ARG;
     } else {
         a.conv = clora_conv_t();
@@ -2052,7 +2138,7 @@
     }
     hipStream_t s = (hipStream_t)stream;
     if (tile_row(tile_cfg).family == CLORA_TILE_STRIP) {
-        const int plan = (a.conv.enabled && split_k <= 1 && !defer && !a.epi.rowadd && !a.epi.residual && !a.epi.lora_t && !a.epi.geglu &&
+        const int plan = (a.conv.enabled && !tail && split_k <= 1 && !defer && !a.epi.rowadd && !a.epi.residual && !a.epi.lora_t && !a.epi.geglu &&
                           !a.epi.ln_out && !a.epi.c_lo && C && (ldc & 3) == 0 && K == 9 * a.conv.Cin)
                              ? strip_plan(M, N, a.conv) : 0;
         if (plan) {
@@ -2085,7 +2171,7 @@
     }
     const clora_gemm_tile_t* row = &tile_row(tile_cfg > 0 ? tile_cfg : kTiles[tile].cfg);
     const bool dma = row->family != CLORA_TILE_V1;
-    const clora_gemm_tile_t& patch = tile_row((N % 160 == 0) ? 76 : 72);
+    const clora_gemm_tile_t& patch = default_patch_tile(N);
     if (tile_cfg == 0 && !a.epi.geglu && patch_eligible(a, patch)) {
         row = &patch;
         if (split_k == 0) {
@@ -2101,13 +2187,21 @@
         if (!dma) return CLORA_ERR_ARG;
         if (a.epi.geglu == 1 && !(row->caps & kG)) { if (tile_cfg > 0) return CLORA_ERR_ARG; row = &tile_row(1); }
     }
+    if (tail && (a.epi.geglu || !tail_eligible(a, *row, a.c2a, a.c2b))) return CLORA_ERR_ARG;
     if (is_patch_tile(*row)) {
         if (!patch_eligible(a, *row)) row = &tile_row(21);
         else {
             const int slabs = a.conv.Cin / 64;
+            if (tail) {
+                const int steps = 9 * slabs + (a.c2a + a.c2b) / 64;
+                a.k_per_split = clora_cdiv(steps, splits < 1 ? 1 : splits);
+                if (a.k_per_split < 9) a.k_per_split = 9;
+                splits = clora_cdiv(steps, a.k_per_split);
+            } else {
             if (splits > slabs) splits = slabs;
             a.k_per_split = clora_cdiv(slabs, splits);
             splits = clora_cdiv(slabs, a.k_per_split);
+            }
             if (splits > 1) {
                 if (!workspace || workspace_bytes < (size_t)splits * M * N * sizeof(float)) return CLORA_ERR_WORKSPACE;
                 a.partial = (float*)workspace;
@@ -2145,6 +2239,27 @@
     if (rc != CLORA_OK) return rc;
     if (splits > 1) rc = finish_or_defer(a, splits, defer, s);
     return rc;
+}
+}
+
+extern "C" int clora_gemm_f16_ex(const clora_half* A, int lda, const clora_half* B, clora_half* C, int ldc, int M, int N,
+                                 int K, const clora_conv_t* conv, const clora_epilogue_t* epi, int split_k, int tile_cfg,
+                                 void* workspace, size_t workspace_bytes, void* stream) {
+    return gemm_f16_impl(A, lda, B, C, ldc, M, N, K, conv, nullptr, epi, split_k, tile_cfg, workspace, workspace_bytes, stream);
+}
+
+extern "C" int clora_conv3x3_tail_f16(const clora_half* A, const clora_half* B, clora_half* C, int ldc, int M, int N, int K,
+                                      const clora_conv_t* conv, const clora_conv_tail_t* tail, const clora_epilogue_t* epi, int split_k,
+                                      int tile_cfg, void* workspace, size_t workspace_bytes, void* stream) {
+    if (!tail) return CLORA_ERR_ARG;
+    return gemm_f16_impl(A, 0, B, C, ldc, M, N, K, conv, tail, epi, split_k, tile_cfg, workspace, workspace_bytes, stream);
+}
+
+extern "C" int clora_conv_tail_eligible(int M, int N, const clora_conv_t* conv, int ca, int cb, int tile_cfg) {
+    if (!conv || M <= 0 || N <= 0) return 0;
+    GemmArgs a;
+    a.M = M; a.N = N; a.conv = *conv;
+    return tail_eligible(a, tile_cfg > 0 ? tile_row(tile_cfg) : default_patch_tile(N), ca, cb) ? 1 : 0;
 }
 
 extern "C" int clora_gemm_ln_fusable(int M, int N, int K, int tile_cfg, int split_k) {
@@ -2194,7 +2309,7 @@
                                 {"lora_down_mode", CLORA_OPT_LORA_DOWN_MODE, 0, 2}, {"gn_unroll", CLORA_OPT_GN_UNROLL, 0, 1},
                                 {"epi_hoist", CLORA_OPT_EPI_HOIST, 0, 1}, {"gn_resident", CLORA_OPT_GN_RESIDENT, 0, 1},
                                 {"defer_max_rows", CLORA_OPT_DEFER_MAX_ROWS, 0, 16}, {"wgrad_patch", CLORA_OPT_WGRAD_PATCH, 0, 8192}, {"strip_blocks", CLORA_OPT_STRIP_BLOCKS, 64, 16384},
-                                {"gn_team", CLORA_OPT_GN_TEAM, 0, 4}};
+                                {"gn_team", CLORA_OPT_GN_TEAM, 0, 4}, {"resnet_fuse_shortcut", CLORA_OPT_RESNET_FUSE_SHORTCUT, 0, 1}};
     for (const Opt& o : kOpts)
         if (!strcmp(name, o.name)) {
             if (value < o.lo || value > o.hi) return CLORA_ERR_ARG;
diff --git a/controllora_amd/kernels.py b/controllora_amd/kernels.py
--- a/controllora_amd/kernels.py
+++ b/controllora_amd/kernels.py
@@ -7,7 +7,7 @@
 import torch
 
 from . import capi
-from .capi import ConvDesc, Epilogue, ptr
+from .capi import ConvDesc, ConvTail, Epilogue, ptr
 
 f16, f32 = torch.float16, torch.float32
 
@@ -162,7 +162,8 @@
          split_k: int = 0, tile_cfg: int = 0, _tuned: bool = True,
          geglu: int = 0, geglu_h: Optional[torch.Tensor] = None, geglu_y: Optional[torch.Tensor] = None,
          geglu_keep_h: bool = True, lora_dpack: Optional[torch.Tensor] = None, lora_t_in: Optional[torch.Tensor] = None,
-         lora_t_in_mask: int = 0, lora_t_in_rows: int = 0, defer: bool = False, ln=None, trunk: bool = False) -> torch.Tensor:
+         lora_t_in_mask: int = 0, lora_t_in_rows: int = 0, defer: bool = False, ln=None, trunk: bool = False,
+         tail: Optional[Tuple[torch.Tensor, Optional[torch.Tensor]]] = None) -> torch.Tensor:
     assert A.dtype == f16 and Bw.dtype == f16 and Bw.shape == (N, K) and Bw.is_contiguous()
     e = Epilogue()
     if geglu == 1:
@@ -212,7 +213,17 @@
             assert lora_t_in.dtype == f32 and lora_t_in.stride(1) == 1
             e.lora_t_in, e.ldt_in, e.lora_t_in_rows, e.lora_t_in_mask = ptr(lora_t_in), lora_t_in.stride(0), int(lora_t_in_rows), int(lora_t_in_mask)
         split_k = 1
-    if (CONV_STRIP and conv is not None and split_k == 0 and tile_cfg == 0 and not geglu and rowadd is None and residual is None
+    ct = None
+    if tail is not None:
+        ta, tb = tail
+        assert conv is not None and not geglu and ln is None and lora_t is None
+        for t_ in (ta, tb):
+            assert t_ is None or (t_.dtype == f16 and t_.dim() == 2 and t_.shape[0] == M and t_.stride(1) == 1)
+        ct = ConvTail(ptr(ta, f16), ptr(tb, f16), ta.shape[1], tb.shape[1] if tb is not None else 0, ta.stride(0),
+                      tb.stride(0) if tb is not None else 0)
+        if _tuned and split_k == 0 and tile_cfg == 0:
+            tile_cfg, split_k = conv_tail_plan(M, N, K, conv, ct.ca + ct.cb)
+    if (CONV_STRIP and conv is not None and tail is None and split_k == 0 and tile_cfg == 0 and not geglu and rowadd is None and residual is None
             and lora_t is None and not defer and ln is None and capi.lib().cdll.clora_conv_strip_eligible(M, N, C.byref(conv))):
         tile_cfg, split_k = 61, 1
     if _tuned and split_k == 0 and tile_cfg == 0:
@@ -239,13 +250,14 @@
     if defer and DEFER_FINISH and split_k != 1 and not geglu and PROFILER is None and C_ is not None and C_.is_contiguous():
         d = capi.Deferred()
         e.defer = C.addressof(d)
-    _call("clora_gemm_f16_ex", ptr(A), lda if lda is not None else K, ptr(Bw), ptr(C_) if C_ is not None else None, ldc, M, N, K,
-          C.byref(conv) if conv is not None else None, C.byref(e), split_k, tile_cfg,
+    head = ("clora_gemm_f16_ex", ptr(A), lda if lda is not None else K) if ct is None else ("clora_conv3x3_tail_f16", ptr(A))
+    _call(*head, ptr(Bw), ptr(C_) if C_ is not None else None, ldc, M, N, K,
+          C.byref(conv) if conv is not None else None, *((C.byref(ct),) if ct is not None else ()), C.byref(e), split_k, tile_cfg,
           ptr(ws) if ws is not None else None, ws.numel() if ws is not None else 0,
           flops=2.0 * M * N * K, nbytes=2.0 * (A.numel() + N * K + M * N),
           tag=f"{M}x{N}x{K}{'conv' if conv is not None else ''}")
     if d is not None and d.splits > 1:
-        _PENDING[C_.data_ptr()] = (d, (C_, bias, rowadd, residual, lora_t, lora_u, ws, trunk_hit))
+        _PENDING[C_.data_ptr()] = (d, (C_, bias, rowadd, residual, lora_t, lora_u, ws, trunk_hit, tail))
         task = _graph_task_id()
         if task >= 0 and _pending_task[0] != task:
             _pending_task[0] = task
@@ -322,6 +334,16 @@
 
 def conv_patch_eligible(M: int, conv: ConvDesc, tile_cfg: int) -> bool:
     return bool(capi.lib().cdll.clora_conv_patch_eligible(M, C.byref(conv), tile_cfg))
+
+
+def conv_tail_plan(M: int, N: int, K: int, conv: ConvDesc, c2: int) -> Tuple[int, int]:
+    hit = tuned_entry(M, N, K, conv) or tuned_entry(M, N, K - c2, conv)
+    return tuple(hit) if hit is not None else (0, 0)
+
+
+def conv_tail_eligible(M: int, N: int, conv: ConvDesc, ca: int, cb: int) -> bool:
+    tile_cfg, _ = conv_tail_plan(M, N, 9 * conv.Cin + ca + cb, conv, ca + cb)
+    return bool(capi.lib().cdll.clora_conv_tail_eligible(M, N, C.byref(conv), ca, cb, tile_cfg))
 
 
 TILE_ORDERS = {"m": 0, "n": 1, "auto": 2, "grid": 3}
@@ -477,13 +499,13 @@
     return workspace(n, device)
 
 
-def groupnorm_fwd(x, gamma, beta, G, eps, silu, x2=None, x_lo=None, x2_lo=None):
+def groupnorm_fwd(x, gamma, beta, G, eps, silu, x2=None, x_lo=None, x2_lo=None, want_cat=True):
     B, HW, Ca = x.shape
     Cc = Ca + (x2.shape[-1] if x2 is not None else 0)
     src, _keep = take_pending(x)
     y = torch.empty((B, HW, Cc), dtype=f16, device=x.device)
     stats = torch.empty((B, G, 2), dtype=f32, device=x.device)
-    xcat = torch.empty((B, HW, Cc), dtype=f16, device=x.device) if x2 is not None else None
+    xcat = torch.empty((B, HW, Cc), dtype=f16, device=x.device) if x2 is not None and want_cat else None
     if src is not None and x2 is not None:
         capi.lib().call("clora_finish_deferred", C.byref(src), capi.stream())
         src = None
diff --git a/controllora_amd/ops.py b/controllora_amd/ops.py
--- a/controllora_amd/ops.py
+++ b/controllora_amd/ops.py
@@ -96,6 +96,22 @@
         self.stride, self.pad, self.upsample, self.asym_pad = stride, pad, upsample, asym_pad
 
 
+class ConvShortcutPack:
+
+    def __init__(self, conv: ConvPack, shortcut: LinearPack):
+        assert conv.kchunk == 64 and conv.stride == 1 and not conv.upsample and not conv.asym_pad and shortcut.N == conv.Cop
+        self.conv, self.shortcut = conv, shortcut
+        self.C2 = shortcut.K
+        self.w = torch.cat([conv.w, shortcut.w], 1).contiguous()
+        self.bias = _sum_biases(conv.bias, shortcut.bias)
+
+
+def _sum_biases(b2: Optional[torch.Tensor], bs: Optional[torch.Tensor]) -> Optional[torch.Tensor]:
+    if b2 is None or bs is None:
+        return b2 if bs is None else bs
+    return (b2.to(f32) + bs.to(f32)).contiguous()
+
+
 class _FrozenLinearFn(torch.autograd.Function):
     @staticmethod
     def forward(ctx, x, pack: LinearPack, residual, rowadd, rows_per_batch, defer_out=False, defer_dx=False, ln=None, trunk=False):
@@ -146,6 +162,43 @@
     return _FrozenConvFn.apply(x, pack, B, H, W, residual, rowadd, defer_out, defer_dx)
 
 
+class _FrozenConvShortcutFn(torch.autograd.Function):
+
+    @staticmethod
+    def forward(ctx, h, xa, xb, pack: ConvShortcutPack, B, H, W, defer_out=False, defer_dx=False):
+        p = pack.conv
+        cd, Ho, Wo = K.conv_fwd_desc(H, W, p.Cip, 3, 1, p.pad, False, False, p.kchunk)
+        M = B * Ho * Wo
+        assert xb is None or not (ctx.needs_input_grad[1] or ctx.needs_input_grad[2])
+        y = K.gemm(h, pack.w, M, p.Cop, 9 * p.Cip + pack.C2, conv=cd, bias=pack.bias, tail=(xa, xb), defer=defer_out, trunk=True)
+        ctx.pack, ctx.dims, ctx.defer_dx = pack, (B, H, W, Ho, Wo), defer_dx
+        return y
+
+    @staticmethod
+    def backward(ctx, dy):
+        dy = dy.contiguous()
+        p, sp = ctx.pack.conv, ctx.pack.shortcut
+        B, H, W, Ho, Wo = ctx.dims
+        dh = dx = None
+        if ctx.needs_input_grad[0]:
+            cdd = K.conv_dgrad_desc(Ho, Wo, p.Cop, H, W, 3, 1, p.pad, False, p.kchunk_d)
+            dh = K.gemm(dy, p.wd, B * H * W, p.Cip, 9 * p.Cop, conv=cdd, defer=ctx.defer_dx)
+        if ctx.needs_input_grad[1]:
+            dx = K.gemm(dy, sp.wt, dy.shape[0], sp.K, sp.N)
+        return dh, dx, None, None, None, None, None, None, None
+
+
+def conv3x3_shortcut_fusable(pack: ConvPack, shortcut: LinearPack, B, H, W, ca, cb=0) -> bool:
+    if pack.kchunk != 64 or pack.stride != 1 or pack.upsample or pack.asym_pad or shortcut.N != pack.Cop or shortcut.K != ca + cb:
+        return False
+    cd, Ho, Wo = K.conv_fwd_desc(H, W, pack.Cip, 3, 1, pack.pad, False, False, pack.kchunk)
+    return K.conv_tail_eligible(B * Ho * Wo, pack.Cop, cd, ca, cb)
+
+
+def frozen_conv3x3_shortcut(h, xa, xb, pack: ConvShortcutPack, B, H, W, defer_out=False, defer_dx=False):
+    return _FrozenConvShortcutFn.apply(h, xa, xb, pack, B, H, W, defer_out, defer_dx)
+
+
 class _GroupNormFn(torch.autograd.Function):
 
     @staticmethod
@@ -176,8 +229,10 @@
 class _GroupNormCatFn(torch.autograd.Function):
 
     @staticmethod
-    def forward(ctx, a, b, gamma, beta, G, eps, silu):
-        y, stats, xcat = K.groupnorm_fwd(a, gamma, beta, G, eps, silu, x2=b, x_lo=K.trunk_lo_of(a, b), x2_lo=K.trunk_lo_of(b, a))
+    def forward(ctx, a, b, gamma, beta, G, eps, silu, want_cat=True):
+        assert want_cat or not (ctx.needs_input_grad[0] or ctx.needs_input_grad[1])
+        y, stats, xcat = K.groupnorm_fwd(a, gamma, beta, G, eps, silu, x2=b, x_lo=K.trunk_lo_of(a, b), x2_lo=K.trunk_lo_of(b, a),
+                                         want_cat=want_cat)
         ctx.save_for_backward(xcat, gamma, beta, stats)
         ctx.cfg = (G, silu, a.shape[-1])
         return y, xcat
@@ -188,11 +243,11 @@
         G, silu, Ca = ctx.cfg
         (da, db), _, _ = K.groupnorm_bwd(xcat, dy.contiguous(), gamma, beta, stats, G, silu,
                                          dres=dres.contiguous().view_as(xcat) if dres is not None else None, split_at=Ca)
-        return da, db, None, None, None, None, None
-
-
-def group_norm_cat(a, b, gamma, beta, G, eps, silu):
-    return _GroupNormCatFn.apply(a, b, gamma, beta, G, eps, silu)
+        return da, db, None, None, None, None, None, None
+
+
+def group_norm_cat(a, b, gamma, beta, G, eps, silu, want_cat=True):
+    return _GroupNormCatFn.apply(a, b, gamma, beta, G, eps, silu, want_cat)
 
 
 def group_norm_fork(x, gamma, beta, G, eps, silu):
diff --git a/controllora_amd/unet.py b/controllora_amd/unet.py
--- a/controllora_amd/unet.py
+++ b/controllora_amd/unet.py
@@ -107,9 +107,9 @@
         g, b = self.pack()
         return ops.group_norm_fork(x, g, b, self.groups, self.eps, silu)
 
-    def fork_cat(self, x, skip, silu):
+    def fork_cat(self, x, skip, silu, want_cat=True):
         g, b = self.pack()
-        return ops.group_norm_cat(x, skip, g, b, self.groups, self.eps, silu)
+        return ops.group_norm_cat(x, skip, g, b, self.groups, self.eps, silu, want_cat)
 
 
 class LayerNorm(_Norm):
@@ -270,6 +270,13 @@
         self.norm2 = GroupNorm(groups, cout, eps)
         self.conv2 = Conv3x3(cout, cout)
         self.conv_shortcut = Conv1x1(cin, cout) if cin != cout else None
+        self._fused, self._fused_key = None, None
+
+    def _fused_pack(self):
+        c, s = self.conv2.pack(), self.conv_shortcut.pack()
+        if self._fused is None or self._fused_key != (id(c), id(s)):
+            self._fused, self._fused_key = ops.ConvShortcutPack(c, s), (id(c), id(s))
+        return self._fused
 
     def forward(self, x, temb_act, H, W, temb_proj=None, skip=None, out_to_norm=False, trunk_out=True):
         B, N, _ = x.shape
@@ -279,14 +286,21 @@
             with torch.no_grad():
                 t = self.time_emb_proj(temb_act)
         grad = torch.is_grad_enabled() and (x.requires_grad or (skip is not None and skip.requires_grad))
+        Ca, Cb = x.shape[-1], (skip.shape[-1] if skip is not None else 0)
+        fuse = self.conv_shortcut is not None and ops.conv3x3_shortcut_fusable(self.conv2.pack(), self.conv_shortcut.pack(), B, H, W, Ca, Cb)
         if skip is not None:
-            n, xr = self.norm1.fork_cat(x, skip, True)
+            n, xr = self.norm1.fork_cat(x, skip, True, want_cat=grad or not fuse)
         else:
             n, xr = self.norm1.fork(x, True) if grad else (self.norm1(x, True), x)
-        Cin = xr.shape[-1]
+        Cin = Ca + Cb
         h = self.conv1(n.reshape(B * N, Cin), B, H, W, rowadd=t, defer_out=True, defer_dx=grad)
         Cout = h.shape[1]
         h = self.norm2(h.reshape(B, N, Cout), True).reshape(B * N, Cout)
+        if fuse:
+            xa, xb = (xr.reshape(B * N, Cin), None) if xr is not None else (x.reshape(B * N, Ca), skip.reshape(B * N, Cb))
+            with K.TrunkNoOut(not trunk_out, norm_reads=out_to_norm):
+                return ops.frozen_conv3x3_shortcut(h, xa, xb, self._fused_pack(), B, H, W, defer_out=out_to_norm,
+                                                   defer_dx=grad).reshape(B, N, Cout)
         x2 = xr.reshape(B * N, Cin)
         sc = self.conv_shortcut(x2, trunk=True) if self.conv_shortcut is not None else x2
         with K.TrunkNoOut(not trunk_out, norm_reads=out_to_norm):
diff --git a/include/clora.h b/include/clora.h
--- a/include/clora.h
+++ b/include/clora.h
@@ -105,6 +105,17 @@
 
 int clora_conv_patch_eligible(int M, const clora_conv_t* conv, int tile_cfg);
 
+typedef struct {
+    const clora_half* a;
+    const clora_half* b;
+    int ca, cb;
+    int lda, ldb;
+} clora_conv_tail_t;
+int clora_conv3x3_tail_f16(const clora_half* A, const clora_half* B, clora_half* C, int ldc, int M, int N, int K,
+                           const clora_conv_t* conv, const clora_conv_tail_t* tail, const clora_epilogue_t* epi, int split_k,
+                           int tile_cfg, void* workspace, size_t workspace_bytes, void* stream);
+int clora_conv_tail_eligible(int M, int N, const clora_conv_t* conv, int ca, int cb, int tile_cfg);
+
 int clora_conv_strip_eligible(int M, int N, const clora_conv_t* conv);
 
 int clora_set_option(const char* name, int value);
```

Result: no change. 185.0 images/s (median of 6 runs) (+0.7%).
